# nv-tlabs/DiffusionTexturePainting

Measured on AMD Instinct MI355X. Metric: 512x512 inpaint stamps/sec @20 DDIM steps, higher is better.
Workload: dtype f16

## Files before the change

### diffusiontexturepainting_amd/_lib.py

```python
import ctypes as C
import os

import torch

_HERE = os.path.dirname(os.path.abspath(__file__))
LIB_PATH = os.environ.get("DTP_LIB") or os.path.join(_HERE, "libdtp.so")
_lib = None
MAX_SLOTS = 16
SCHEDULERS = {"DDIM": 0, "DPM": 1, "LMSD": 2}
SCHED_ROW = 8


def scheduler_id(name):
    if name not in SCHEDULERS:
        raise ValueError(f"scheduler {name!r} is not supported: choose one of {', '.join(SCHEDULERS)}")
    return SCHEDULERS[name]


class DtpError(RuntimeError):
    pass


class Settings(C.Structure):
    _fields_ = [("steps", C.c_int), ("context_pad", C.c_int), ("tg_steps", C.c_int), ("cfg_weight", C.c_float),
# ... 115 lines not shown
                ("st_out", C.c_void_p), ("st_in", C.c_void_p), ("st_parts", C.c_int), ("st_parts_out", C.c_int),
                ("W8", C.c_void_p), ("ldw8", C.c_int), ("a_scale", C.c_float), ("w_scale", C.c_float), ("gn_cpg", C.c_int), ("Wfr", C.c_void_p),
                ("A8", C.c_void_p), ("lda8", C.c_int), ("A2_8", C.c_void_p), ("lda2_8", C.c_int), ("C8", C.c_void_p), ("ldc8", C.c_int),
                ("c_scale", C.c_float), ("a2_scale", C.c_float)]


GF_BIAS, GF_BIAS_M, GF_RESID, GF_GEGLU, GF_GELU, GF_QUICKGELU, GF_OUT_F32, GF_SILU, GF_LNFOLD = 1, 2, 4, 8, 64, 128, 256, 512, 1024
GF_SOFTMAX16 = 4096
GF_ROWSTATS = 2048
GF_GNSTATS = 1 << 24
GF_RAGGED = 1 << 25

_vp, _i, _f, _i64 = C.c_void_p, C.c_int, C.c_float, C.c_int64
SYMBOLS = {
    "dtp_abi_version": (_i, []),
    "dtp_last_error": (C.c_char_p, []),
    "dtp_create": (_i, [_i, _i, _i, C.POINTER(_vp)]),
    "dtp_destroy": (None, [_vp]),
    "dtp_load_tensor": (_i, [_vp, C.c_char_p, _vp, _i, C.POINTER(_i64), _i]),
    "dtp_finalize_weights": (_i, [_vp]),
    "dtp_vae_encode": (_i, [_vp, _vp, _vp, _vp, _i, _vp]),
    "dtp_unet": (_i, [_vp, _vp, _f, _vp, _vp, _i, _vp]),
    "dtp_vae_decode": (_i, [_vp, _vp, _vp, _i, _vp]),
    "dtp_set_brush": (_i, [_vp, _vp, _i, _i, _vp, _vp]),
    "dtp_set_conditioning": (_i, [_vp, _vp, _vp, _vp, _vp]),
    "dtp_get_conditioning": (_i, [_vp, _vp, _vp, _vp]),
    "dtp_stamp": (_i, [_vp, _vp, C.POINTER(Settings), _vp, _vp, _vp, _i, _vp]),
    "dtp_stamp_slots": (_i, [_vp, _vp, C.POINTER(Settings), _vp, _vp, _vp, _i, C.POINTER(_i), _vp]),
    "dtp_stamp_mixed": (_i, [_vp, _vp, C.POINTER(Settings), _vp, _vp, _vp, _i, C.POINTER(_i), _vp]),
    "dtp_set_brush_slot": (_i, [_vp, _i, _vp, _i, _i, _vp, _vp]),
    "dtp_set_conditioning_slot": (_i, [_vp, _i, _vp, _vp, _vp, _vp]),
    "dtp_get_conditioning_slot": (_i, [_vp, _i, _vp, _vp, _vp]),
    "dtp_ddim_tables": (_i, [_i, C.POINTER(_i64), C.POINTER(_f), C.POINTER(_f)]),
    "dtp_last_stamp_times": (_i, [_vp, C.POINTER(_f * 3)]),
    "dtp_last_stamp_info": (_i, [_vp, C.POINTER(_i), C.POINTER(_i)]),
    "dtp_last_stamp_unet_rows": (_i, [_vp, C.POINTER(_i)]),
    "dtp_profile": (_i, [_vp, _i]),
    "dtp_profile_rows": (_i, [_vp, C.POINTER(ProfRow), _i, C.POINTER(_i)]),
    "dtp_profile_dump": (_i, [_vp, C.c_char_p]),
    "dtp_set_option": (_i, [_vp, C.c_char_p, _i]),
    "dtp_last_stamp_finite": (_i, [_vp, C.POINTER(_i)]),
    "dtp_op_gemm": (_i, [C.POINTER(GemmDesc), _vp]),
    "dtp_op_gemm_f8f8": (_i, [C.POINTER(GemmDesc), _vp]),
    "dtp_op_quant_e4m3": (_i, [_vp, _i, _vp, _i, _i, _f, _i, _vp, _i, _vp, _i, _i, _f, _i, _i, _vp, _i, _f, _vp]),
    "dtp_op_pack_linear": (_i, [_vp, _vp, _i, _i, _i, _i, _vp]),
    "dtp_op_pack_conv": (_i, [_vp, _vp, _i, _i, _i, _i, _i, _vp]),
    "dtp_op_rowsum": (_i, [_vp, _i, _i, _vp, _i, _vp]),
    "dtp_op_quantize_w8": (_i, [_vp, _i, _i, _i, _vp, _i, C.POINTER(_f), _vp]),
    "dtp_op_pack_conv_cb": (_i, [_vp, _vp, _i, _i, _i, _vp]),
    "dtp_op_groupnorm_apply": (_i, [_vp, _i, _vp, _i, _vp, _vp, _vp, _i, _i, _i, _i, _i, _f, _i, _vp]),
    "dtp_op_groupnorm_stats_apply": (_i, [_vp, _i, _vp, _vp, _vp, _vp, _vp, _vp, _i, _i, _i, _i, _f, _i, _vp]),
    "dtp_op_pack_conv_ws": (_i, [_vp, _vp, _vp, _i, _i, _i, _vp]),
    "dtp_op_pack_conv_ws_elems": (C.c_longlong, [_i, _i, _i]),
    "dtp_op_pack_linear_ws": (_i, [_vp, _i, _vp, _i, _i, _vp]),
    "dtp_op_pack_linear_ws_elems": (C.c_longlong, [_i, _i]),
    "dtp_op_groupnorm": (_i, [_vp, _i, _vp, _i, _vp, _vp, _i, _i, _i, _i, _f, _i, _vp]),
    "dtp_op_measure_peaks": (_i, [C.POINTER(C.c_double), C.POINTER(C.c_double)]),
    "dtp_op_reduce_groupnorm": (_i, [_vp, _i, _vp, _vp, _vp, _vp, _vp, _vp, _i, _i, _i, _i, _f, _i, _vp]),
    "dtp_op_xattn": (_i, [_vp, _vp, _vp, _vp, _vp, _i, _vp, _vp, _vp, _vp, _vp, _i, _i, _i, _i, _f, _vp]),
    "dtp_op_reduce_groupnorm_cx": (_i, [_vp, _i, _vp, _vp, _vp, _vp, _vp, _vp, _i, _i, _i, _i, _f, _i, _i, _vp]),
    "dtp_op_xattn_ct": (_i, [_vp, _vp, _vp, _vp, _vp, _i, _vp, _vp, _vp, _vp, _vp, _i, _i, _i, _i, _f, _i, _vp]),
    "dtp_op_gn_fold_weights": (_i, [_vp, _vp, _i, _vp, _vp, _vp, _i, _i, _i, _i, _i, _f, _vp, _vp, _vp]),
    "dtp_op_ffchain": (_i, [_vp, _vp, _i, _vp, _vp, _vp, _i, _vp, _vp, _vp, _i, _i, _f, _vp]),
    "dtp_op_xchain": (_i, [_vp, _vp, _i, _vp, _vp, _vp, _vp, _vp, _vp, _vp, _vp, _vp, _i, _i, _i, _i, _f, _vp]),
    "dtp_op_gn_linear": (_i, [_vp, _vp, _i, _vp, _vp, _vp, _i, _i, _i, _i, _i, _f, _vp, _vp, _i, _vp]),
    "dtp_op_layernorm": (_i, [_vp, _i, _vp, _i, _vp, _vp, _i, _i, _f, _vp]),
    "dtp_op_attention": (_i, [_vp, _vp, _vp, _vp, _i, _i, _i, _i, _i, _i, _i, _i, _i, _i64, _i64, _i64, _i64, _f, _vp]),
    "dtp_op_attention_dma": (_i, [_vp, _vp, _vp, _vp, _i, _i, _i, _i, _i, _i, _i, _i, _i, _i64, _i64, _i64, _i64, _f, _i, _vp]),
    "dtp_op_softmax_rows": (_i, [_vp, _i, _vp, _i, _i, _i, _f, _vp]),
    "dtp_op_attention_fp8": (_i, [_vp, _vp, _vp, _vp, _i, _i, _i, _i, _i, _i, _i, _i, _i, _i64, _i64, _i64, _i64, _f, _f, _f, _vp]),
    "dtp_op_dilate": (_i, [_vp, _vp, _vp, _i, _i, _i, _vp]),
    "dtp_op_dilate_pads": (_i, [_vp, _vp, _vp, _i, _i, C.POINTER(_i), _vp]),
    "dtp_scheduler_tables": (_i, [_i, _i, C.POINTER(_i), C.POINTER(_f), C.POINTER(_f), C.POINTER(_f), C.POINTER(_f)]),
    "dtp_op_sched_step": (_i, [_i, _vp, _vp, _vp, _vp, _vp, _vp, _vp, _vp, _vp, _i, _i, _i, _i, _vp]),
    "dtp_stamp_strength": (_i, [_vp, _vp, C.POINTER(Settings), _vp, _vp, _vp, C.c_double, _vp, _i, C.POINTER(_i), _vp]),
    "dtp_strength_schedule": (_i, [_i, _i, C.c_double, C.POINTER(_i), C.POINTER(_i), C.POINTER(_f)]),
    "dtp_op_strength_init": (_i, [_vp, _vp, _f, _f, _vp, C.c_longlong, _vp]),
    "dtp_stamp_seeded": (_i, [_vp, _vp, C.POINTER(Settings), C.POINTER(C.c_uint64), _i, C.c_double, _vp, _i, C.POINTER(_i), _vp]),
    "dtp_op_stamp_noise": (_i, [C.c_uint64, _i, _vp, C.c_longlong, _vp]),
    "dtp_philox4x32": (_i, [C.POINTER(C.c_uint32), C.POINTER(C.c_uint32), C.POINTER(C.c_uint32)]),
    "dtp_refit_stage": (_i, [_vp, C.c_char_p, _vp, _i, C.POINTER(_i64), _i]),
    "dtp_refit_lora": (_i, [_vp, _f]),
    "dtp_last_refit_info": (_i, [_vp, C.POINTER(_i), C.POINTER(_i), C.POINTER(_f)]),
    "dtp_op_lora_refit": (_i, [_vp, _vp, _vp, _i, _f, _vp, _vp, _i, _i, _i, _i, _vp]),
    "dtp_stroke": (_i, [_vp, _vp, _i, _i, C.POINTER(StrokeStamp), _i, C.POINTER(Settings), C.POINTER(StrokeOpts), _vp, _vp]),
    "dtp_stroke_plan": (_i, [_i, _i, _i, _i, C.POINTER(StrokeStamp), _i, _i, C.POINTER(_i), C.POINTER(_i)]),
    "dtp_last_stroke_info": (_i, [_vp, C.POINTER(_i), C.POINTER(_i), C.POINTER(_i)]),
    "dtp_op_stroke_gather": (_i, [_vp, _i, _i, _vp, _i, _i, C.POINTER(_i), C.POINTER(_i), C.POINTER(_i), _i, _i, _i, _vp]),
    "dtp_op_stroke_paste": (_i, [_vp, _vp, _vp, _i, _i, _i, _i, C.POINTER(_i), C.POINTER(_i), C.POINTER(_i), _i, _vp]),
    "dtp_mesh_create": (_i, [_vp, _vp, _i, _vp, _i, _vp, C.POINTER(_vp)]),
    "dtp_mesh_destroy": (_i, [_vp]),
    "dtp_mesh_camera": (_i, [C.POINTER(_f * 3), C.POINTER(_f * 3), C.POINTER(_f * 3), _f, C.POINTER(_f * 12)]),
    "dtp_mesh_stroke": (_i, [_vp, _vp, _vp, _i, _i, C.POINTER(MeshStamp), _i, C.POINTER(Settings), C.POINTER(MeshStrokeOpts), _vp, _vp]),
    "dtp_op_mesh_render": (_i, [_vp, C.POINTER(_f * 12), _f, _i, _vp, _i, _i, _i, _i, _i, _i, _vp, _vp, _vp]),
    "dtp_op_mesh_backproject": (_i, [_vp, _vp, _i, _vp, _vp, _i, _vp, _i, _i, _vp]),
    "dtp_mesh_stroke_bleed": (_i, [_vp, _vp, _vp, _i, _i, C.POINTER(MeshStamp), _i, C.POINTER(Settings), C.POINTER(MeshStrokeOpts), _vp, _i, _vp]),
    "dtp_mesh_bleed": (_i, [_vp, _vp, _i, _i, _i, C.POINTER(_i * 4), _vp]),
    "dtp_op_mesh_coverage": (_i, [_vp, _i, _i, _vp, _vp]),
    "dtp_mesh_bleed_offsets": (_i, [_i, C.POINTER(_i), C.POINTER(C.c_byte)]),
    "dtp_mesh_pick": (_i, [_vp, C.POINTER(Ray), _i, _vp, _vp]),
    "dtp_mesh_ray_frame": (_i, [C.POINTER(_f * 3), C.POINTER(_f * 3), C.POINTER(_f * 12)]),
    "dtp_mesh_path_plan": (_i, [_vp, _i, _f, C.POINTER(PathState), _vp, _vp, _vp, _i, C.POINTER(_i)]),
    "dtp_op_mesh_pick": (_i, [_vp, C.POINTER(Ray), _i, _vp, _vp]),
    "dtp_view_camera": (_i, [C.POINTER(_f * 3), C.POINTER(_f * 3), C.POINTER(_f * 3), _f, _i, _i, _f, C.POINTER(ViewCam)]),
    "dtp_view_rays": (_i, [C.POINTER(ViewCam), _i, _i, _vp, _i, _vp]),
    "dtp_mesh_view": (_i, [_vp, _vp, _i, _i, C.POINTER(ViewCam), _i, _i, C.POINTER(ViewOpts), _vp, _vp, _vp, _vp]),
# ... 68 lines not shown
```

### diffusiontexturepainting_amd/csrc/api_ops.hip

```cpp
#include <stdarg.h>
#include <stdio.h>
#include <stdlib.h>
#include <mutex>
#include <vector>

#include "../../include/dtp.h"
#include "common.h"

static thread_local char g_err[1024] = "";

void dtp_set_error(const char* fmt, ...) {
  va_list ap;
  va_start(ap, fmt);
  vsnprintf(g_err, sizeof(g_err), fmt, ap);
  va_end(ap);
}

namespace {
struct OpsScratch {
  f16* zero = nullptr;
  float* ws = nullptr;
  size_t ws_bytes = 0;
  int* geglu_map = nullptr;
  int geglu_map_n = 0;
  int num_cu = 256;
  bool init = false;
};
OpsScratch g_ops;
std::mutex g_ops_mu;

int ops_init() {
  if (g_ops.init) return DTP_OK;
  HIP_CHECK(hipMalloc(&g_ops.zero, 256));
  HIP_CHECK(hipMemset(g_ops.zero, 0, 256));
  hipDeviceProp_t prop;
  int dev = 0;
  HIP_CHECK(hipGetDevice(&dev));
  HIP_CHECK(hipGetDeviceProperties(&prop, dev));
  g_ops.num_cu = prop.multiProcessorCount;
  g_ops.init = true;
  return DTP_OK;
}

int ops_ws(size_t bytes) {
  if (bytes <= g_ops.ws_bytes) return DTP_OK;
  HIP_CHECK(hipDeviceSynchronize());
  if (g_ops.ws) HIP_CHECK(hipFree(g_ops.ws));
  g_ops.ws = nullptr;
  g_ops.ws_bytes = 0;
  HIP_CHECK(hipMalloc(&g_ops.ws, bytes));
  g_ops.ws_bytes = bytes;
  return DTP_OK;
}
}

extern "C" {

int dtp_abi_version(void) { return DTP_ABI_VERSION; }
const char* dtp_last_error(void) { return g_err; }

int dtp_op_gemm(dtp_gemm_desc* d, dtp_stream s) {
  std::lock_guard<std::mutex> lk(g_ops_mu);
  int rc = ops_init();
  if (rc) return rc;
  static bool halo_init = false;
  if (!halo_init) { dtp_conv_halo_init(); dtp_gemm_wide_init(); dtp_lnlin_init(); dtp_conv_ws_init(); dtp_gemm_ws_init(); halo_init = true; }
  GemmParams p = {};
  p.A = (const f16*)d->A; p.W = (const f16*)d->W; p.C = d->C; p.bias = d->bias; p.R = (const f16*)d->R;
  p.zero = g_ops.zero;
  p.M = d->M; p.N = d->N; p.K = d->K;
  p.lda = d->lda; p.ldw = d->ldw; p.ldc = d->ldc; p.ldr = d->ldr;
  p.nkb = (d->K + 63) / 64;
  p.Hi = d->Hi; p.Wi = d->Wi; p.Ho = d->Ho; p.Wo = d->Wo; p.Cin = d->Cin; p.stride = d->stride; p.pad = d->pad;
  p.flags = d->flags | (d->conv ? GF_CONV3 : 0) | (d->upsample2x ? GF_UPS2 : 0);
  p.lns = d->lns; p.ln_eps = d->ln_eps;
  p.A2 = (const f16*)d->A2; p.lda2 = d->lda2; p.Cin2 = d->Cin2;
  p.batch = d->batch; p.a_bs = d->a_bs; p.w_bs = d->w_bs; p.c_bs = d->c_bs; p.r_bs = d->r_bs;
  p.bias_bs = d->bias_bs; p.lns_bs = d->lns_bs; p.sm_valid = d->sm_valid;
  p.st_out = d->st_out; p.st_in = d->st_in; p.st_parts = d->st_parts;
  if (p.batch > 1) p.st_rows = p.batch * p.M;
  p.W8 = (const unsigned char*)d->W8; p.ldw8 = d->ldw8; p.a_scale = d->a_scale; p.w_scale = d->w_scale;
  p.Wfr = (const f16*)d->Wfr;
  p.gn_cpg = d->gn_cpg;
  static bool fp8_init = false;
  if (!fp8_init) { dtp_gemm_fp8_init(); fp8_init = true; }
  if (p.ldw < p.nkb * 64) { dtp_set_error("gemm: ldw=%d smaller than padded K=%d", p.ldw, p.nkb * 64); return DTP_ERR_ARG; }
  int tile = 0;
  dtp_gemm_pick(p, &tile, g_ops.num_cu);
  if (d->tile >= 0) tile = d->tile;
  const DtpTile t = dtp_tile(tile);
  int sp = t.split == SPLIT_COLS ? 4 : t.split == SPLIT_K ? p.splits : 1;
  if (d->splits >= 1 && (d->batch <= 1 || t.split != SPLIT_K)) sp = d->splits;
  if ((t.fam == TF_FP8) != (p.W8 != nullptr)) { dtp_set_error("gemm: tiles 24..28 and W8 go together"); return DTP_ERR_ARG; }
  if (t.fam == TF_HALO && !d->Wcb) { dtp_set_error("conv_halo: Wcb missing"); return DTP_ERR_ARG; }
  p.Wcb = (const f16*)d->Wcb;
  (void)dtp_tile_apply(p, tile, sp);
  rc = ops_ws(dtp_gemm_workspace_bytes(p));
  if (rc) return rc;
  p.part = g_ops.ws;
  if (p.flags & GF_ROWSTATS) d->st_parts_out = dtp_tile_row_parts(p, tile);
  return dtp_launch_tile(p, tile, (hipStream_t)s);
}

int dtp_op_gemm_f8f8(dtp_gemm_desc* d, dtp_stream s) {
  std::lock_guard<std::mutex> lk(g_ops_mu);
  int rc = ops_init();
  if (rc) return rc;
  static bool f8f8_init = false;
  if (!f8f8_init) { dtp_gemm_f8f8_init(); f8f8_init = true; }
  GemmParams p = {};
  p.A8 = (const unsigned char*)d->A8; p.lda8 = d->lda8;
  p.A2_8 = (const unsigned char*)d->A2_8; p.lda2_8 = d->lda2_8; p.Cin2 = d->A2_8 ? d->Cin2 : 0;
  p.W8 = (const unsigned char*)d->W8; p.ldw8 = d->ldw8;
  p.C = d->C; p.ldc = d->ldc; p.C8 = (unsigned char*)d->C8; p.ldc8 = d->ldc8;
  p.bias = d->bias; p.R = (const f16*)d->R; p.ldr = d->ldr;
  p.zero = g_ops.zero;
  p.M = d->M; p.N = d->N; p.K = d->K;
  p.flags = d->flags;
  p.st_out = d->st_out;
  p.a_scale = d->a_scale; p.w_scale = d->w_scale; p.c_scale = d->c_scale; p.a2_scale = d->a2_scale;
  p.splits = 1;
  const int tile = d->tile >= 0 ? d->tile : dtp_gemm_f8f8_pick(p, g_ops.num_cu);
  if (p.flags & GF_ROWSTATS) d->st_parts_out = (p.N + 127) / 128;
  return dtp_launch_gemm_f8f8(p, tile, (hipStream_t)s);
}

int dtp_op_quant_e4m3(const void* x, int ldx, void* y, int ldy, int K, float scale, int ln, const void* x2, int ldx2, void* y2, int ldy2,
                      int K2, float scale2, int ln2, int M, const float* st_in, int st_parts, float eps, dtp_stream s) {
  Quant8Params q = {};
  q.M = M; q.njobs = x2 ? 2 : 1;
  q.job[0] = Quant8Job{(const f16*)x, ldx, K, (unsigned char*)y, ldy, scale, ln};
  if (x2) q.job[1] = Quant8Job{(const f16*)x2, ldx2, K2, (unsigned char*)y2, ldy2, scale2, ln2};
  q.st_in = st_in; q.st_parts = st_parts; q.st_rows = M; q.eps = eps;
  return dtp_launch_quant8(q, (hipStream_t)s);
}

int dtp_op_pack_linear(const float* w, void* out, int N, int K, int ldw, int geglu, dtp_stream s) {
  std::lock_guard<std::mutex> lk(g_ops_mu);
  int rc = ops_init();
  if (rc) return rc;
  const int* map = nullptr;
  if (geglu) {
    if (N % 256) { dtp_set_error("pack_linear: GEGLU needs N %% 256 == 0"); return DTP_ERR_ARG; }
    std::vector<int> h(N);
    for (int f = 0; f < N / 2; ++f) {
      h[f] = (f / 64) * 128 + (f % 64);
      h[N / 2 + f] = (f / 64) * 128 + 64 + (f % 64);
    }
    if (g_ops.geglu_map_n < N) {
      if (g_ops.geglu_map) HIP_CHECK(hipFree(g_ops.geglu_map));
      HIP_CHECK(hipMalloc(&g_ops.geglu_map, sizeof(int) * N));
      g_ops.geglu_map_n = N;
    }
    HIP_CHECK(hipMemcpyAsync(g_ops.geglu_map, h.data(), sizeof(int) * N, hipMemcpyHostToDevice, (hipStream_t)s));
    HIP_CHECK(hipStreamSynchronize((hipStream_t)s));
    map = g_ops.geglu_map;
  }
  return dtp_launch_pack_linear_weight(w, (f16*)out, N, K, ldw, map, (hipStream_t)s);
}

int dtp_op_quantize_w8(const void* w, int ldw, int K, int rows, void* out, int ldw8, float* w_scale, dtp_stream s) {
  if (!w || !out || !w_scale || (ldw8 & 127) || ldw8 < K) { dtp_set_error("quantize_w8: bad argument"); return DTP_ERR_ARG; }
  return dtp_quantize_weights_fp8((const f16*)w, ldw, K, rows, (unsigned char*)out, ldw8, w_scale, (hipStream_t)s);
}

int dtp_op_rowsum(const void* w, int ld, int K, float* out, int rows, dtp_stream s) {
  return dtp_launch_rowsum_f16((const f16*)w, ld, K, out, rows, (hipStream_t)s);
}

int dtp_op_pack_conv(const float* w, void* out, int Cout, int Cin, int Cin_pad, int taps, int ldw, dtp_stream s) {
  return dtp_launch_pack_conv_weight(w, (f16*)out, Cout, Cin, Cin_pad, taps, ldw, (hipStream_t)s);
}

int dtp_op_pack_conv_cb(const float* w, void* out, int Cout, int Cin, int ldw, dtp_stream s) {
  return dtp_launch_pack_conv_weight_cb(w, (f16*)out, Cout, Cin, ldw, (hipStream_t)s);
}

int dtp_op_pack_conv_ws(const float* w, const float* w1, void* out, int Cout, int Cin, int Cin2, dtp_stream s) {
  return dtp_launch_pack_conv_ws(w, w1, (f16*)out, Cout, Cin, Cin2, (hipStream_t)s);
}
int dtp_op_pack_linear_ws(const void* w, int ldw, void* out, int N, int K, dtp_stream s) {
  return dtp_launch_pack_linear_ws((const f16*)w, ldw, (f16*)out, N, K, (hipStream_t)s);
}
long long dtp_op_pack_linear_ws_elems(int N, int K) { return (long long)dtp_gemm_ws_packed_elems(N, K); }
long long dtp_op_pack_conv_ws_elems(int Cout, int Cin, int Cin2) { return (long long)dtp_conv_ws_packed_elems(Cout, Cin, Cin2); }

int dtp_op_groupnorm(const void* x, int ldx, void* y, int ldy, const float* gamma, const float* beta, int B, int HW, int C,
                     int groups, float eps, int silu, dtp_stream s) {
  std::lock_guard<std::mutex> lk(g_ops_mu);
  int rc = ops_init();
  if (rc) return rc;
  rc = ops_ws(dtp_groupnorm_ws_bytes(B, HW, C, groups));
  if (rc) return rc;
  return dtp_launch_groupnorm(GnParams{(const f16*)x, ldx, (f16*)y, ldy, gamma, beta, B, HW, C, groups, eps, silu}, g_ops.ws, (hipStream_t)s);
}

int dtp_op_groupnorm_apply(const void* x, int ldx, void* y, int ldy, const float* gamma, const float* beta, const float* partial, int nchunk,
                           int B, int HW, int C, int groups, float eps, int silu, dtp_stream s) {
  return dtp_launch_groupnorm_apply(GnParams{(const f16*)x, ldx, (f16*)y, ldy, gamma, beta, B, HW, C, groups, eps, silu}, partial, nchunk, (hipStream_t)s);
}

int dtp_op_reduce_groupnorm_cx(const float* part, int splits, const float* bias, const void* resid, void* conv_out, void* y, const float* gamma,
                               const float* beta, int B, int HW, int C, int groups, float eps, int silu, int cx, dtp_stream s) {
  std::lock_guard<std::mutex> lk(g_ops_mu);
  int rc = ops_init();
  if (rc) return rc;
  rc = ops_ws(dtp_groupnorm_ws_bytes(B, HW, C, groups));
  if (rc) return rc;
  if (cx <= 0 || cx > C) { dtp_set_error("reduce_groupnorm: cx %d outside (0, C = %d]", cx, C); return DTP_ERR_ARG; }
  const GnReduceSrc rd = {part, splits, (long long)B * HW * cx, cx, bias, (const f16*)resid, cx};
  return dtp_launch_reduce_groupnorm(GnParams{(const f16*)conv_out, C, (f16*)y, C, gamma, beta, B, HW, C, groups, eps, silu}, rd, cx, g_ops.ws, (hipStream_t)s);
}

int dtp_op_reduce_groupnorm(const float* part, int splits, const float* bias, const void* resid, void* conv_out, void* y, const float* gamma,
                            const float* beta, int B, int HW, int C, int groups, float eps, int silu, dtp_stream s) {
  return dtp_op_reduce_groupnorm_cx(part, splits, bias, resid, conv_out, y, gamma, beta, B, HW, C, groups, eps, silu, C, s);
}

int dtp_op_gn_fold_weights(const void* x, const void* W, int ldw, const float* bias, const float* gamma, const float* beta, int B, int HW, int C,
                           int Nout, int groups, float eps, void* Wout, float* bias_out, dtp_stream s) {
  std::lock_guard<std::mutex> lk(g_ops_mu);
  int rc = ops_init();
  if (rc) return rc;
  rc = ops_ws(dtp_groupnorm_ws_bytes(B, HW, C, groups));
  if (rc) return rc;
  const GnParams gp = {(const f16*)x, C, nullptr, 0, gamma, beta, B, HW, C, groups, eps, 0};
  rc = dtp_launch_groupnorm_stats(gp, g_ops.ws, nullptr, (hipStream_t)s);
  if (rc) return rc;
  const int rows = (Nout + 127) / 128 * 128;
  return dtp_launch_gn_fold_weights(gp, g_ops.ws, 0, (const f16*)W, ldw, bias, Nout, (f16*)Wout, (long long)rows * ldw, bias_out, rows, (hipStream_t)s);
}

int dtp_op_groupnorm_stats_apply(const float* part, int splits, const float* bias, const void* resid, void* x, void* y, const float* gamma,
                                 const float* beta, int B, int HW, int C, int groups, float eps, int silu, dtp_stream s) {
  if (part && splits < 1) { dtp_set_error("groupnorm_stats_apply: %d slabs", splits); return DTP_ERR_ARG; }
  std::lock_guard<std::mutex> lk(g_ops_mu);
  int rc = ops_init();
  if (rc) return rc;
// ... 129 lines not shown
```

### diffusiontexturepainting_amd/csrc/builder.hip

```cpp
#include "engine.h"

#include <math.h>
#include <stdio.h>

#include <algorithm>

static Op make_gemm_op(Ctx* c, GemmParams p, int tile, int bias_step_off);

static const float* step_bias(const Ctx* c, int bias_step_off, int step, const float* fallback) {
  return bias_step_off >= 0 ? c->temb_table + (size_t)step * c->unet.temb_total + bias_step_off : fallback;
}
static constexpr int GF_CLAIMABLE = GF_BIAS | GF_RESID | GF_CONV3 | GF_UPS2 | GF_MFAST | GF_RAGGED;

void prog_push(Ctx* c, Prog* prog, int kind, double flops, double bytes, Op fn, const std::string& label) {
  prog->last_gemm.valid = false;
  prog->ops.push_back([=](hipStream_t s, int step) -> int {
    if (!c->profile) return fn(s, step);
    ProfRec r;
    r.kind = kind; r.flops = flops; r.bytes = bytes; r.label = label.c_str();
    HIP_CHECK(hipEventCreate(&r.e0));
    HIP_CHECK(hipEventCreate(&r.e1));
    HIP_CHECK(hipEventRecord(r.e0, s));
    const int rc = fn(s, step);
    HIP_CHECK(hipEventRecord(r.e1, s));
// ... 250 lines not shown
  HIP_CHECK(hipMemsetAsync(c->fp8_amax, 0, DTP_FP8_SLOTS * sizeof(unsigned int), s));
  c->calibrating = true;
  const int rc = up->main.run(s, step);
  c->calibrating = false;
  RC(rc);
  std::vector<float> amax(DTP_FP8_SLOTS);
  HIP_CHECK(hipMemcpyAsync(amax.data(), c->fp8_amax, DTP_FP8_SLOTS * sizeof(float), hipMemcpyDeviceToHost, s));
  HIP_CHECK(hipStreamSynchronize(s));
  auto pow2_for = [](float a) { return a > 0.f ? exp2f(ceilf(log2f(a * DTP_FP8_MARGIN / 448.0f))) : 1.0f; };
  for (size_t i = up->cal_begin; i < up->cal_end; ++i) {
    Fp8Cal& r = c->fp8_cals[i];
    if (r.kind == 0) {
      *r.s0 = pow2_for(amax[r.slot0]);
    } else {
      const float aq = amax[r.slot0] * r.softmax_scale * 1.4426950408889634f, ak = amax[r.slot0 + 1], av = amax[r.slot0 + 2];
      *r.s0 = (aq > 0.f && ak > 0.f) ? exp2f(roundf(0.5f * log2f(ak / aq))) : 1.0f;
      *r.s1 = pow2_for(av);
    }
  }
  up->fp8_calibrated = true;
  return DTP_OK;
}

static Op make_gemm_op(Ctx* c, GemmParams p, int tile, int bias_step_off) {
  return [=](hipStream_t s, int step) -> int {
    GemmParams q = p;
    q.part = c->ws;
    if (p.a_scale_host) {
      if (c->calibrating && p.amax_slot1 > 0) {
        const int ka = p.A2 ? p.K - p.Cin2 : p.K;
        RC(dtp_launch_amax_f16(p.A, p.M, ka, p.lda, c->fp8_amax + p.amax_slot1 - 1, s));
        if (p.A2) RC(dtp_launch_amax_f16(p.A2, p.M, p.Cin2, p.lda2, c->fp8_amax + p.amax_slot1 - 1, s));
      }
      q.a_scale = *p.a_scale_host;
    }
    q.bias = step_bias(c, bias_step_off, step, q.bias);
    return dtp_launch_tile(q, tile, s);
  };
}

int push_gemm(Ctx* c, Prog* prog, GemmParams p, int bias_step_off, double k_alg, RowStats* emit) {
  if (!emit_rowstats(p, emit)) emit = nullptr;
  int tile = 0;
  dtp_gemm_pick(p, &tile, c->num_cu);
  int sp = p.splits;
  if (p.W8) { tile = 24 + ((p.flags & GF_GEGLU) ? (p.M >= 512 ? 0 : 3) : (p.M >= 512 ? 0 : 2)); sp = 1; }
  if ((p.flags & GF_GNAPPLY) && (p.flags & GF_CONV3)) { tile = (p.Hi * p.Wi <= 256) ? 14 : 12; sp = 1; }
  if ((p.flags & GF_GNAPPLY) && !(p.flags & GF_CONV3)) {
    tile = DTP_TILE_LNLIN;
    sp = lnlin_default_ranges(p);
    if (!sp) { dtp_set_error("push_gemm: no lnlin configuration for the GroupNorm-on-load Linear (M %d N %d K %d)", p.M, p.N, p.K); return DTP_ERR_ARG; }
  }
  if (c->autotune) RC(tune_gemm(c, p, &tile, &sp));
  (void)dtp_tile_apply(p, tile, sp);
  const DtpTile t = dtp_tile(tile);
  if (emit) {
    emit->parts = dtp_tile_row_parts(p, tile);
    emit->M = p.M * (p.batch > 1 ? p.batch : 1);
  }
  c->ws_need = std::max(c->ws_need, dtp_gemm_workspace_bytes(p));
  p.zero = c->zero;
  const double n_out = (p.flags & GF_GEGLU) ? p.N / 2.0 : (double)p.N;
  const double a_elems = (p.flags & GF_CONV3) ? (double)p.M * (k_alg / 9.0) * ((p.flags & GF_UPS2) ? 0.25 : (double)(p.stride * p.stride))
                                               : (double)p.M * k_alg;
  const double nb = p.batch > 1 ? (double)p.batch : 1.0;
  const double bytes = 2.0 * nb * (a_elems + (double)p.N * k_alg + (double)p.M * n_out);
  char lab[160];
  const bool f8tile = t.fam == TF_FP8;
  snprintf(lab, sizeof(lab), "%s M=%d N=%d K=%d tile=%d splits=%d%s%s%s%s", (p.flags & GF_CONV3) ? "conv3" : "gemm", p.M, p.N, p.K, tile,
           t.split == SPLIT_COLS ? p.col_ranges : p.splits, (p.flags & GF_UPS2) ? " ups" : "", (p.flags & GF_GEGLU) ? (f8tile ? " geglu fp8" : " geglu") : (f8tile ? " fp8" : ""), p.stride == 2 ? " s2" : "",
           p.batch > 1 ? (" x" + std::to_string(p.batch)).c_str() : "");
  const double flops = 2.0 * nb * p.M * (double)p.N * k_alg;
  prog_push(c, prog, t.pk, flops, bytes, make_gemm_op(c, p, tile, bias_step_off), lab);
  if (p.splits > 1 || (t.fam == TF_CONVWS && t.var >= 2)) {
    LastGemm& lg = prog->last_gemm;
    lg.valid = true; lg.p = p; lg.tile = tile; lg.bias_step_off = bias_step_off; lg.op_index = prog->ops.size() - 1;
    lg.kind = t.pk; lg.flops = flops; lg.bytes = bytes; lg.label = lab;
  }
  return DTP_OK;
}

int Builder::conv3(const T& x, const ConvW& w, int stride, int pad, bool ups, int Ho, int Wo, const T* resid, int bias_step_off, T& y,
                   const Conv3Opts& o) {
  if ((w.cin2 > 0) != (o.tail != nullptr) || (o.tail && o.tail->C != w.cin2)) { dtp_set_error("conv3: shortcut tail mismatch"); return DTP_ERR_ARG; }
  if (x.C != w.cin || w.taps != 9) { dtp_set_error("conv3: channel mismatch %d vs %d", x.C, w.cin); return DTP_ERR_ARG; }
  GemmParams p = {};
  p.A = x.p; p.W = w.w;
  p.M = x.B * Ho * Wo; p.N = w.cout; p.K = w.K;
  p.lda = x.ld; p.ldw = w.ldw;
  p.nkb = w.ldw / 64;
  p.Hi = x.H; p.Wi = x.W; p.Ho = Ho; p.Wo = Wo; p.Cin = w.cin; p.stride = stride; p.pad = pad;
  p.flags = GF_CONV3 | (ups ? GF_UPS2 : 0) | o.extra_flags;
  if (c->R % 64) p.flags |= GF_RAGGED;
  if (o.tail) { p.A2 = o.tail->p; p.lda2 = o.tail->ld; p.Cin2 = w.cin2; }
  p.Wcb = w.wcb;
  p.Wfr = w.wfr;
  if (o.extra_flags & GF_GNAPPLY) {
    if (!o.gn.part) { dtp_set_error("conv3: GF_GNAPPLY without GroupNorm parameters"); return DTP_ERR_ARG; }
    p.gn_part = o.gn.part; p.gn_gamma = o.gn.gamma; p.gn_beta = o.gn.beta; p.gn_eps = o.gn.eps;
    p.gn_nchunk = o.gn.nchunk; p.gn_cpg = o.gn.cpg; p.gn_silu = 1;
  }
  if (o.out_override) {
    y = T();
    y.p = (f16*)o.out_override; y.B = x.B; y.H = Ho; y.W = Wo; y.C = w.cout; y.ld = o.ldc_override;
  } else if (o.dst) {
    if (o.dst->C != w.cout || o.dst->rows() != (long long)x.B * Ho * Wo) { dtp_set_error("conv3: destination view mismatch"); return DTP_ERR_ARG; }
    y = *o.dst;
  } else {
    y = alloc(x.B, Ho, Wo, w.cout);
    if (!y.p) return DTP_ERR_HIP;
  }
  p.C = y.p; p.ldc = y.ld;
  if (w.b || bias_step_off >= 0) { p.flags |= GF_BIAS; p.bias = w.b; }
  if (resid) { p.flags |= GF_RESID; p.R = resid->p; p.ldr = resid->ld; }
  return push_gemm(c, prog, p, bias_step_off, 9.0 * w.cin_true + w.cin2);
}

int Builder::gn_conv3(const T& x, const NormW& n, float eps, const ConvW& w, const T* resid, int bias_step_off, T& y, const T* tail, const T* dst) {
  Ctx* cc = c;
  const int HW = x.H * x.W, C = x.C;
  Conv3Opts opts;
  opts.tail = tail; opts.dst = dst;
  const bool fuse = cc->fuse_gn_conv && HW >= 1024 && x.rows() <= 16384 && w.wcb && w.taps == 9 && (C & 63) == 0 && C <= 1024 && x.C == w.cin && (C % 32) == 0 && C / 32 >= 8 &&
                    (w.cout & 7) == 0 && (x.ld & 7) == 0;
  if (!fuse) {
    T t;
    RC(gn(x, n, eps, true, t));
    RC(conv3(t, w, 1, 1, false, x.H, x.W, resid, bias_step_off, y, opts));
    release(t);
    return DTP_OK;
  }
  const ReduceClaim claim = claim_reduce(x);
  float* partials = (float*)block_clear_of_claim(cc, dtp_groupnorm_ws_bytes(x.B, HW, C, 32), claim, "gn_conv3", "partials");
  if (!partials) return DTP_ERR_HIP;
  cc->ws_need = std::max(cc->ws_need, claim.slab_bytes());
  push_gn_stats(*this, gn_params(x, n, eps, true), partials, claim, " (apply in conv)");
  opts.extra_flags = GF_GNAPPLY; opts.gn = {partials, n.g, n.b, eps, dtp_groupnorm_stat_chunks(HW), C / 32};
  const int rc = conv3(x, w, 1, 1, false, x.H, x.W, resid, bias_step_off, y, opts);
  ctx_pool_put(cc, partials);
  return rc;
}

int Builder::alloc_stats(long long rows, int C, RowStats& st) {
  void* p = nullptr;
  RC(ctx_pool_get(c, (size_t)((C + 63) / 64) * rows * 2 * sizeof(float), &p));
  st.buf = (float*)p;
  st.parts = 0;
  st.M = (int)rows;
  return DTP_OK;
// ... 176 lines not shown
```

### diffusiontexturepainting_amd/csrc/common.h

```cpp
#pragma once
#include <hip/hip_runtime.h>
#include <stdint.h>

#include "../../include/dtp.h"

typedef _Float16 f16;
typedef f16 f16x2 __attribute__((ext_vector_type(2)));
typedef f16 f16x4 __attribute__((ext_vector_type(4)));
typedef f16 f16x8 __attribute__((ext_vector_type(8)));
typedef float f32x4 __attribute__((ext_vector_type(4)));
typedef float f32x16 __attribute__((ext_vector_type(16)));

static __device__ __forceinline__ uint32_t lds_addr(const void* p) {
  return (uint32_t)(uintptr_t)(const __attribute__((address_space(3))) void*)p;
}
static __device__ __forceinline__ f16x8 lds_read16(uint32_t addr) {
  f16x8 v;
  asm volatile("ds_read_b128 %0, %1" : "=v"(v) : "v"(addr));
  return v;
}
template <int N, int NF>
static __device__ __forceinline__ void wait_lds_frags(f16x8 (&f)[NF]) {
  static_assert(NF == 2 || NF == 3 || NF == 4 || NF == 5 || NF == 6 || NF == 7 || NF == 8, "fragment count");
  if constexpr (NF == 2) asm volatile("s_waitcnt lgkmcnt(%2)" : "+v"(f[0]), "+v"(f[1]) : "n"(N));
// ... 140 lines not shown
}
static __device__ __forceinline__ void gn_mean_rstd(double s, double q, float inv_count, float eps, float& mean, float& rstd) {
  const float nf = rintf(1.0f / inv_count);
  const double n = (double)nf;
  double inv = (double)(1.0f / nf);
  inv = inv * (2.0 - n * inv);
  const double m = s * inv;
  const double var = q * inv - m * m;
  mean = (float)m;
  rstd = rsqrtf(fmaxf((float)var, 0.f) + eps);
}

#define DTP_WAVE 64

#define HIP_CHECK(x)                                                                        \
  do {                                                                                      \
    hipError_t e_ = (x);                                                                    \
    if (e_ != hipSuccess) {                                                                 \
      dtp_set_error("%s:%d %s -> %s", __FILE__, __LINE__, #x, hipGetErrorString(e_));       \
      return DTP_ERR_HIP;                                                                   \
    }                                                                                       \
  } while (0)


void dtp_set_error(const char* fmt, ...);

enum {
  GF_BIAS = 1,
  GF_BIAS_M = 2,
  GF_RESID = 4,
  GF_GEGLU = 8,
  GF_CONV3 = 16,
  GF_UPS2 = 32,
  GF_GELU = 64,
  GF_QUICKGELU = 128,
  GF_OUT_F32 = 256,
  GF_SILU = 512,
  GF_LNFOLD = 1024,
  GF_ROWSTATS = 2048,
  GF_SOFTMAX16 = 4096,
  GF_MFAST = 1 << 20,
  GF_NOREDUCE = 1 << 21,
  GF_XCDSPLIT = 1 << 23,
  GF_GNSTATS = 1 << 24,
  GF_RAGGED = 1 << 25,
  GF_GNAPPLY = 1 << 22,
};

struct GemmParams {
  const f16* A;
  const f16* W;
  const f16* Wcb;
  const f16* Wfr;
  void* C;
  float* part;
  const float* bias;
  const f16* R;
  const f16* zero;
  const float* lns;
  float ln_eps;
  const float* st_in;
  int st_parts;
  float* st_out;
  int M, N, K;
  int lda, ldw, ldc, ldr;
  int nkb;
  int splits;
  int kb_per_split;
  int col_ranges;
  int Hi, Wi, Ho, Wo, Cin, stride, pad;
  const f16* A2;
  int lda2, Cin2;
  int flags;
  int batch;
  long long a_bs, w_bs, c_bs, r_bs;
  int bias_bs, lns_bs, st_rows;
  int sm_valid;
  const float *gn_part, *gn_gamma, *gn_beta;
  int gn_nchunk, gn_cpg, gn_silu;
  float gn_eps;
  const unsigned char* W8;
  int ldw8;
  float a_scale, w_scale;
  const float* a_scale_host;
  int amax_slot1;
  const unsigned char* A8;
  int lda8;
  const unsigned char* A2_8;
  int lda2_8;
  unsigned char* C8;
  int ldc8;
  float c_scale;
  float a2_scale;
};

struct Quant8Job {
  const f16* x; int ld, K;
  unsigned char* y; int ldy;
  float scale;
  int ln;
};
struct Quant8Params {
  int M, njobs;
  Quant8Job job[2];
  const float* st_in; int st_parts, st_rows;
  float eps;
// ... 93 lines not shown
  int dup;
};
bool dtp_xchain_supported(const XchainParams& p);
int dtp_launch_xchain(const XchainParams& p, hipStream_t s);
void dtp_xchain_init();

struct FfchainParams {
  const f16* X; int ldx;
  const f16* W1; int ldw1;
  const float *lns1, *b1;
  const f16* Wm; int ldwm;
  const float* bm;
  const f16* R; int ldr;
  f16* Out; int ldo;
  int M, C;
  float ln_eps;
};
bool dtp_ffchain_supported(const FfchainParams& p);
int dtp_launch_ffchain(const FfchainParams& p, hipStream_t s);
void dtp_ffchain_init();

int dtp_launch_concat_channels(const f16* a, int lda, int Ca, const f16* b, int ldb, int Cb, f16* y, int ldy, long long rows,
                               hipStream_t s);
#define DTP_COPY_SEGS 8
struct CopySegs {
  int n;
  const char* src[DTP_COPY_SEGS];
  char* dst[DTP_COPY_SEGS];
  long long rows[DTP_COPY_SEGS], row_bytes[DTP_COPY_SEGS], src_stride[DTP_COPY_SEGS], dst_stride[DTP_COPY_SEGS];
  long long chunks[DTP_COPY_SEGS], total;
};
int dtp_launch_copy_rows(CopySegs segs, hipStream_t s);
int dtp_launch_f32_to_f16(const float* x, f16* y, long long n, hipStream_t s);
int dtp_launch_nchw_f32_to_nhwc_f16(const float* x, f16* y, int B, int C, int HW, int Cpad, hipStream_t s);
int dtp_launch_nhwc_f16_to_nchw_f32(const f16* x, int ldx, float* y, int B, int C, int HW, hipStream_t s);
int dtp_launch_pack_conv_weight(const float* w, f16* out, int Cout, int Cin, int Cin_pad, int taps, int ldw, hipStream_t s);
int dtp_launch_pack_linear_weight(const float* w, f16* out, int N, int K, int ldw, const int* row_map, hipStream_t s);
int dtp_launch_rowdot(const float* w, const float* v, float* out, int N, int K, hipStream_t s);
int dtp_launch_scale_cols(float* w, const float* g, int N, int K, hipStream_t s);
int dtp_launch_rowsum_f16(const f16* w, int ld, int K, float* out, int rows, hipStream_t s);
int dtp_launch_matmul_f32(const float* A, const float* B, float* C, int M, int N, int K, hipStream_t s);
int dtp_launch_expand_kv(const f16* kv, f16* kexp, f16* vexp, int N, int T, int C, int H, float scale, hipStream_t s);
int dtp_launch_transpose_f16(const f16* src, int lds_, f16* dst, int ldd, int rows, int cols, hipStream_t s);
int dtp_launch_rowdot_f16(const f16* a, int ld, const float* v, float* out, int rows, int K, hipStream_t s);
bool dtp_gemm_fp8_supported(const GemmParams& p);
int dtp_launch_gemm_fp8(const GemmParams& p, int tile, hipStream_t s);
void dtp_gemm_fp8_init();
int dtp_quantize_weights_fp8(const f16* w, int ldw, int K, int rows, unsigned char* out, int ldw8, float* scale_out, hipStream_t s);
bool dtp_gemm_wide_supported(const GemmParams& p, int variant);
int dtp_launch_gemm_wide(const GemmParams& p, int variant, hipStream_t s);
void dtp_gemm_wide_init();
constexpr int DTP_TILE_LNLIN = 50;
constexpr int DTP_TILE_WS0 = 51;
constexpr int DTP_WS_VARIANTS = 4;
constexpr int DTP_TILE_GEMMWS = 55;
constexpr int DTP_TILE_IDS = 56;

enum { PK_GEMM0 = 0, PK_ATTN = 12, PK_GN = 13, PK_LN = 14, PK_ELEM = 15, PK_SOFTMAX = 16, PK_HALO0 = 17, PK_BIG0 = 21, PK_WIDE0 = 25, PK_FP8 = 27, PK_KH2 = 28, PK_LW = 36, PK_XATTN = 44, PK_HALO3 = 45, PK_LNLIN = 47, PK_WS0 = 48, PK_GEMMWS = 52, PK_F8F8 = 53, PK_QUANT8 = 54, PK_COUNT = 55 };

enum DtpFamily : unsigned char { TF_NONE, TF_GEMM, TF_HALO, TF_WIDE, TF_FP8, TF_LNLIN, TF_CONVWS, TF_GEMMWS };
enum DtpSplit : unsigned char {
  SPLIT_K,
  SPLIT_HALO,
  SPLIT_BLOCKS,
  SPLIT_COLS,
  SPLIT_NONE,
};
struct DtpTile {
  DtpFamily fam;
  int var;
  int bm, bn, ns;
  int kh, lw;
  DtpSplit split;
  int pk;
};
inline DtpTile dtp_tile(int id) {
  static constexpr int sm[4] = {128, 128, 64, 64}, sn[4] = {128, 64, 64, 128};
  const int s = id & 3;
  if (id >= 0 && id < 12) return {TF_GEMM, 0, sm[s], sn[s], 2 + id / 4, 1, 0, SPLIT_K, PK_GEMM0 + id};
  if (id >= 12 && id < 16) return {TF_HALO, id - 12, 0, 0, 0, 0, 0, SPLIT_HALO, PK_HALO0 + id - 12};
  if (id >= 16 && id < 20) return {TF_GEMM, 0, id < 18 ? 256 : 128, id < 18 ? 128 : 256, 2 + (id & 1), 1, 0, SPLIT_K, PK_BIG0 + id - 16};
  if (id == 20 || id == 21) return {TF_WIDE, id - 20, 256, id == 20 ? 256 : 320, 2, 0, 0, SPLIT_NONE, PK_WIDE0 + id - 20};
  if (id >= 24 && id < 28) return {TF_FP8, id - 24, sm[s], sn[s], 2, 0, 0, SPLIT_NONE, PK_FP8};
  if (id == 28) return {TF_FP8, 4, 256, 256, 2, 0, 0, SPLIT_NONE, PK_FP8};
  if (id >= 32 && id < 40) return {TF_GEMM, 0, sm[s], sn[s], 2 + (id - 32) / 4, 2, 0, SPLIT_K, PK_KH2 + id - 32};
  if (id >= 40 && id < 48) return {TF_GEMM, 0, sm[s], sn[s], 3, 1, id < 44 ? 4 : 8, SPLIT_K, PK_LW + id - 40};
  if (id == 48 || id == 49) return {TF_HALO, id - 44, 0, 0, 0, 0, 0, SPLIT_HALO, PK_HALO3 + id - 48};
  if (id == DTP_TILE_LNLIN) return {TF_LNLIN, 0, 0, 0, 0, 0, 0, SPLIT_COLS, PK_LNLIN};
  if (id >= DTP_TILE_WS0 && id < DTP_TILE_WS0 + DTP_WS_VARIANTS) return {TF_CONVWS, id - DTP_TILE_WS0, 0, 0, 0, 0, 0, SPLIT_BLOCKS, PK_WS0 + id - DTP_TILE_WS0};
  if (id == DTP_TILE_GEMMWS) return {TF_GEMMWS, 0, 64, 64, 0, 0, 0, SPLIT_BLOCKS, PK_GEMMWS};
  return {};
}
inline bool dtp_tile_apply(GemmParams& p, int tile, int sp) {
  const DtpTile t = dtp_tile(tile);
  if (sp < 1) sp = 1;
  if (t.fam == TF_HALO) p.W = p.Wcb;
  if (t.split == SPLIT_NONE || t.split == SPLIT_COLS) {
    p.kb_per_split = p.nkb; p.splits = 1;
    if (t.split == SPLIT_COLS) p.col_ranges = sp;
    return t.split == SPLIT_COLS || sp == 1;
  }
  p.kb_per_split = (p.nkb + sp - 1) / sp;
  if (t.split == SPLIT_BLOCKS) { p.splits = sp; return true; }
  if (t.split == SPLIT_HALO && sp > 1) p.kb_per_split = (((p.nkb + 8) / 9 + sp - 1) / sp) * 9;
  p.splits = (p.nkb + p.kb_per_split - 1) / p.kb_per_split;
  return p.splits == sp;
}
inline int dtp_tile_row_parts(const GemmParams& p, int tile) {
  const DtpTile t = dtp_tile(tile);
  if (t.split == SPLIT_COLS) return p.col_ranges;
  if (!t.bn) return 0;
  return p.splits > 1 ? 1 : (p.N + t.bn - 1) / t.bn;
}
bool dtp_lnlin_supported(const GemmParams& p, int nsplit);
int dtp_launch_lnlin(const GemmParams& p, int nsplit, hipStream_t s);
void dtp_lnlin_init();
bool dtp_conv_ws_supported(const GemmParams& p, int variant, int nsplit);
int dtp_launch_conv_ws(const GemmParams& p, int variant, hipStream_t s);
void dtp_conv_ws_init();
size_t dtp_conv_ws_packed_elems(int Cout, int Cin, int Cin2);
int dtp_conv_ws_gn_chunks(int Ho, int Wo);
int dtp_launch_pack_conv_ws(const float* w, const float* w1, f16* out, int Cout, int Cin, int Cin2, hipStream_t s);
bool dtp_gemm_ws_supported(const GemmParams& p, int nsplit);
int dtp_launch_gemm_ws(const GemmParams& p, hipStream_t s);
void dtp_gemm_ws_init();
size_t dtp_gemm_ws_packed_elems(int N, int K);
int dtp_launch_pack_linear_ws(const f16* w, int ldw, f16* out, int N, int K, hipStream_t s);
bool dtp_conv_halo_supported(const GemmParams& p);
bool dtp_conv_halo3_supported(const GemmParams& p);
int dtp_launch_conv_halo(const GemmParams& p, int variant, hipStream_t s);
void dtp_conv_halo_init();
int dtp_launch_pack_conv_weight_cb(const float* w, f16* out, int Cout, int Cin, int ldw, hipStream_t s);
int dtp_launch_touch(const void* p, size_t bytes, float* sink, hipStream_t s);
int dtp_launch_amax_f16(const f16* x, long long rows, int cols, int ld, unsigned int* slot, hipStream_t s);
int dtp_launch_lora_merge(float* w, const float* up, const float* down, int N, int K, int rank, float scale, hipStream_t s);
```

### diffusiontexturepainting_amd/csrc/context.hip

```cpp
#include <stdio.h>
#include <stdlib.h>
#include <string.h>
#include <algorithm>

#include "engine.h"

int stamp_init(Ctx* c) {
  void* p;
  const size_t hw = (size_t)c->h * c->h, RR = (size_t)c->R * c->R;
  RC(ctx_persistent(c, c->maxB * hw * 4 * 4, &p, true)); c->x32 = (float*)p;
  RC(ctx_persistent(c, 3 * c->maxB * hw * 4 * 4, &p, true)); c->hist32 = (float*)p;
  RC(ctx_persistent(c, c->maxB * 4 * RR * 4, &p, true)); c->canvas32 = (float*)p;
  RC(ctx_persistent(c, 2 * c->maxB * RR * 4, &p, true)); c->alpha_tmp = (float*)p;
  RC(ctx_persistent(c, sizeof(StampParams), &p, true)); c->stamp_params = (StampParams*)p;
  RC(ctx_persistent(c, (size_t)DTP_MAX_SLOTS * 2 * 14 * 768 * 4, &p, true)); c->cond32 = (float*)p;
  RC(ctx_persistent(c, (size_t)DTP_MAX_SLOTS * 3 * RR * 4, &p, true)); c->brush32 = (float*)p;
  RC(ctx_persistent(c, 64 * sizeof(int), &p, true)); c->slot_map = (int*)p;
  RC(ctx_persistent(c, 256, &p, true)); c->finite_flag = (int*)p;
  RC(ctx_persistent(c, RR * 4, &p, true)); c->mesh_face_idx = (int*)p;
  return DTP_OK;
}

extern "C" {

int dtp_create(int device, int resolution, int max_batch, dtp_ctx** out) {
  if (!out || resolution < 64 || resolution % 8 || max_batch < 1 || max_batch > 64) {
    dtp_set_error("dtp_create: resolution must be a multiple of 8 and at least 64, 1 <= max_batch <= 64 (got resolution %d, max_batch %d)", resolution, max_batch);
    return DTP_ERR_ARG;
  }
  HIP_CHECK(hipSetDevice(device));
  Ctx* c = new Ctx();
  c->device = device; c->R = resolution; c->h = resolution / 8; c->maxB = max_batch;
  hipDeviceProp_t prop;
  HIP_CHECK(hipGetDeviceProperties(&prop, device));
  c->num_cu = prop.multiProcessorCount;
  void* z;
  HIP_CHECK(hipMalloc(&z, 4096));
  HIP_CHECK(hipMemset(z, 0, 4096));
  c->zero = (f16*)z;
  for (int i = 0; i < 4; ++i) HIP_CHECK(hipEventCreate(&c->ev[i]));
  tune_cache_load(c);
  auto on = [](const char* name) { const char* e = getenv(name); return e && e[0] && e[0] != '0'; };
  c->fuse_reduce_gn = !on("DTP_NO_FUSE_REDUCE_GN"); c->dedupe_prefix = !on("DTP_NO_DEDUPE");
#ifdef DTP_EXPERIMENTAL
  c->fuse_gn_conv = on("DTP_GN_CONV");
#endif
  c->fuse_xattn = !on("DTP_NO_XATTN"); c->fold_gn_linear = !on("DTP_NO_FOLD_GN");
  c->conv_ws = !on("DTP_NO_WS"); c->conv_ws_vae = !on("DTP_NO_WS_VAE"); c->gemm_ws = on("DTP_GEMMWS");
  c->gn_epilogue = !on("DTP_NO_GN_EPILOGUE"); c->reduce_in_concat_gn = !on("DTP_NO_REDUCE_IN_CONCAT_GN"); c->gna_lnlin = !on("DTP_NO_GNA_LNLIN");
  c->tune_lnlin = !on("DTP_NO_LNLIN"); c->tune_halo3 = !on("DTP_NO_HALO3");
  c->xchain = !on("DTP_NO_XCHAIN"); c->xattn_tiles = !on("DTP_XATTN_CT1");
  if (const char* e = getenv("DTP_FFCHAIN")) c->ffchain = atoi(e);
  *out = (dtp_ctx*)c;
  return DTP_OK;
}

void dtp_destroy(dtp_ctx* ctx) {
  Ctx* c = (Ctx*)ctx;
  if (!c) return;
  (void)hipSetDevice(c->device);
  (void)hipDeviceSynchronize();
  graphs_drop_all(c);
  journal_drop_ctx(c);
  delta_drop_ctx(c);
  mesh_drop_ctx(c);
  for (auto& s : c->staged) (void)hipFree(s.second.d);
  for (auto& s : c->refit_staged) (void)hipFree(s.second.d);
  for (int i = 0; i < 2; ++i) if (c->refit_ev[i]) (void)hipEventDestroy(c->refit_ev[i]);
  for (void* p : c->chunks) (void)hipFree(p);
  for (auto& b : c->pool.blocks) (void)hipFree(b.p);
  for (void* p : c->persistent) (void)hipFree(p);
  if (c->ws) (void)hipFree(c->ws);
  if (c->zero) (void)hipFree(c->zero);
  if (c->tune_thrash) (void)hipFree(c->tune_thrash);
  for (int i = 0; i < 4; ++i) if (c->ev[i]) (void)hipEventDestroy(c->ev[i]);
  delete c;
}

int dtp_load_tensor(dtp_ctx* ctx, const char* name, const float* data, int is_device, const int64_t* shape, int ndim) {
  Ctx* c = (Ctx*)ctx;
  if (!c || !name || !data || ndim < 1 || ndim > 4) { dtp_set_error("dtp_load_tensor: bad argument"); return DTP_ERR_ARG; }
  if (c->finalized) { dtp_set_error("dtp_load_tensor: weights already finalized"); return DTP_ERR_STATE; }
  HIP_CHECK(hipSetDevice(c->device));
  Staged s;
  s.n = 1;
  for (int i = 0; i < ndim; ++i) { s.shape.push_back(shape[i]); s.n *= (size_t)shape[i]; }
  HIP_CHECK(hipMalloc(&s.d, std::max<size_t>(s.n * 4, 16)));
  HIP_CHECK(hipMemcpy(s.d, data, s.n * 4, is_device ? hipMemcpyDeviceToDevice : hipMemcpyHostToDevice));
  auto it = c->staged.find(name);
  if (it != c->staged.end()) { (void)hipFree(it->second.d); c->staged.erase(it); }
  c->staged.emplace(name, std::move(s));
  return DTP_OK;
}

int dtp_finalize_weights(dtp_ctx* ctx) {
  Ctx* c = (Ctx*)ctx;
  if (!c) { dtp_set_error("dtp_finalize_weights: null handle"); return DTP_ERR_ARG; }
  if (c->finalized) { dtp_set_error("dtp_finalize_weights: already finalized"); return DTP_ERR_STATE; }
  HIP_CHECK(hipSetDevice(c->device));
  dtp_gemm_init();
  dtp_conv_halo_init();
  dtp_gemm_wide_init();
  dtp_gemm_fp8_init();
  dtp_gemm_f8f8_init();
  dtp_xattn_init();
// ... 75 lines not shown
  c->profile = enable != 0;
  return DTP_OK;
}

int dtp_profile_rows(dtp_ctx* ctx, dtp_prof_row* rows, int max_rows, int* n_rows) {
  Ctx* c = (Ctx*)ctx;
  if (!c || !rows || !n_rows) return DTP_ERR_ARG;
  HIP_CHECK(hipDeviceSynchronize());
  dtp_prof_row acc[PK_COUNT] = {};
  for (int k = 0; k < PK_COUNT; ++k) acc[k].kind = k;
  for (const ProfRec& r : c->prof) {
    float ms = 0.f;
    HIP_CHECK(hipEventElapsedTime(&ms, r.e0, r.e1));
    dtp_prof_row& a = acc[r.kind];
    a.launches += 1; a.ms += ms; a.flops += r.flops; a.bytes += r.bytes;
  }
  int n = 0;
  for (int k = 0; k < PK_COUNT && n < max_rows; ++k)
    if (acc[k].launches) rows[n++] = acc[k];
  *n_rows = n;
  return DTP_OK;
}

int dtp_profile_dump(dtp_ctx* ctx, const char* path) {
  Ctx* c = (Ctx*)ctx;
  if (!c || !path) return DTP_ERR_ARG;
  HIP_CHECK(hipDeviceSynchronize());
  FILE* f = fopen(path, "w");
  if (!f) { dtp_set_error("dtp_profile_dump: cannot open %s", path); return DTP_ERR_ARG; }
  fprintf(f, "kind,us,tflops,algo_GBps,label\n");
  for (const ProfRec& r : c->prof) {
    float ms = 0.f;
    (void)hipEventElapsedTime(&ms, r.e0, r.e1);
    fprintf(f, "%d,%.2f,%.1f,%.1f,%s\n", r.kind, ms * 1e3, r.flops / (ms * 1e-3) / 1e12, r.bytes / (ms * 1e-3) / 1e9, r.label ? r.label : "");
  }
  fclose(f);
  return DTP_OK;
}

int dtp_set_option(dtp_ctx* ctx, const char* name, int value) {
  Ctx* c = (Ctx*)ctx;
  if (!c || !name) return DTP_ERR_ARG;
  if (!strcmp(name, "scheduler")) {
    if (value != DTP_SCHED_DDIM && value != DTP_SCHED_DPM && value != DTP_SCHED_LMSD) {
      dtp_set_error("dtp_set_option: scheduler %d is not one of DDIM = 0, DPM = 1, LMSD = 2", value);
      return DTP_ERR_ARG;
    }
    c->scheduler = value;
    return DTP_OK;
  }
  if (!strcmp(name, "use_graph")) { c->use_graph = value != 0; return DTP_OK; }
  if (!strcmp(name, "autotune")) { c->autotune = value != 0; return DTP_OK; }
  if (!strcmp(name, "check_finite")) { c->check_finite = value != 0; return DTP_OK; }
  if (!strcmp(name, "fuse_gn_conv")) {
#ifndef DTP_EXPERIMENTAL
    if (value) { dtp_set_error("dtp_set_option: fuse_gn_conv is an experiment (slower: DESIGN.md 3.6) -- build with DTP_EXPERIMENTAL=1"); return DTP_ERR_ARG; }
#endif
    if (!c->unet_progs.empty() || !c->enc_progs.empty() || !c->dec_progs.empty()) {
      dtp_set_error("dtp_set_option: fuse_gn_conv must be chosen before the first launch program is built");
      return DTP_ERR_STATE;
    }
    c->fuse_gn_conv = value != 0;
    return DTP_OK;
  }
  if (!strcmp(name, "dedupe_prefix")) {
    c->dedupe_prefix = value != 0;
    graphs_drop_all(c);
    return DTP_OK;
  }
  if (value && c->R % 64 && (!strcmp(name, "fp8_linear") || !strcmp(name, "fp8_operands") || !strcmp(name, "fp8_attention"))) {
    dtp_set_error("dtp_set_option: %s is parity-only and not offered at resolution %d (a multiple of 8 that is not a multiple of 64)", name, c->R);
    return DTP_ERR_STATE;
  }
  const struct { const char* name; bool Ctx::*flag; } fp8[] = {
      {"fp8_linear", &Ctx::fp8_linear}, {"fp8_operands", &Ctx::fp8_operands}, {"fp8_attention", &Ctx::fp8_attention}};
  for (const auto& o : fp8) {
    if (strcmp(name, o.name)) continue;
    if (!c->unet_progs.empty() && c->*o.flag != (value != 0)) {
      dtp_set_error("dtp_set_option: %s must be chosen before the first UNet program is built", o.name);
      return DTP_ERR_STATE;
    }
    c->*o.flag = value != 0;
    return DTP_OK;
  }
  dtp_set_error("dtp_set_option: unknown option '%s'", name);
  return DTP_ERR_ARG;
}

int dtp_last_stamp_info(dtp_ctx* ctx, int* unet_evals, int* graph_nodes) {
  Ctx* c = (Ctx*)ctx;
  if (!c) return DTP_ERR_ARG;
  if (unet_evals) *unet_evals = c->last_evals;
  if (graph_nodes) *graph_nodes = c->last_nodes;
  return DTP_OK;
}

int dtp_last_stamp_unet_rows(dtp_ctx* ctx, int* rows) {
  Ctx* c = (Ctx*)ctx;
  if (!c || !rows) return DTP_ERR_ARG;
  *rows = c->last_unet_rows;
  return DTP_OK;
}

}
```

### diffusiontexturepainting_amd/csrc/conv_ws.hip

```cpp
#include <stdlib.h>
#include <type_traits>

#include "common.h"

namespace {

typedef __attribute__((address_space(3))) void* lds_ptr_t;
typedef unsigned int u32x4 __attribute__((ext_vector_type(4)));

template <int OFF>
__device__ __forceinline__ f16x8 lds_read16_off(uint32_t addr) {
  f16x8 v;
  asm volatile("ds_read_b128 %0, %1 offset:%2" : "=v"(v) : "v"(addr), "n"(OFF));
  return v;
}
template <int N>
__device__ __forceinline__ void wait_vmcnt() { asm volatile("s_waitcnt vmcnt(%0)" ::"n"(N) : "memory"); }

template <int TH, int TW, int NI, int NT, bool CO = false>
struct WsGeom {
  static constexpr int PW = TW + 3, PH = TH + 2;
  static constexpr int HP1 = PH * PW, HP = NI * HP1;
  static constexpr int HL = (HP + 31) / 32;
  static constexpr int PBYTES = HL * 32 * 128;
  static constexpr int TM = NI * TH * TW / 32;
  static constexpr int RPT = 32 / TW, TPI = TH / RPT;
  static constexpr int CBLK = 1152;
  static constexpr int CMB = 4 * (CO ? 1 : NT) * TM * 4 * CBLK;
  static constexpr int MAINB = (3 * PBYTES > CMB ? 3 * PBYTES : CMB);
  static constexpr int STATB = (NI == 1 && NT == 2) ? (4 * NT * 32 * 2 + NT * 32 * 2) * 8 : 0;
  static constexpr int LDS = MAINB + STATB;
  static constexpr int LT = (HL - 1) / (NT * TM);
  static constexpr int WAITB = (17 - LT) * NT;
  static_assert(TW == 8 || TW == 16, "pixel tile width");
  static_assert(TH % RPT == 0 && (NI * TH * TW) % 32 == 0, "whole MFMA tiles");
  static_assert(HP * 128 < 65536, "fragment offsets are 16-bit immediates");
  static_assert(LT < 8 && WAITB < 64, "patch pieces fit in the taps before the barrier; vmcnt is a 6-bit counter");
  static_assert(LDS <= (CO ? 80 : 160) * 1024, "LDS");
};

__global__ void pack_conv_ws_kernel(const float* __restrict__ w, f16* __restrict__ out, int Cout, int Cin, long long total) {
  for (long long i = (long long)blockIdx.x * 256 + threadIdx.x; i < total; i += (long long)gridDim.x * 256) {
    const int e = (int)(i & 7), l = (int)((i >> 3) & 63);
    long long f = i >> 9;
    const int tap = (int)(f % 9); f /= 9;
    const int wq = (int)(f & 3); f >>= 2;
    const int ncb = Cin >> 6;
    const int cb = (int)(f % ncb), nt = (int)(f / ncb);
    const int n = nt * 32 + (l & 31), ch = cb * 64 + 16 * wq + 8 * (l >> 5) + e;
    out[i] = n < Cout ? (f16)w[((size_t)n * Cin + ch) * 9 + tap] : (f16)0.f;
  }
}

__global__ void pack_conv_ws_tail_kernel(const float* __restrict__ w, f16* __restrict__ out, int Cout, int Cin2, long long total) {
  for (long long i = (long long)blockIdx.x * 256 + threadIdx.x; i < total; i += (long long)gridDim.x * 256) {
    const int e = (int)(i & 7), l = (int)((i >> 3) & 63);
    long long g = i >> 9;
    const int wq = (int)(g & 3); g >>= 2;
    const int ntb = Cin2 >> 6;
    const int tb = (int)(g % ntb), nt = (int)(g / ntb);
    const int n = nt * 32 + (l & 31), ch = tb * 64 + 16 * wq + 8 * (l >> 5) + e;
    out[i] = n < Cout ? (f16)w[(size_t)n * Cin2 + ch] : (f16)0.f;
  }
}

template <class G, int KY, int J>
__device__ __forceinline__ void rd_frags(f16x8 (&dst)[G::TM], uint32_t ct) {
  if constexpr (J < G::TM) {
    dst[J] = lds_read16_off<((J / G::TPI) * G::HP1 + (G::RPT * (J % G::TPI) + KY) * G::PW) * 128>(ct);
    rd_frags<G, KY, J + 1>(dst, ct);
  }
}

template <int TH, int TW, int NI, int NT, bool NTW, bool CO = false, bool RAG = false>
__global__ __launch_bounds__(256, CO ? 2 : 1) void convws_kernel(const GemmParams p) {
  using G = WsGeom<TH, TW, NI, NT, CO>;
  constexpr int TM = G::TM, HL = G::HL, PW = G::PW, PH = G::PH, HP1 = G::HP1, PB = G::PBYTES, NTM = NT * TM;
  extern __shared__ __attribute__((aligned(16))) char smem[];

  const int tid = threadIdx.x, lane = tid & 63;
  const int wave = __builtin_amdgcn_readfirstlane(tid >> 6);
  const int frow = lane & 31, fhalf = lane >> 5;

  const int H = p.Ho, W = p.Wo;
  const int tiles_x = RAG ? (W + TW - 1) / TW : W / TW, tiles_y = RAG ? (H + TH - 1) / TH : H / TH;
  const int hw = H * W;
  const bool pow2 = ((hw & (hw - 1)) | (tiles_x & (tiles_x - 1)) | (tiles_y & (tiles_y - 1))) == 0;
  const int images = pow2 ? (p.M >> __builtin_ctz(hw)) : p.M / hw;
  const int npg = (images / NI) * tiles_y * tiles_x;
  const int nts = (p.N + 31) >> 5, nrs = (nts + NT - 1) / NT, S = p.splits;
  const int units = nrs * S;
  const int xcd = blockIdx.x & 7, idx = blockIdx.x >> 3;
  int pg, u;
  if ((units & 7) == 0) { const int q = idx / npg; pg = idx - q * npg; u = q * 8 + xcd; }
  else { const int pgq = (npg + 7) >> 3; const int q = idx / pgq; pg = (idx - q * pgq) * 8 + xcd; u = q; }
  if (u >= units || pg >= npg) return;
  const int ncb = p.Cin >> 6;
  int z = 0, nr = u, mb0 = 0, mb1 = ncb;
  if (S > 1) {
    nr = u / S; z = u - nr * S;
    mb0 = z * ncb / S; mb1 = (z + 1) * ncb / S;
  }
  int tx, ty, img0;
  if (pow2) {
    const int sx = __builtin_ctz(tiles_x), sy = __builtin_ctz(tiles_y);
    tx = pg & (tiles_x - 1); ty = (pg >> sx) & (tiles_y - 1); img0 = (pg >> (sx + sy)) * NI;
  } else {
    tx = pg % tiles_x; ty = (pg / tiles_x) % tiles_y; img0 = (pg / (tiles_x * tiles_y)) * NI;
  }
  const int y0 = ty * TH, x0 = tx * TW;

  const auto rsW = __builtin_amdgcn_make_buffer_rsrc((void*)p.Wfr, 0, (int)0x80000000u, 0x00020000);
  constexpr int OOB = (int)0x80000000u;
  int wvoff[NT], wbase[NT];
#pragma unroll
  for (int i = 0; i < NT; ++i) {
    const int nt = nr * NT + i;
    wvoff[i] = nt < nts ? lane * 16 : OOB;
    wbase[i] = (nt < nts ? nt : 0) * ncb * 4 + wave;
  }
  auto wload = [&](int i, int cb, int tap) -> f16x8 {
    const u32x4 v = __builtin_amdgcn_raw_buffer_load_b128(rsW, wvoff[i], ((wbase[i] + cb * 4) * 9 + tap) * 1024, NTW ? 2 : 0);
    return __builtin_bit_cast(f16x8, v);
  };
  f16x8 wf[NT][9];
  if (mb0 < mb1) {
#pragma unroll
    for (int t = 0; t < 9; ++t)
#pragma unroll
      for (int i = 0; i < NT; ++i) wf[i][t] = wload(i, mb0, t);
  }
  __builtin_amdgcn_sched_barrier(0);

  const auto rsA = __builtin_amdgcn_make_buffer_rsrc((void*)p.A, 0, (int)0x80000000u, 0x00020000);
  int voffA[HL];
  {
    const int ups = (p.flags & GF_UPS2) ? 1 : 0;
    const int s0 = wave * 8 + (lane >> 3);
    int il = 0, hy = s0 / PW, hx = s0 - hy * PW;
    constexpr int DY = 32 / PW, DX = 32 - DY * PW;
#pragma unroll
    for (int i = 0; i < HL; ++i) {
      const int iy = y0 + hy - 1, ix = x0 + hx - 1;
      const bool ok = il < NI && hx < TW + 2 && (unsigned)iy < (unsigned)H && (unsigned)ix < (unsigned)W;
      voffA[i] = ok ? ((((img0 + il) * p.Hi + (iy >> ups)) * p.Wi + (ix >> ups)) * p.lda + (((lane & 7) ^ (hx & 7)) << 3)) * 2 : -1;
      hx += DX; hy += DY;
      if (hx >= PW) { hx -= PW; ++hy; }
      if (hy >= PH) { hy -= PH; ++il; }
    }
  }
  auto a_piece_at = [&](uint32_t bo, int cb, int i) {
    const int vo = voffA[i];
    __builtin_amdgcn_raw_ptr_buffer_load_lds(rsA, (lds_ptr_t)(smem + bo + (i * 4 + wave) * 1024), 16, vo, cb * 128, 0, 0);
  };
  if (mb0 < mb1) {
#pragma unroll
    for (int i = 0; i < HL; ++i) a_piece_at(0u, mb0, i);
    if (mb0 + 1 < mb1) {
#pragma unroll
      for (int i = 0; i < HL; ++i) a_piece_at((uint32_t)PB, mb0 + 1, i);
    }
  }

  const int pxl = frow % TW, pyl = frow / TW;
  uint32_t colterm[3];
#pragma unroll
  for (int kx = 0; kx < 3; ++kx)
    colterm[kx] = lds_addr(smem) + (pyl * PW + pxl + kx) * 128 + ((((2 * wave + fhalf) ^ ((pxl + kx) & 7))) << 4);

  f32x16 acc[NT][TM];
#pragma unroll
  for (int i = 0; i < NT; ++i)
#pragma unroll
    for (int j = 0; j < TM; ++j)
#pragma unroll
      for (int r = 0; r < 16; ++r) acc[i][j][r] = 0.f;

  constexpr int NBF = CO ? 2 : 3;
  f16x8 bf[NBF][TM];
  auto rd = [&](auto tapc, uint32_t bo, f16x8 (&dst)[TM]) {
    constexpr int TAP = decltype(tapc)::value, KY = TAP / 3, KX = TAP % 3;
#ifndef DTP_WS_NO_LDSREAD
    rd_frags<G, KY, 0>(dst, colterm[KX] + bo);
#else
#pragma unroll
    for (int j = 0; j < TM; ++j) asm volatile("" : "+v"(dst[j]));
#endif
  };
  if (mb0 < mb1 && !(p.sm_valid & 1)) {
    wait_vmcnt<0>();
    __builtin_amdgcn_s_barrier();
    rd(std::integral_constant<int, 0>{}, 0u, bf[0]);
    auto do_cb = [&](auto morec, auto more2c, int cb, uint32_t bo, uint32_t bo1, uint32_t bo2) {
      constexpr bool MORE = decltype(morec)::value, MORE2 = decltype(more2c)::value;
      auto tap = [&](auto tapc) {
        constexpr int TAP = decltype(tapc)::value, CUR = TAP % NBF, NXT = (TAP + 1) % NBF;
        __builtin_amdgcn_sched_barrier(0);
#ifdef DTP_WS_NO_LDSREAD
#define DTP_WS_WAIT(n, f) asm volatile("" ::: "memory")
#else
#define DTP_WS_WAIT(n, f) wait_lds_frags<n, TM>(f)
#endif
        if constexpr (TAP < 8) {
          rd(std::integral_constant<int, TAP + 1>{}, bo, bf[NXT]);
          __builtin_amdgcn_sched_barrier(0);
          DTP_WS_WAIT(TM, bf[CUR]);
        } else {
          DTP_WS_WAIT(0, bf[CUR]);
          if constexpr (MORE) {
            wait_vmcnt<G::WAITB>();
            __builtin_amdgcn_s_barrier();
            if constexpr (!CO) {
              rd(std::integral_constant<int, 0>{}, bo1, bf[NXT]);
              __builtin_amdgcn_sched_barrier(0);
            }
          }
        }
#pragma unroll
        for (int j = 0; j < TM; ++j)
#pragma unroll
          for (int i = 0; i < NT; ++i) {
#ifndef DTP_WS_NO_MFMA
            acc[i][j] = __builtin_amdgcn_mfma_f32_32x32x16_f16(wf[i][TAP], bf[CUR][j], acc[i][j], 0, 0, 0);
#else
            asm volatile("" : "+v"(acc[i][j]) : "v"(wf[i][TAP]), "v"(bf[CUR][j]));
#endif
            if constexpr (MORE2) {
              if (TAP * NTM + j * NT + i < HL) {
                __builtin_amdgcn_sched_barrier(0);
#ifndef DTP_WS_NO_DMA
                a_piece_at(bo2, cb + 2, TAP * NTM + j * NT + i);
#endif
                __builtin_amdgcn_sched_barrier(0);
              }
            }
          }
        if constexpr (MORE) {
          __builtin_amdgcn_sched_barrier(0);
#ifndef DTP_WS_NO_WLOAD
#pragma unroll
          for (int i = 0; i < NT; ++i) wf[i][TAP] = wload(i, cb + 1, TAP);
#endif
          __builtin_amdgcn_sched_barrier(0);
          if constexpr (CO && TAP == 8) rd(std::integral_constant<int, 0>{}, bo1, bf[0]);
        }
      };
#undef DTP_WS_WAIT
      tap(std::integral_constant<int, 0>{}); tap(std::integral_constant<int, 1>{}); tap(std::integral_constant<int, 2>{});
      tap(std::integral_constant<int, 3>{}); tap(std::integral_constant<int, 4>{}); tap(std::integral_constant<int, 5>{});
      tap(std::integral_constant<int, 6>{}); tap(std::integral_constant<int, 7>{}); tap(std::integral_constant<int, 8>{});
    };
    typedef std::true_type Y;
    typedef std::false_type N_;
    uint32_t bo = 0, bo1 = PB, bo2 = 2 * PB;
    int cb = mb0;
    for (; cb + 2 < mb1; ++cb) {
      do_cb(Y{}, Y{}, cb, bo, bo1, bo2);
      const uint32_t t = bo; bo = bo1; bo1 = bo2; bo2 = t;
    }
    if (cb + 1 < mb1) {
      do_cb(Y{}, N_{}, cb, bo, bo1, bo2);
      ++cb;
      bo = bo1;
    }
    do_cb(N_{}, N_{}, cb, bo, bo1, bo2);
  }

  if (p.A2 && !(p.sm_valid & 1)) {
    const int ntb = p.Cin2 >> 6;
    const int tk0 = (int)((long long)z * ntb / S), tk1 = (int)((long long)(z + 1) * ntb / S);
    if (tk0 < tk1) {
      const auto rsT = __builtin_amdgcn_make_buffer_rsrc((void*)p.A2, 0, (int)0x80000000u, 0x00020000);
      int voffT[TM];
#pragma unroll
      for (int j = 0; j < TM; ++j) {
        const int il = j / G::TPI, py = G::RPT * (j % G::TPI) + pyl;
        voffT[j] = ((((img0 + il) * H + y0 + py) * W + x0 + pxl) * p.lda2 + 8 * fhalf) * 2;
        if (RAG && (y0 + py >= H || x0 + pxl >= W)) voffT[j] = OOB;
      }
      int tbase[NT];
#pragma unroll
      for (int i = 0; i < NT; ++i) tbase[i] = nts * ncb * 36 + (nr * NT + i < nts ? nr * NT + i : 0) * ntb * 4;
      constexpr int D = CO ? 2 : (TM % 4 == 0) ? 4 : 3;
      static_assert(TM % D == 0, "tile ring");
      f16x8 ring[4 * D];
      constexpr int WTB = CO ? 1 : 2;
      f16x8 wt[WTB][NT][4];
      auto frag_load = [&](int tb, int j, int slot) {
        const int vo = tb < tk1 ? voffT[j] : OOB;
#pragma unroll
        for (int ks = 0; ks < 4; ++ks) {
          const u32x4 v = __builtin_amdgcn_raw_buffer_load_b128(rsT, vo, tb * 128 + ks * 32, 0);
          ring[slot * 4 + ks] = __builtin_bit_cast(f16x8, v);
        }
      };
      auto wt_load = [&](int tb, int par) {
#pragma unroll
        for (int i = 0; i < NT; ++i) {
          const int vo = tb < tk1 ? wvoff[i] : OOB;
#pragma unroll
          for (int ks = 0; ks < 4; ++ks) {
            const u32x4 v = __builtin_amdgcn_raw_buffer_load_b128(rsW, vo, (tbase[i] + tb * 4 + ks) * 1024, NTW ? 2 : 0);
            wt[par % WTB][i][ks] = __builtin_bit_cast(f16x8, v);
          }
        }
      };
      const int nround = (tk1 - tk0 + 3) >> 2;
      int tb = tk0 + wave;
      wt_load(tb, 0);
#pragma unroll
      for (int j = 0; j < D; ++j) frag_load(tb, j, j);
      auto block = [&](auto parc, int tbc, bool more) {
        constexpr int PAR = decltype(parc)::value % WTB;
        if (WTB == 2 && more) wt_load(tbc + 4, PAR ^ 1);
#pragma unroll
        for (int j = 0; j < TM; ++j) {
#pragma unroll
          for (int ks = 0; ks < 4; ++ks)
#pragma unroll
            for (int i = 0; i < NT; ++i)
              acc[i][j] = __builtin_amdgcn_mfma_f32_32x32x16_f16(wt[PAR][i][ks], ring[(j % D) * 4 + ks], acc[i][j], 0, 0, 0);
// ... 3 lines not shown
        if (WTB == 1 && more) wt_load(tbc + 4, 0);
      };
      for (int r = 0; r < nround; r += 2) {
        block(std::integral_constant<int, 0>{}, tb, r + 1 < nround);
        if (r + 1 < nround) block(std::integral_constant<int, 1>{}, tb + 4, r + 2 < nround);
        tb += 8;
      }
    }
  }

  if (p.sm_valid & 2) return;
  __builtin_amdgcn_s_barrier();
  constexpr int CB = G::CBLK;
  constexpr int RT = CO ? 1 : NT;
  const int epx = tid >> 3, c4 = tid & 7;
  const int epxl = epx % TW, epyl = epx / TW;
  const char* const src0 = smem + (c4 >> 1) * CB + ((epx * 2 + (c4 & 1)) ^ ((epx >> 2) & 1)) * 16;
  constexpr bool CAN_STATS = G::STATB > 0;
  const bool stats = CAN_STATS && (p.flags & GF_GNSTATS) && p.splits == 1;
  double* const sred = (double*)(smem + G::MAINB);
#pragma unroll
  for (int i0 = 0; i0 < NT; i0 += RT) {
    if (i0 > 0) __syncthreads();
    {
      char* const mine = smem + wave * RT * TM * 4 * CB + ((frow * 2 + fhalf) ^ ((frow >> 2) & 1)) * 16;
#pragma unroll
      for (int i = 0; i < RT; ++i)
#pragma unroll
        for (int j = 0; j < TM; ++j)
#pragma unroll
          for (int q = 0; q < 4; ++q) {
            const f32x4 v = {acc[i0 + i][j][4 * q], acc[i0 + i][j][4 * q + 1], acc[i0 + i][j][4 * q + 2], acc[i0 + i][j][4 * q + 3]};
            *(f32x4*)(mine + ((i * TM + j) * 4 + q) * CB) = v;
          }
    }
    __syncthreads();
#pragma unroll
    for (int i = 0; i < RT; ++i) {
      const int n = (nr * NT + i0 + i) * 32 + 4 * c4;
      const bool ncol = n + 4 <= p.N;
      f32x4 bv = {0.f, 0.f, 0.f, 0.f};
      if (p.splits == 1 && (p.flags & GF_BIAS) && ncol) bv = *(const f32x4*)(p.bias + n);
      float ssum[4] = {0.f, 0.f, 0.f, 0.f}, qsum[4] = {0.f, 0.f, 0.f, 0.f};
#pragma unroll
      for (int j = 0; j < TM; ++j) {
        const char* src = src0 + (i * TM + j) * 4 * CB;
        const f32x4 v0 = *(const f32x4*)src, v1 = *(const f32x4*)(src + RT * TM * 4 * CB), v2 = *(const f32x4*)(src + 2 * RT * TM * 4 * CB),
                    v3 = *(const f32x4*)(src + 3 * RT * TM * 4 * CB);
        f32x4 v;
#pragma unroll
        for (int e = 0; e < 4; ++e) v[e] = ((v0[e] + v1[e]) + v2[e]) + v3[e];
        const int il = j / G::TPI, py = G::RPT * (j % G::TPI) + epyl;
        if (RAG && (y0 + py >= H || x0 + epxl >= W)) continue;
        const size_t m = ((size_t)(img0 + il) * H + y0 + py) * W + x0 + epxl;
        if (!ncol) continue;
        if (p.splits > 1) {
          *(f32x4*)(p.part + ((size_t)z * p.M + m) * p.N + n) = v;
        } else {
#pragma unroll
          for (int e = 0; e < 4; ++e) v[e] += bv[e];
          if (p.flags & GF_RESID) {
            const f16x4 r = *(const f16x4*)(p.R + m * p.ldr + n);
#pragma unroll
            for (int e = 0; e < 4; ++e) v[e] += (float)r[e];
          }
          const f16x4 o = {(f16)v[0], (f16)v[1], (f16)v[2], (f16)v[3]};
          *(f16x4*)((f16*)p.C + m * p.ldc + n) = o;
          if constexpr (CAN_STATS) {
#pragma unroll
            for (int e = 0; e < 4; ++e) { const float f = (float)o[e]; ssum[e] += f; qsum[e] += f * f; }
          }
        }
      }
      if constexpr (CAN_STATS) {
        if (stats) {
          double sd[4], qd[4];
#pragma unroll
          for (int e = 0; e < 4; ++e) {
            sd[e] = (double)ssum[e]; qd[e] = (double)qsum[e];
#pragma unroll
            for (int o = 8; o < 64; o <<= 1) { sd[e] += shfl_xor_d(sd[e], o); qd[e] += shfl_xor_d(qd[e], o); }
          }
          if (lane < 8) {
            double* d = sred + ((wave * NT + i0 + i) * 32 + 4 * c4) * 2;
#pragma unroll
            for (int e = 0; e < 4; ++e) { d[2 * e] = sd[e]; d[2 * e + 1] = qd[e]; }
          }
        }
      }
    }
  }
  if constexpr (CAN_STATS) {
    if (stats) {
      __syncthreads();
      double* const tot = sred + 4 * NT * 32 * 2;
      if (tid < NT * 32 * 2) tot[tid] = ((sred[tid] + sred[NT * 64 + tid]) + sred[2 * NT * 64 + tid]) + sred[3 * NT * 64 + tid];
      __syncthreads();
      const int cpg = p.gn_cpg, groups = p.N / cpg;
      const int c_lo = nr * NT * 32, c_hi = min(p.N, c_lo + NT * 32);
      const int g_lo = c_lo / cpg, g_hi = (c_hi - 1) / cpg;
      const int g = g_lo + tid;
      if (g <= g_hi) {
        const int a = max(g * cpg, c_lo), b = min((g + 1) * cpg, c_hi);
        double sg = 0.0, qg = 0.0;
        for (int c = a; c < b; ++c) { sg += tot[(c - c_lo) * 2]; qg += tot[(c - c_lo) * 2 + 1]; }
        const int ntile = tiles_x * tiles_y, pt = ty * tiles_x + tx;
        float* const base = p.st_out + ((size_t)img0 * 2 * ntile + 2 * pt) * groups * 2;
        float* const mine = base + (size_t)(nr & 1) * groups * 2 + g * 2;
        mine[0] = (float)sg; mine[1] = (float)qg;
        if (g * cpg >= c_lo && (g + 1) * cpg <= c_hi) {
          float* const other = base + (size_t)((nr & 1) ^ 1) * groups * 2 + g * 2;
          other[0] = 0.f; other[1] = 0.f;
        }
      }
    }
  }
}

template <int TH, int TW, int NI, int NT, bool CO = false>
int launch_ws(const GemmParams& p, hipStream_t s) {
  using G = WsGeom<TH, TW, NI, NT, CO>;
  const bool rag = (p.Ho % TH) || (p.Wo % TW);
  const int npg = (p.M / (p.Ho * p.Wo) / NI) * ((p.Ho + TH - 1) / TH) * ((p.Wo + TW - 1) / TW);
  const int nrs = (((p.N + 31) >> 5) + NT - 1) / NT;
  const int units = nrs * p.splits;
  const int blocks = (units & 7) == 0 ? units * npg : ((npg + 7) >> 3) * 8 * units;
  static const int dbg = [] { const char* e = getenv("DTP_WS_DEBUG"); return e ? atoi(e) : 0; }();
  GemmParams q = p;
  q.sm_valid = dbg & 3;
  const bool nt = (dbg & 4) ? false : (dbg & 8) ? true : npg == 1;
  if constexpr (NI == 1 && NT == 2) {
    if (rag) {
      if (nt) hipLaunchKernelGGL((convws_kernel<TH, TW, NI, NT, true, CO, true>), dim3(blocks), dim3(256), G::LDS, s, q);
      else hipLaunchKernelGGL((convws_kernel<TH, TW, NI, NT, false, CO, true>), dim3(blocks), dim3(256), G::LDS, s, q);
      return hipGetLastError() == hipSuccess ? DTP_OK : DTP_ERR_HIP;
    }
  }
  if (nt) hipLaunchKernelGGL((convws_kernel<TH, TW, NI, NT, true, CO>), dim3(blocks), dim3(256), G::LDS, s, q);
  else hipLaunchKernelGGL((convws_kernel<TH, TW, NI, NT, false, CO>), dim3(blocks), dim3(256), G::LDS, s, q);
  return hipGetLastError() == hipSuccess ? DTP_OK : DTP_ERR_HIP;
}

template <int TH, int TW, int NI, int NT, bool CO = false>
void set_ws_attr() {
  (void)hipFuncSetAttribute((const void*)convws_kernel<TH, TW, NI, NT, true, CO>, hipFuncAttributeMaxDynamicSharedMemorySize, WsGeom<TH, TW, NI, NT, CO>::LDS);
  (void)hipFuncSetAttribute((const void*)convws_kernel<TH, TW, NI, NT, false, CO>, hipFuncAttributeMaxDynamicSharedMemorySize, WsGeom<TH, TW, NI, NT, CO>::LDS);
  if constexpr (NI == 1 && NT == 2) {
    (void)hipFuncSetAttribute((const void*)convws_kernel<TH, TW, NI, NT, true, CO, true>, hipFuncAttributeMaxDynamicSharedMemorySize, WsGeom<TH, TW, NI, NT, CO>::LDS);
    (void)hipFuncSetAttribute((const void*)convws_kernel<TH, TW, NI, NT, false, CO, true>, hipFuncAttributeMaxDynamicSharedMemorySize, WsGeom<TH, TW, NI, NT, CO>::LDS);
  }
}

}

void dtp_conv_ws_init() {
  set_ws_attr<8, 8, 3, 1>();
  set_ws_attr<16, 16, 1, 1>();
  set_ws_attr<8, 16, 1, 2>();
  set_ws_attr<8, 16, 1, 2, true>();
}

int dtp_conv_ws_gn_chunks(int Ho, int Wo) { return 2 * ((Ho + 7) / 8) * ((Wo + 15) / 16); }

size_t dtp_conv_ws_packed_elems(int Cout, int Cin, int Cin2) { return (size_t)((Cout + 31) / 32) * ((size_t)(Cin / 64) * 36 + (size_t)(Cin2 / 64) * 4) * 512; }

int dtp_launch_pack_conv_ws(const float* w, const float* w1, f16* out, int Cout, int Cin, int Cin2, hipStream_t s) {
  if ((Cin & 63) || (Cin2 & 63) || (Cin2 > 0) != (w1 != nullptr)) { dtp_set_error("pack_conv_ws: Cin %d / Cin2 %d must be multiples of 64", Cin, Cin2); return DTP_ERR_ARG; }
  const long long total = (long long)dtp_conv_ws_packed_elems(Cout, Cin, 0);
  const int blocks = (int)((total + 255) / 256 > 65535 ? 65535 : (total + 255) / 256);
  hipLaunchKernelGGL(pack_conv_ws_kernel, dim3(blocks), dim3(256), 0, s, w, out, Cout, Cin, total);
  if (Cin2 > 0) {
    const long long t2 = (long long)dtp_conv_ws_packed_elems(Cout, 0, Cin2);
    const int b2 = (int)((t2 + 255) / 256 > 65535 ? 65535 : (t2 + 255) / 256);
    hipLaunchKernelGGL(pack_conv_ws_tail_kernel, dim3(b2), dim3(256), 0, s, w1, out + total, Cout, Cin2, t2);
  }
  return hipGetLastError() == hipSuccess ? DTP_OK : DTP_ERR_HIP;
}

bool dtp_conv_ws_supported(const GemmParams& p, int variant, int nsplit) {
  if (!p.Wfr || !(p.flags & GF_CONV3) || p.batch > 1) return false;
  if (p.A2 && ((p.Cin2 & 63) || (p.lda2 & 7) || (size_t)p.M * p.lda2 * 2 >= ((size_t)1 << 31))) return false;
  if (p.flags & (GF_GEGLU | GF_OUT_F32 | GF_LNFOLD | GF_ROWSTATS | GF_BIAS_M | GF_GELU | GF_QUICKGELU | GF_SILU | GF_GNAPPLY | GF_SOFTMAX16)) return false;
  if (p.stride != 1 || p.pad != 1 || (p.Cin & 63) || (p.N & 3) || (p.lda & 7) || (p.ldc & 3)) return false;
  const bool rag = (p.flags & GF_RAGGED) != 0;
  if (p.flags & GF_UPS2) {
    if ((p.Ho != 2 * p.Hi && !(rag && p.Ho == 2 * p.Hi - 1)) || (p.Wo != 2 * p.Wi && !(rag && p.Wo == 2 * p.Wi - 1))) return false;
  }
  else if (p.Ho != p.Hi || p.Wo != p.Wi) return false;
  if ((p.flags & GF_RESID) && (p.ldr & 3)) return false;
  if (p.Ho < 1 || p.Wo < 1 || p.M % (p.Ho * p.Wo)) return false;
  const int images = p.M / (p.Ho * p.Wo);
  if (variant == 0) { if (p.Ho != 8 || p.Wo != 8 || images % 3) return false; }
  else if (variant == 1) { if (p.Ho != 16 || p.Wo != 16) return false; }
  else if (variant == 2 || variant == 3) { if (((p.Ho & 7) || (p.Wo & 15)) && !rag) return false; }
  else return false;
  if (p.flags & GF_GNSTATS) {
    if (variant < 2 || nsplit != 1 || !p.st_out || p.gn_cpg < 4 || p.gn_cpg > 64 || (p.N % p.gn_cpg) || p.N / p.gn_cpg > 32) return false;
  }
  if (nsplit < 1 || nsplit > p.Cin / 64) return false;
  if ((size_t)images * p.Hi * p.Wi * p.lda * 2 >= ((size_t)1 << 31) || dtp_conv_ws_packed_elems(p.N, p.Cin, p.A2 ? p.Cin2 : 0) * 2 >= ((size_t)1 << 31)) return false;
  return true;
}

int dtp_launch_conv_ws(const GemmParams& pin, int variant, hipStream_t s) {
  if (!dtp_conv_ws_supported(pin, variant, pin.splits)) {
    dtp_set_error("conv_ws: unsupported problem (M %d N %d Cin %d %dx%d flags %#x, variant %d, %d slices)", pin.M, pin.N, pin.Cin, pin.Hi, pin.Wi, pin.flags, variant, pin.splits);
    return DTP_ERR_ARG;
  }
  const int rc = variant == 0 ? launch_ws<8, 8, 3, 1>(pin, s) : variant == 1 ? launch_ws<16, 16, 1, 1>(pin, s) : variant == 2 ? launch_ws<8, 16, 1, 2>(pin, s) : launch_ws<8, 16, 1, 2, true>(pin, s);
  if (rc != DTP_OK) { dtp_set_error("conv_ws launch failed: %s", hipGetErrorString(hipGetLastError())); return rc; }
  if (pin.splits > 1 && !(pin.flags & GF_NOREDUCE)) return dtp_launch_splitk_reduce(pin, s);
  return DTP_OK;
}
```

### diffusiontexturepainting_amd/csrc/engine.h

```cpp
#pragma once
#include <deque>
#include <functional>
#include <map>
#include <string>
#include <tuple>
#include <unordered_map>
#include <vector>

#include "../../include/dtp.h"
#include "common.h"

#define RC(x)            \
  do {                   \
    int rc_ = (x);       \
    if (rc_) return rc_; \
  } while (0)

struct Staged {
  float* d = nullptr;
  std::vector<int64_t> shape;
  size_t n = 0;
};

struct ConvW {
  f16* w = nullptr;
  f16* wcb = nullptr;
  f16* wfr = nullptr;
  float* b = nullptr;
  float* lns = nullptr;
  int cout = 0, cin = 0 , cin_true = 0, taps = 1, K = 0, ldw = 0;
  int cin2 = 0;
  unsigned char* w8 = nullptr;
  int ldw8 = 0;
  float w8_scale = 1.f;
};
struct NormW {
  float *g = nullptr, *b = nullptr;
  int c = 0;
};

struct T {
  f16* p = nullptr;
  int B = 0, H = 0, W = 0, C = 0, ld = 0;
  long long rows() const { return (long long)B * H * W; }
};

struct T8 {
  unsigned char* p = nullptr;
  int B = 0, H = 0, W = 0, C = 0, ld = 0;
  const float* scale_host = nullptr;
  float scale = 1.f;
  int amax_slot1 = 0;
  long long rows() const { return (long long)B * H * W; }
  float now() const { return scale_host ? *scale_host : scale; }
};

struct Ctx;

using Op = std::function<int(hipStream_t, int )>;
struct ProfRec {
  int kind;
  double flops, bytes;
  hipEvent_t e0, e1;
  const char* label;
};
struct LastGemm {
  bool valid = false;
  GemmParams p;
  int tile = 0, bias_step_off = -1;
  size_t op_index = 0;
  int kind = 0;
  double flops = 0, bytes = 0;
  std::string label;
};
struct Prog {
  std::vector<Op> ops;
  LastGemm last_gemm;
  int run(hipStream_t s, int step) const {
    for (const Op& o : ops) RC(o(s, step));
    return DTP_OK;
// ... 174 lines not shown
struct Ctx {
  int device = 0, R = 0, h = 0, maxB = 1, num_cu = 256;
  bool finalized = false;
  std::unordered_map<std::string, Staged> staged;

  std::vector<void*> chunks;
  char* cur = nullptr;
  size_t cur_left = 0, arena_total = 0;
  Pool pool;
  std::vector<void*> persistent;
  f16* zero = nullptr;
  float* ws = nullptr;
  size_t ws_bytes = 0, ws_need = 0;

  UNetW unet;
  VaeW vae;
  ImgEncW ienc;

  std::map<int, UNetProg> unet_progs;
  std::map<int, VaeEncProg> enc_progs;
  std::map<int, VaeDecProg> dec_progs;

  float* temb_table = nullptr;
  int temb_rows = 0;
  f16* temb_sin = nullptr;
  f16 *temb_h1 = nullptr, *temb_h2 = nullptr;
  int sched_steps = -1;
  int sched_kind = -1;
  int scheduler = DTP_SCHED_DDIM;

  float* cond32 = nullptr;
  float* brush32 = nullptr;
  bool slot_set[DTP_MAX_SLOTS] = {};
  unsigned long long slot_version[DTP_MAX_SLOTS] = {};
  unsigned long long cond_version = 0;
  int* slot_map = nullptr;

  float* x32 = nullptr;
  float* hist32 = nullptr;
  float* canvas32 = nullptr;
  float* alpha_tmp = nullptr;
  StampParams* stamp_params = nullptr;
  std::map<int, StampBufs> stamp_bufs;
  IencBufs ienc_bufs;
  int* finite_flag = nullptr;
  bool check_finite = false;
  bool dedupe_prefix = true;
  bool fuse_gn_conv = false;
  bool fuse_xattn = true;
  bool fold_gn_linear = true;
  bool fuse_reduce_gn = true;
  bool pack_ws = false;
  bool conv_ws = true, conv_ws_vae = true;
  bool gemm_ws = false;
  bool gn_epilogue = true;
  bool reduce_in_concat_gn = true;
  bool gna_lnlin = true;
  bool tune_lnlin = true, tune_halo3 = true;
  bool xchain = true;
  bool xattn_tiles = true;
  int ffchain = -1;
  bool fp8_linear = false;
  bool fp8_attention = false;
  bool fp8_operands = false;
  std::deque<float> fp8_scales;
  std::deque<Fp8Cal> fp8_cals;
  unsigned int* fp8_amax = nullptr;
  int fp8_nslots = 0;
  bool calibrating = false;
  bool finite_pending = false;
  std::map<StageKey, StampGraph> graphs;
  unsigned long long graph_clock = 0;
  hipEvent_t ev[4] = {nullptr, nullptr, nullptr, nullptr};
  int last_evals = 0, last_nodes = 0, last_unet_rows = 0;
  std::map<int, unsigned char*> stroke_masks;
  int last_stroke_stamps = -1, last_stroke_groups = 0, last_stroke_evals = 0;
  int* mesh_face_idx = nullptr;
  unsigned char* mesh_disc = nullptr;
  struct Journal* journal_open = nullptr;
  bool use_graph = true;
  bool exec_imgenc_ready = false;
  bool profile = false;
  std::vector<ProfRec> prof;
  bool autotune = true;
  std::map<std::string, std::pair<int, int>> tuned;
  std::map<std::string, std::pair<float, float>> tune_ms;
  double rep_cold_ms = 0, rep_hot_ms = 0;
  hipEvent_t tune_ev[2] = {nullptr, nullptr};
  void* tune_thrash = nullptr;
  std::string tune_cache_path;
  size_t tune_saved = 0;

  std::unordered_map<std::string, float*> refit_base;
  std::vector<RefitTarget> refit_targets;
  std::vector<RowsumJob> refit_rowsums;
  std::vector<TransposeJob> refit_transposes;
  std::unordered_map<std::string, Staged> refit_staged;
  void* refit_tables = nullptr;
  hipEvent_t refit_ev[2] = {nullptr, nullptr};
  int refit_matrices = -1, refit_launches = 0;
  float refit_ms = 0.f;
};

int ctx_arena_alloc(Ctx* c, size_t bytes, void** out);
int ctx_pool_get(Ctx* c, size_t bytes, void** out);
void ctx_pool_put(Ctx* c, void* p);
int ctx_persistent(Ctx* c, size_t bytes, void** out, bool zero);
void mesh_drop_ctx(Ctx* c);
void journal_drop_ctx(Ctx* c);
struct Journal* journal_armed(Ctx* c, const void* texture, int H, int W);
int journal_save_windows(struct Journal* j, int R, const int* xs, const int* ys, int k, int wrap, hipStream_t s);
int journal_save_box(struct Journal* j, const int* bb, int grow, hipStream_t s);
void delta_drop_ctx(Ctx* c);
const Staged* ctx_find(Ctx* c, const std::string& name);
int ctx_fetch_host(Ctx* c, const std::string& name, std::vector<float>& out);
int ctx_upload_f32(Ctx* c, const std::vector<float>& v, float** out);
int load_norm(Ctx* c, const std::string& name, NormW& n);
int load_conv(Ctx* c, const std::string& name, ConvW& w, int cin_pad = 0, bool bias = true);
int load_conv_with_shortcut(Ctx* c, const std::string& conv, const std::string& shortcut, ConvW& w);
int load_linear_pair(Ctx* c, const std::string& first, const std::string& second, ConvW& w);
int load_linear(Ctx* c, const std::vector<std::string>& names, ConvW& w, bool bias, bool geglu = false,
                const std::string& fold_ln = std::string());
int load_plain_f16(Ctx* c, const std::string& name, f16** out);

int dtp_launch_lora_refit(const LoraRefitJob* jobs, int njobs, int max_n, int max_k, float scale, hipStream_t s);
int dtp_launch_lora_wbeta(const LoraRefitJob* jobs, int njobs, int max_n, float scale, hipStream_t s);
int dtp_launch_rowsum_f16_grouped(const RowsumJob* jobs, int njobs, int max_rows, hipStream_t s);
int dtp_launch_transpose_f16_grouped(const TransposeJob* jobs, int njobs, int max_rows, int max_cols, hipStream_t s);

struct RowStats {
  float* buf = nullptr;
  int parts = 0, M = 0;
  int rows_total = 0, row_off = 0;
};

void prog_push(Ctx* c, Prog* prog, int kind, double flops, double bytes, Op fn, const std::string& label);
int push_gemm(Ctx* c, Prog* prog, GemmParams p, int bias_step_off, double k_alg, RowStats* emit = nullptr);
bool dtp_conv_output_can_carry_gn_stats(const GemmParams& p);

struct MemRange { const void* p; size_t bytes; };

struct ReduceClaim {
  bool claimed = false;
  GemmParams p = {};
  int bias_step_off = -1;
  explicit operator bool() const { return claimed; }
  size_t slab_bytes() const;
  std::vector<MemRange> busy() const;
  GnReduceSrc src(const Ctx* c, int step) const;
};

struct GnOnLoad { const float *part = nullptr, *gamma = nullptr, *beta = nullptr; float eps = 0.f; int nchunk = 0, cpg = 0; };
struct Conv3Opts {
  int extra_flags = 0;
  void* out_override = nullptr; int ldc_override = 0;
  const T* tail = nullptr;
  const T* dst = nullptr;
  GnOnLoad gn;
  static Conv3Opts into(const T& view) { Conv3Opts o; o.dst = &view; return o; }
  static Conv3Opts f32_out(float* out, int ldc) { Conv3Opts o; o.extra_flags = GF_OUT_F32; o.out_override = out; o.ldc_override = ldc; return o; }
};

struct Builder {
  Ctx* c;
  Prog* prog;
  bool fp8 = false;
  bool f8ops = false;
  void push(int kind, double flops, double bytes, Op fn, const std::string& label = std::string());
  T alloc(int B, int H, int W, int C);
  void release(const T& t);
  int gn(const T& x, const NormW& n, float eps, bool silu, T& y);
// ... 101 lines not shown
```

### diffusiontexturepainting_amd/csrc/engine.hip

```cpp
#include "engine.h"

#include <algorithm>

static size_t up_to(size_t x, size_t m) { return (x + m - 1) / m * m; }

int ctx_arena_alloc(Ctx* c, size_t bytes, void** out) {
  bytes = up_to(bytes, 256);
  if (bytes > c->cur_left) {
    const size_t chunk = std::max(bytes, (size_t)512 << 20);
    void* p = nullptr;
    HIP_CHECK(hipMalloc(&p, chunk));
    HIP_CHECK(hipMemset(p, 0, chunk));
    c->chunks.push_back(p);
    c->cur = (char*)p;
    c->cur_left = chunk;
    c->arena_total += chunk;
  }
  *out = c->cur;
  c->cur += bytes;
  c->cur_left -= bytes;
  return DTP_OK;
}

int ctx_pool_get(Ctx* c, size_t bytes, void** out) {
// ... 49 lines not shown
int ctx_upload_f32(Ctx* c, const std::vector<float>& v, float** out) {
  void* p;
  RC(ctx_arena_alloc(c, v.size() * sizeof(float), &p));
  HIP_CHECK(hipMemcpy(p, v.data(), v.size() * sizeof(float), hipMemcpyHostToDevice));
  *out = (float*)p;
  return DTP_OK;
}

int load_norm(Ctx* c, const std::string& name, NormW& n) {
  const Staged *g = ctx_find(c, name + ".weight"), *b = ctx_find(c, name + ".bias");
  if (!g || !b) { dtp_set_error("missing norm '%s'", name.c_str()); return DTP_ERR_MISSING; }
  void *pg, *pb;
  RC(ctx_arena_alloc(c, g->n * 4, &pg));
  RC(ctx_arena_alloc(c, b->n * 4, &pb));
  HIP_CHECK(hipMemcpy(pg, g->d, g->n * 4, hipMemcpyDeviceToDevice));
  HIP_CHECK(hipMemcpy(pb, b->d, b->n * 4, hipMemcpyDeviceToDevice));
  n.g = (float*)pg; n.b = (float*)pb; n.c = (int)g->n;
  return DTP_OK;
}

int load_conv(Ctx* c, const std::string& name, ConvW& w, int cin_pad, bool bias) {
  const Staged* s = ctx_find(c, name + ".weight");
  if (!s) { dtp_set_error("missing weight '%s.weight'", name.c_str()); return DTP_ERR_MISSING; }
  const int cout = (int)s->shape[0], cin = (int)s->shape[1];
  const int taps = s->shape.size() == 4 ? (int)(s->shape[2] * s->shape[3]) : 1;
  if (cin_pad <= 0) cin_pad = (int)up_to(cin, 8);
  w.cout = cout; w.cin = cin_pad; w.cin_true = cin; w.taps = taps; w.K = taps * cin_pad; w.ldw = (int)up_to(w.K, 64);
  void* p;
  RC(ctx_arena_alloc(c, up_to(cout, 128) * (size_t)w.ldw * 2, &p));
  w.w = (f16*)p;
  RC(dtp_launch_pack_conv_weight(s->d, w.w, cout, cin, cin_pad, taps, w.ldw, 0));
  if (taps == 9 && (cin & 63) == 0) {
    void* p2;
    RC(ctx_arena_alloc(c, up_to(cout, 128) * (size_t)w.ldw * 2, &p2));
    w.wcb = (f16*)p2;
    RC(dtp_launch_pack_conv_weight_cb(s->d, w.wcb, cout, cin, w.ldw, 0));
  }
  if (c->pack_ws && taps == 9 && (cin & 63) == 0 && cout >= 32) {
    void* p3;
    RC(ctx_arena_alloc(c, dtp_conv_ws_packed_elems(cout, cin, 0) * 2, &p3));
    w.wfr = (f16*)p3;
    RC(dtp_launch_pack_conv_ws(s->d, nullptr, w.wfr, cout, cin, 0, 0));
  }
  w.b = nullptr;
  if (bias) {
    const Staged* b = ctx_find(c, name + ".bias");
    if (!b) { dtp_set_error("missing bias '%s.bias'", name.c_str()); return DTP_ERR_MISSING; }
    void* pb;
    RC(ctx_arena_alloc(c, b->n * 4, &pb));
    HIP_CHECK(hipMemcpy(pb, b->d, b->n * 4, hipMemcpyDeviceToDevice));
    w.b = (float*)pb;
  }
  return DTP_OK;
}

int load_conv_with_shortcut(Ctx* c, const std::string& conv, const std::string& shortcut, ConvW& w) {
  const Staged *s = ctx_find(c, conv + ".weight"), *t = ctx_find(c, shortcut + ".weight");
  const Staged *sb = ctx_find(c, conv + ".bias"), *tb = ctx_find(c, shortcut + ".bias");
  if (!s || !t || !sb || !tb) { dtp_set_error("missing tensors for '%s' + '%s'", conv.c_str(), shortcut.c_str()); return DTP_ERR_MISSING; }
  const int cout = (int)s->shape[0], cin = (int)s->shape[1], cin2 = (int)t->shape[1];
  if ((int)t->shape[0] != cout || ((9 * cin) & 63) || (cin2 & 63)) { dtp_set_error("shortcut fusion: unsupported shape at '%s'", conv.c_str()); return DTP_ERR_ARG; }
  w.cout = cout; w.cin = cin; w.cin_true = cin; w.taps = 9; w.cin2 = cin2;
  w.K = 9 * cin + cin2; w.ldw = (int)up_to(w.K, 64);
  void* p;
  RC(ctx_arena_alloc(c, up_to(cout, 128) * (size_t)w.ldw * 2, &p));
  w.w = (f16*)p;
  RC(dtp_launch_pack_conv_weight(s->d, w.w, cout, cin, cin, 9, w.ldw, 0));
  RC(dtp_launch_pack_conv_weight(t->d, w.w + 9 * cin, cout, cin2, cin2, 1, w.ldw, 0));
  void* p2;
  RC(ctx_arena_alloc(c, up_to(cout, 128) * (size_t)w.ldw * 2, &p2));
  w.wcb = (f16*)p2;
  RC(dtp_launch_pack_conv_weight_cb(s->d, w.wcb, cout, cin, w.ldw, 0));
  RC(dtp_launch_pack_conv_weight(t->d, w.wcb + 9 * cin, cout, cin2, cin2, 1, w.ldw, 0));
  if (c->pack_ws && (cin & 63) == 0 && cout >= 32) {
    void* p3;
    RC(ctx_arena_alloc(c, dtp_conv_ws_packed_elems(cout, cin, cin2) * 2, &p3));
    w.wfr = (f16*)p3;
    RC(dtp_launch_pack_conv_ws(s->d, t->d, w.wfr, cout, cin, cin2, 0));
  }
  std::vector<float> b1, b2;
  RC(ctx_fetch_host(c, conv + ".bias", b1));
  RC(ctx_fetch_host(c, shortcut + ".bias", b2));
  for (size_t i = 0; i < b1.size(); ++i) b1[i] += b2[i];
  b1.resize(up_to(b1.size(), 128), 0.f);
  return ctx_upload_f32(c, b1, &w.b);
}

static int pack_linear_ws(Ctx* c, ConvW& w) {
  if (!c->pack_ws || !c->gemm_ws || w.taps != 1 || (w.K & 63) || w.K < 128 || w.cout < 32 || (w.cout & 3)) return DTP_OK;
  void* p;
  RC(ctx_arena_alloc(c, dtp_gemm_ws_packed_elems(w.cout, w.K) * 2, &p));
  w.wfr = (f16*)p;
  return dtp_launch_pack_linear_ws(w.w, w.ldw, w.wfr, w.cout, w.K, 0);
}

int load_linear_pair(Ctx* c, const std::string& first, const std::string& second, ConvW& w) {
  const Staged *wa = ctx_find(c, first + ".weight"), *wb = ctx_find(c, second + ".weight");
  const Staged *ba = ctx_find(c, first + ".bias"), *bb = ctx_find(c, second + ".bias");
  if (!wa || !wb || !ba || !bb) { dtp_set_error("linear pair: missing '%s' / '%s'", first.c_str(), second.c_str()); return DTP_ERR_MISSING; }
  const int Na = (int)wa->shape[0], Ka = (int)(wa->n / Na), Nb = (int)wb->shape[0], Kb = (int)(wb->n / Nb);
  if (Kb != Na || (Ka & 63) || (Kb & 63)) { dtp_set_error("linear pair: shapes [%d,%d] then [%d,%d] do not chain", Na, Ka, Nb, Kb); return DTP_ERR_ARG; }
  const int K = Ka + Kb;
  float *prod = nullptr, *cat = nullptr, *bias = nullptr;
  HIP_CHECK(hipMalloc(&prod, (size_t)Nb * Ka * 4));
  HIP_CHECK(hipMalloc(&cat, (size_t)Nb * K * 4));
  HIP_CHECK(hipMalloc(&bias, (size_t)Nb * 4));
// ... 134 lines not shown
```

### diffusiontexturepainting_amd/csrc/tune.hip

```cpp
#include "engine.h"

#include <stdio.h>
#include <stdlib.h>
#include <string.h>
#include <unistd.h>

#include <algorithm>

static void tune_read_file(Ctx* c, const char* path) {
  FILE* f = fopen(path, "r");
  if (!f) return;
  char key[256];
  int tile, splits;
  while (fscanf(f, "%255s %d %d", key, &tile, &splits) == 3)
    if (tile >= 0 && tile < DTP_TILE_IDS && splits >= 1 && splits <= 64) c->tuned[key] = std::make_pair(tile, splits);
  fclose(f);
}

void tune_cache_load(Ctx* c) {
  const char* seed = getenv("DTP_TUNE_SEED");
  if (seed && *seed) tune_read_file(c, seed);
  const char* e = getenv("DTP_TUNE_CACHE");
  if (!e || !*e) return;
  c->tune_cache_path = e;
// ... 62 lines not shown
      continue;
    }
    if (geglu && t.bn != 128) continue;
    if (p.nkb < 3 && t.ns > 2) continue;
    if ((t.bm == 256 && p.M < 192) || (t.bn == 256 && p.N < 192)) continue;
    for (int sp : cand_splits) {
      if (sp > 1 && (geglu || (p.flags & GF_LNFOLD) || p.batch > 1 || p.nkb / sp < 2)) break;
      add(tile, sp);
    }
  }
  {
    static const int ranges[] = {1, 2, 3, 4, 5, 6, 8, 10, 12, 16, 20, 24, 32, 40};
    for (int sp : ranges)
      if (c->tune_lnlin && dtp_lnlin_supported(p, sp)) add(DTP_TILE_LNLIN, sp);
  }
  for (int tile = 0; tile < DTP_TILE_IDS && p.Wcb && dtp_conv_halo_supported(p); ++tile) {
    const DtpTile t = dtp_tile(tile);
    if (t.fam != TF_HALO) continue;
    const bool small = p.Hi * p.Wi <= 256;
    if (t.var < 4 ? (t.var >= 2) != small : (!c->tune_halo3 || !small || !dtp_conv_halo3_supported(p))) continue;
    for (int sp : cand_splits) {
      if (sp > 1 && p.nkb / sp < 9) break;
      add(tile, sp);
    }
  }
  for (int tile = 0; tile < DTP_TILE_IDS; ++tile) {
    const DtpTile t = dtp_tile(tile);
    static const int slices[] = {1, 2, 3, 4, 5, 6, 8, 10};
    if (t.fam != TF_CONVWS) continue;
    for (int sp : slices) {
      if (!c->conv_ws || !ws_ok[t.var] || !dtp_conv_ws_supported(p, t.var, sp)) continue;
      if (t.var >= 2 && sp > 4) continue;
      add(tile, sp);
    }
  }
  if (gw_ok) {
    static const int slices[] = {1, 2, 3, 4, 5, 6, 8};
    for (int sp : slices)
      if (dtp_gemm_ws_supported(p, sp) && !(sp > 1 && p.nkb / sp < 4)) add(DTP_TILE_GEMMWS, sp);
  }
  return out;
}

int tune_gemm(Ctx* c, const GemmParams& p, int* tile, int* sp) {
  char key[200];
  int kl = snprintf(key, sizeof(key), "k8|%d,%d,%d,%d,%d,%d,%d,%d,%d,%d,%d,%d,%d,%d", p.M, p.N, p.K, p.flags & ~GF_MFAST, p.Hi, p.Wi, p.Cin,
                    p.stride, p.lda, p.ldc, p.ldw, p.st_parts, p.Cin2, p.lda2);
  if (p.batch > 1) kl += snprintf(key + kl, sizeof(key) - kl, ",b%d", p.batch);
  if (p.W8) kl += snprintf(key + kl, sizeof(key) - kl, ",f8");
  bool ws_ok[DTP_WS_VARIANTS];
  bool ws_any = false;
  for (int v = 0; v < DTP_WS_VARIANTS; ++v) { ws_ok[v] = p.Wfr && (p.flags & GF_CONV3) && dtp_conv_ws_supported(p, v, 1); ws_any = ws_any || ws_ok[v]; }
  if (ws_any) kl += snprintf(key + kl, sizeof(key) - kl, ",ws2");
  if (!(p.flags & GF_LNFOLD)) {
    bool ll = false;
    for (int r = 1; r <= 40 && !ll; ++r) ll = dtp_lnlin_supported(p, r);
    if (ll) snprintf(key + kl, sizeof(key) - kl, ",ll");
  }
  const bool gw_ok = dtp_gemm_ws_supported(p, 1);
  if (gw_ok) { kl = (int)strlen(key); snprintf(key + kl, sizeof(key) - kl, ",gw"); }
  auto it = c->tuned.find(key);
  if (it != c->tuned.end() && !tune_entry_valid(p, it->second.first, it->second.second)) {
    fprintf(stderr, "[dtp] tune table entry '%s' -> (%d, %d) does not fit the problem; re-tuning\n", key, it->second.first, it->second.second);
    c->tuned.erase(it);
    it = c->tuned.end();
  }
  if (it == c->tuned.end()) {
    if (!c->tune_ev[0]) { HIP_CHECK(hipEventCreate(&c->tune_ev[0])); HIP_CHECK(hipEventCreate(&c->tune_ev[1])); }
    constexpr size_t THRASH_BYTES = (size_t)512 << 20;
    if (!c->tune_thrash) HIP_CHECK(hipMalloc(&c->tune_thrash, THRASH_BYTES));
    const size_t a_bytes = (p.flags & GF_CONV3) ? (size_t)(p.M / (p.Ho * p.Wo)) * p.Hi * p.Wi * p.lda * 2 : (size_t)p.M * p.lda * 2;
    auto time_cfg = [&](int cfg_tile, int cfg_sp, int reps, bool cold, float* out_ms) -> int {
      GemmParams q = p;
      (void)dtp_tile_apply(q, cfg_tile, cfg_sp);
      const size_t need = dtp_gemm_workspace_bytes(q);
      if (need > c->ws_bytes) { c->ws_need = std::max(c->ws_need, need); RC(ensure_ws(c)); }
      q.part = c->ws;
      q.zero = c->zero;
      float ms = 1e30f;
      for (int rep = 0; rep < reps; ++rep) {
        if (cold) {
          HIP_CHECK(hipMemsetAsync(c->tune_thrash, rep, THRASH_BYTES, 0));
          RC(dtp_launch_touch(q.A, a_bytes, (float*)c->tune_thrash, 0));
          if (q.R) RC(dtp_launch_touch(q.R, (size_t)q.M * q.ldr * 2, (float*)c->tune_thrash, 0));
        }
        HIP_CHECK(hipEventRecord(c->tune_ev[0], 0));
        RC(dtp_launch_tile(q, cfg_tile, 0));
        HIP_CHECK(hipEventRecord(c->tune_ev[1], 0));
        HIP_CHECK(hipEventSynchronize(c->tune_ev[1]));
        float ev = 0.f;
        HIP_CHECK(hipEventElapsedTime(&ev, c->tune_ev[0], c->tune_ev[1]));
        if (cold || rep) ms = std::min(ms, ev);
      }
      *out_ms = ms;
      return DTP_OK;
    };
    struct Cand { float ms; int tile, sp; };
    std::vector<Cand> cands;
    for (const TuneCfg& cfg : tune_candidates(c, p, ws_ok, gw_ok)) {
      float ms;
      RC(time_cfg(cfg.tile, cfg.sp, 5, true, &ms));
      cands.push_back({ms, cfg.tile, cfg.sp});
    }
    std::sort(cands.begin(), cands.end(), [](const Cand& x, const Cand& y) { return x.ms < y.ms; });
    for (size_t i = 0; i < cands.size() && i < 3; ++i) {
      float ms;
// ... 35 lines not shown
```

### diffusiontexturepainting_amd/csrc/unet.hip

```cpp
#include <math.h>

#include "engine.h"

static const int CH[4] = {320, 640, 1280, 1280};

static int load_res(Ctx* c, const std::string& p, ResW& w, bool temb, int& temb_off_acc, std::vector<std::string>* tnames) {
  RC(load_norm(c, p + ".norm1", w.n1));
  RC(load_conv(c, p + ".conv1", w.c1));
  RC(load_norm(c, p + ".norm2", w.n2));
  w.has_sc = ctx_find(c, p + ".conv_shortcut.weight") != nullptr;
  if (w.has_sc) RC(load_conv_with_shortcut(c, p + ".conv2", p + ".conv_shortcut", w.c2));
  else RC(load_conv(c, p + ".conv2", w.c2));
  if (temb) {
    w.temb_off = temb_off_acc;
    temb_off_acc += w.c1.cout;
    tnames->push_back(p);
  }
  return DTP_OK;
}

static int load_xf(Ctx* c, const std::string& p, XfW& w, int& kv_counter) {
  const std::string t = p + ".transformer_blocks.0";
  RC(load_norm(c, p + ".norm", w.gn));
  RC(load_conv(c, p + ".proj_in", w.proj_in));
// ... 67 lines not shown
  for (auto& kv : c->staged)
    if (kv.first.rfind("lora.", 0) == 0 && kv.first.find("_lora.down.weight") != std::string::npos) keys.push_back(kv.first);
  for (const std::string& k : keys) {
    const size_t pp = k.find(".processor.");
    if (pp == std::string::npos) continue;
    const std::string module = k.substr(5, pp - 5);
    const size_t ps = pp + 11, pe = k.find("_lora.down.weight");
    const std::string proj = k.substr(ps, pe - ps);
    const std::string upk = "lora." + module + ".processor." + proj + "_lora.up.weight";
    const std::string tgt = "unet." + module + (proj == "to_out" ? ".to_out.0.weight" : "." + proj + ".weight");
    const Staged *dn = ctx_find(c, k), *up = ctx_find(c, upk), *w = ctx_find(c, tgt);
    if (!up || !w) { dtp_set_error("LoRA: missing '%s' or target '%s'", upk.c_str(), tgt.c_str()); return DTP_ERR_MISSING; }
    const int rank = (int)dn->shape[0], K = (int)dn->shape[1], N = (int)up->shape[0];
    if ((int)w->shape[0] != N || (int)w->shape[1] != K || (int)up->shape[1] != rank) {
      dtp_set_error("LoRA: shape mismatch for '%s'", tgt.c_str());
      return DTP_ERR_ARG;
    }
    RC(dtp_launch_lora_merge(w->d, up->d, dn->d, N, K, rank, 1.0f, 0));
  }
  HIP_CHECK(hipDeviceSynchronize());
  return DTP_OK;
}

int load_unet_weights(Ctx* c) {
  RC(keep_refit_bases(c));
  RC(merge_lora(c));
  struct WsScope {
    Ctx* c;
    explicit WsScope(Ctx* cc) : c(cc) { c->pack_ws = c->conv_ws; }
    ~WsScope() { c->pack_ws = false; }
  } ws_scope(c);
  UNetW& u = c->unet;
  const std::string P = "unet.";
  int toff = 0, kvn = 0;
  std::vector<std::string> tn;
  RC(load_conv(c, P + "conv_in", u.conv_in, 16));
  RC(load_linear(c, {P + "time_embedding.linear_1"}, u.t1, true));
  RC(load_linear(c, {P + "time_embedding.linear_2"}, u.t2, true));
  for (int i = 0; i < 4; ++i) {
    for (int j = 0; j < 2; ++j) {
      RC(load_res(c, P + "down_blocks." + std::to_string(i) + ".resnets." + std::to_string(j), u.down_res[i][j], true, toff, &tn));
      if (i < 3) RC(load_xf(c, P + "down_blocks." + std::to_string(i) + ".attentions." + std::to_string(j), u.down_xf[i][j], kvn));
    }
    if (i < 3) RC(load_conv(c, P + "down_blocks." + std::to_string(i) + ".downsamplers.0.conv", u.down_conv[i]));
  }
  RC(load_res(c, P + "mid_block.resnets.0", u.mid_res[0], true, toff, &tn));
  RC(load_xf(c, P + "mid_block.attentions.0", u.mid_xf, kvn));
  RC(load_res(c, P + "mid_block.resnets.1", u.mid_res[1], true, toff, &tn));
  for (int i = 0; i < 4; ++i) {
    for (int j = 0; j < 3; ++j) {
      RC(load_res(c, P + "up_blocks." + std::to_string(i) + ".resnets." + std::to_string(j), u.up_res[i][j], true, toff, &tn));
      if (i > 0) RC(load_xf(c, P + "up_blocks." + std::to_string(i) + ".attentions." + std::to_string(j), u.up_xf[i][j], kvn));
    }
    if (i < 3) RC(load_conv(c, P + "up_blocks." + std::to_string(i) + ".upsamplers.0.conv", u.up_conv[i]));
  }
  RC(load_norm(c, P + "conv_norm_out", u.norm_out));
  RC(load_conv(c, P + "conv_out", u.conv_out));
  u.temb_total = toff;
  std::vector<std::string> names;
  for (auto& p : tn) names.push_back(p + ".time_emb_proj");
  RC(load_linear(c, names, u.tproj, false));
  std::vector<float> bias;
  for (auto& p : tn) {
    std::vector<float> a, b;
    RC(ctx_fetch_host(c, p + ".time_emb_proj.bias", a));
    RC(ctx_fetch_host(c, p + ".conv1.bias", b));
    for (size_t i = 0; i < a.size(); ++i) bias.push_back(a[i] + b[i]);
  }
  bias.resize((bias.size() + 127) / 128 * 128, 0.f);
  RC(ctx_upload_f32(c, bias, &u.tproj.b));
  return DTP_OK;
}

int ensure_temb(Ctx* c, const std::vector<float>& timesteps) {
  const int n = (int)timesteps.size();
  if (n > 1000) { dtp_set_error("temb: too many timesteps"); return DTP_ERR_ARG; }
  if (n > c->temb_rows) {
    const int rows = 1000;
    void* p;
    RC(ctx_persistent(c, (size_t)rows * c->unet.temb_total * 4, &p, true)); c->temb_table = (float*)p;
    RC(ctx_persistent(c, (size_t)rows * 320 * 2, &p, true)); c->temb_sin = (f16*)p;
    RC(ctx_persistent(c, (size_t)rows * 1280 * 2, &p, true)); c->temb_h1 = (f16*)p;
    RC(ctx_persistent(c, (size_t)rows * 1280 * 2, &p, true)); c->temb_h2 = (f16*)p;
    c->temb_rows = rows;
  }
  std::vector<f16> sin_tab((size_t)n * 320);
  for (int i = 0; i < n; ++i)
    for (int j = 0; j < 160; ++j) {
      const float f = expf(-logf(10000.0f) * (float)j / 160.0f);
      const float a = timesteps[i] * f;
      sin_tab[(size_t)i * 320 + j] = (f16)cosf(a);
      sin_tab[(size_t)i * 320 + 160 + j] = (f16)sinf(a);
    }
  HIP_CHECK(hipMemcpy(c->temb_sin, sin_tab.data(), sin_tab.size() * 2, hipMemcpyHostToDevice));
  auto gemm = [&](const f16* A, const ConvW& w, void* C, int flags) -> int {
    GemmParams p = {};
    p.A = A; p.W = w.w; p.C = C; p.bias = w.b; p.zero = c->zero;
    p.M = n; p.N = w.cout; p.K = w.K; p.lda = w.K; p.ldw = w.ldw; p.ldc = w.cout; p.nkb = w.ldw / 64;
    p.flags = flags | GF_BIAS;
    p.splits = 1; p.kb_per_split = p.nkb;
    return dtp_launch_gemm(p, p.M > 64 ? 0 : 3, 0);
  };
  RC(gemm(c->temb_sin, c->unet.t1, c->temb_h1, GF_SILU));
  RC(gemm(c->temb_h1, c->unet.t2, c->temb_h2, GF_SILU));
  RC(gemm(c->temb_h2, c->unet.tproj, c->temb_table, GF_OUT_F32));
  HIP_CHECK(hipDeviceSynchronize());
  return DTP_OK;
// ... 441 lines not shown
```

### diffusiontexturepainting_amd/csrc/vae.hip

```cpp
#include <math.h>


#include "engine.h"

int launch_nhwc_f32_to_nchw(const float* x, float* y, int B, int C, int HW, int ldx, hipStream_t s);

static int load_res_v(Ctx* c, const std::string& p, ResW& w) {
  RC(load_norm(c, p + ".norm1", w.n1));
  RC(load_conv(c, p + ".conv1", w.c1));
  RC(load_norm(c, p + ".norm2", w.n2));
  w.has_sc = ctx_find(c, p + ".conv_shortcut.weight") != nullptr;
  if (w.has_sc) RC(load_conv_with_shortcut(c, p + ".conv2", p + ".conv_shortcut", w.c2));
  else RC(load_conv(c, p + ".conv2", w.c2));
  return DTP_OK;
}

static int load_attn_v(Ctx* c, const std::string& p, VaeAttnW& w) {
  RC(load_norm(c, p + ".group_norm", w.gn));
  RC(load_linear(c, {p + ".query", p + ".key"}, w.qk, true));
  RC(load_linear(c, {p + ".proj_attn"}, w.out, true));
  RC(load_plain_f16(c, p + ".value.weight", &w.wv));
  std::vector<float> bv;
  RC(ctx_fetch_host(c, p + ".value.bias", bv));
  return ctx_upload_f32(c, bv, &w.bv);
}

int load_vae_weights(Ctx* c) {
  struct WsScope {
    Ctx* c;
    explicit WsScope(Ctx* cc) : c(cc) { c->pack_ws = c->conv_ws && c->conv_ws_vae; }
    ~WsScope() { c->pack_ws = false; }
  } ws_scope(c);
  VaeW& v = c->vae;
  const std::string P = "vae.";
  RC(load_conv(c, P + "encoder.conv_in", v.enc_in, 8));
  for (int i = 0; i < 4; ++i) {
    for (int j = 0; j < 2; ++j)
      RC(load_res_v(c, P + "encoder.down_blocks." + std::to_string(i) + ".resnets." + std::to_string(j), v.enc_res[i][j]));
    if (i < 3) RC(load_conv(c, P + "encoder.down_blocks." + std::to_string(i) + ".downsamplers.0.conv", v.enc_down[i]));
  }
  RC(load_res_v(c, P + "encoder.mid_block.resnets.0", v.enc_mid[0]));
  RC(load_attn_v(c, P + "encoder.mid_block.attentions.0", v.enc_attn));
  RC(load_res_v(c, P + "encoder.mid_block.resnets.1", v.enc_mid[1]));
  RC(load_norm(c, P + "encoder.conv_norm_out", v.enc_norm_out));
  RC(load_conv(c, P + "encoder.conv_out", v.enc_out));
  RC(load_conv(c, P + "decoder.conv_in", v.dec_in, 8));
  RC(load_res_v(c, P + "decoder.mid_block.resnets.0", v.dec_mid[0]));
  RC(load_attn_v(c, P + "decoder.mid_block.attentions.0", v.dec_attn));
  RC(load_res_v(c, P + "decoder.mid_block.resnets.1", v.dec_mid[1]));
  for (int i = 0; i < 4; ++i) {
    for (int j = 0; j < 3; ++j)
      RC(load_res_v(c, P + "decoder.up_blocks." + std::to_string(i) + ".resnets." + std::to_string(j), v.dec_res[i][j]));
    if (i < 3) RC(load_conv(c, P + "decoder.up_blocks." + std::to_string(i) + ".upsamplers.0.conv", v.dec_up[i]));
  }
  RC(load_norm(c, P + "decoder.conv_norm_out", v.dec_norm_out));
  RC(load_conv(c, P + "decoder.conv_out", v.dec_out));
  std::vector<float> t;
  RC(ctx_fetch_host(c, P + "quant_conv.weight", t)); RC(ctx_upload_f32(c, t, &v.quant_w));
  RC(ctx_fetch_host(c, P + "quant_conv.bias", t)); RC(ctx_upload_f32(c, t, &v.quant_b));
  RC(ctx_fetch_host(c, P + "post_quant_conv.weight", t)); RC(ctx_upload_f32(c, t, &v.pquant_w));
  RC(ctx_fetch_host(c, P + "post_quant_conv.bias", t)); RC(ctx_upload_f32(c, t, &v.pquant_b));
  return DTP_OK;
}

static int vae_attention(Builder& b, const T& x, const VaeAttnW& w, T& out) {
  Ctx* c = b.c;
  const int C = x.C, S = x.H * x.W, B = x.B;
  T t, qk, o;
  RC(b.gn(x, w.gn, 1e-6f, false, t));
  RC(b.linear(t, w.qk, nullptr, 0, qk));
  o = b.alloc(x.B, x.H, x.W, C);
  const int Sp = (S % 64) ? (S + 63) / 64 * 64 : S;
  T sc = b.alloc(1, 1, S, Sp), vt = b.alloc(1, 1, C, Sp);
  if (!o.p || !sc.p || !vt.p) return DTP_ERR_HIP;
  if (Sp != S) {
    const T scz = sc, vtz = vt;
    b.push(PK_ELEM, 0.0, 2.0 * ((double)S + C) * Sp, [=](hipStream_t s, int) {
      HIP_CHECK(hipMemsetAsync(scz.p, 0, (size_t)S * Sp * sizeof(f16), s));
      HIP_CHECK(hipMemsetAsync(vtz.p, 0, (size_t)C * Sp * sizeof(f16), s));
      return DTP_OK;
    }, "vae attention: zero the k-block tails S=" + std::to_string(S));
  }
  const float scale = 1.0f / sqrtf((float)C);
  for (int bi = 0; bi < B; ++bi) {
    auto push = [&](GemmParams g) {
      int tile = 0;
      g.zero = c->zero;
      g.nkb = (g.K + 63) / 64;
      dtp_gemm_pick(g, &tile, c->num_cu);
      g.splits = 1; g.kb_per_split = g.nkb;
      b.push(dtp_tile(tile).pk, 2.0 * g.M * (double)g.N * g.K, 2.0 * ((double)g.M * g.K + (double)g.N * g.K + (double)g.M * g.N),
             [=](hipStream_t s, int) { return dtp_launch_gemm(g, tile, s); });
    };
    GemmParams g = {};
    g.A = w.wv; g.W = t.p + (size_t)bi * S * t.ld; g.C = vt.p; g.bias = w.bv;
    g.M = C; g.N = S; g.K = C; g.lda = C; g.ldw = t.ld; g.ldc = Sp; g.flags = GF_BIAS_M;
    push(g);
    g = GemmParams();
    g.A = qk.p + (size_t)bi * S * qk.ld; g.W = qk.p + (size_t)bi * S * qk.ld + C; g.C = sc.p;
    g.M = S; g.N = S; g.K = C; g.lda = qk.ld; g.ldw = qk.ld; g.ldc = Sp;
    push(g);
    const T scc = sc;
    b.push(PK_SOFTMAX, 0.0, 4.0 * (double)S * S, [=](hipStream_t s, int) { return dtp_launch_softmax_rows(scc.p, Sp, scc.p, Sp, S, S, scale, s); });
    g = GemmParams();
    g.A = sc.p; g.W = vt.p; g.C = o.p + (size_t)bi * S * o.ld;
    g.M = S; g.N = C; g.K = S; g.lda = Sp; g.ldw = Sp; g.ldc = o.ld;
// ... 214 lines not shown
```

### diffusiontexturepainting_amd/ops.py

```python
import ctypes as C

import torch

from . import _lib
from ._lib import (GF_BIAS, GF_BIAS_M, GF_GEGLU, GF_GELU, GF_LNFOLD, GF_OUT_F32, GF_QUICKGELU, GF_RESID, GemmDesc, check,
                   ptr)


def _stream():
    return C.c_void_p(torch.cuda.current_stream().cuda_stream)


def _up(x, m):
    return (x + m - 1) // m * m


def pack_linear(w, geglu=False):
    lib = _lib.load()
    n, k = w.shape
    out = torch.zeros(_up(n, 128), _up(k, 64), dtype=torch.float16, device=w.device)
    w = w.contiguous().float()
    check(lib.dtp_op_pack_linear(ptr(w), ptr(out), n, k, out.shape[1], int(geglu), _stream()), "pack_linear")
    return out


def pack_conv(w, cin_pad=None):
    lib = _lib.load()
    cout, cin, kh, kw = w.shape
    cin_pad = cin_pad or _up(cin, 8)
    out = torch.zeros(_up(cout, 128), _up(kh * kw * cin_pad, 64), dtype=torch.float16, device=w.device)
    w = w.contiguous().float()
    check(lib.dtp_op_pack_conv(ptr(w), ptr(out), cout, cin, cin_pad, kh * kw, out.shape[1], _stream()), "pack_conv")
    return out


def pack_conv_cb(w):
    lib = _lib.load()
    cout, cin = w.shape[:2]
    out = torch.zeros(_up(cout, 128), 9 * cin, dtype=torch.float16, device=w.device)
    w = w.contiguous().float()
    check(lib.dtp_op_pack_conv_cb(ptr(w), ptr(out), cout, cin, out.shape[1], _stream()), "pack_conv_cb")
    return out


def pack_conv_ws(w, w1=None):
    lib = _lib.load()
    cout, cin = w.shape[:2]
    cin2 = w1.shape[1] if w1 is not None else 0
    out = torch.zeros(lib.dtp_op_pack_conv_ws_elems(cout, cin, cin2), dtype=torch.float16, device=w.device)
    w = w.contiguous().float()
    w1 = w1.reshape(cout, cin2).contiguous().float() if w1 is not None else None
    check(lib.dtp_op_pack_conv_ws(ptr(w), ptr(w1), ptr(out), cout, cin, cin2, _stream()), "pack_conv_ws")
    return out


def pack_linear_ws(wp, n, k):
    lib = _lib.load()
    out = torch.zeros(lib.dtp_op_pack_linear_ws_elems(n, k), dtype=torch.float16, device=wp.device)
    check(lib.dtp_op_pack_linear_ws(ptr(wp), wp.stride(0), ptr(out), n, k, _stream()), "pack_linear_ws")
    return out


def lora_refit(w0, up, down, scale=1.0, gamma=None, out=None, row0=0):
    lib = _lib.load()
    n, k = w0.shape
    if out is None:
        out = torch.zeros(_up(row0 + n, 128), _up(k, 64), dtype=torch.float16, device=w0.device)
    if out.dim() != 2 or out.dtype != torch.float16 or out.stride(1) != 1 or out.shape[0] < row0 + n:
        raise ValueError(f"lora_refit: out must be f16 [>= {row0 + n}, ldw] with unit column stride, got {tuple(out.shape)}")
    w0 = w0.contiguous().float()
    rank = 0 if up is None else up.shape[1]
    up = up.contiguous().float() if up is not None else None
    down = down.contiguous().float() if down is not None else None
    gamma = gamma.contiguous().float() if gamma is not None else None
    check(lib.dtp_op_lora_refit(ptr(w0), ptr(up), ptr(down), rank, float(scale), ptr(gamma), ptr(out), int(row0), n, k, out.stride(0),
                                _stream()), "lora_refit")
    return out


def rowsum(wp, k):
    lib = _lib.load()
    out = torch.empty(wp.shape[0], dtype=torch.float32, device=wp.device)
    check(lib.dtp_op_rowsum(ptr(wp), wp.stride(0), k, ptr(out), wp.shape[0], _stream()), "rowsum")
    return out


def quantize_w8(wp, k):
    lib = _lib.load()
    out = torch.zeros(wp.shape[0], _up(k, 128), dtype=torch.uint8, device=wp.device)
    sc = C.c_float()
    check(lib.dtp_op_quantize_w8(ptr(wp), wp.stride(0), k, wp.shape[0], ptr(out), out.shape[1], C.byref(sc), _stream()), "quantize_w8")
    return out, sc.value


def quant_e4m3(x, scale, ln=False, stats_in=None, eps=1e-5, k=None, x2=None, scale2=1.0, ln2=False, k2=None):
    lib = _lib.load()
    m = x.shape[0]
    k = k or x.shape[1]
    y = torch.empty(m, k, dtype=torch.uint8, device=x.device)
    y2 = None
    if x2 is not None:
        k2 = k2 or x2.shape[1]
        y2 = torch.empty(m, k2, dtype=torch.uint8, device=x.device)
    st = stats_in.contiguous() if stats_in is not None else None
    check(lib.dtp_op_quant_e4m3(ptr(x), x.stride(0), ptr(y), y.stride(0), k, float(scale), int(ln),
# ... 37 lines not shown
        st = st[:d.st_parts_out]
    return out, out8, st


def gemm(a, wp, n, k=None, bias=None, resid=None, flags=0, tile=-1, splits=0, out=None, lda=None, lns=None, ln_eps=1e-5, batch=0,
         sm_valid=0, bias_shared=False, tail=None, row_stats=False, stats_in=None, w8=None, w_scale=1.0, a_scale=1.0, layernorm=False,
         wfr=None):
    lib = _lib.load()
    m = a.shape[0] // batch if batch > 1 else a.shape[0]
    k = k or a.shape[1]
    n_out = n // 2 if flags & GF_GEGLU else n
    if out is None:
        out = torch.empty(a.shape[0], n_out, dtype=torch.float32 if flags & GF_OUT_F32 else torch.float16, device=a.device)
    d = GemmDesc()
    d.A, d.W, d.C = a.data_ptr(), wp.data_ptr(), out.data_ptr()
    d.bias = bias.data_ptr() if bias is not None else None
    d.R = resid.data_ptr() if resid is not None else None
    d.M, d.N, d.K = m, n, k
    d.lda, d.ldw, d.ldc = lda or a.stride(0), wp.stride(0), out.stride(0)
    d.ldr = resid.stride(0) if resid is not None else 0
    d.flags = flags | (GF_BIAS if bias is not None and not flags & GF_BIAS_M else 0) | (GF_RESID if resid is not None else 0)
    d.tile, d.splits = tile, splits
    if lns is not None:
        d.lns, d.ln_eps = lns.data_ptr(), ln_eps
        d.flags |= GF_LNFOLD
    if batch > 1:
        npad = wp.shape[0] // batch
        d.batch, d.a_bs, d.w_bs, d.c_bs = batch, m * d.lda, npad * d.ldw, m * d.ldc
        d.r_bs, d.bias_bs, d.lns_bs = m * d.ldr, 0 if bias_shared else npad, npad
    d.sm_valid = sm_valid
    if tail is not None:
        d.A2, d.lda2, d.Cin2 = tail.data_ptr(), tail.stride(0), tail.shape[1]
        d.K = k + tail.shape[1]
    if w8 is not None:
        d.W8, d.ldw8, d.w_scale, d.a_scale = w8.data_ptr(), w8.stride(0), w_scale, a_scale
        if layernorm:
            d.flags |= GF_LNFOLD
            d.ln_eps = ln_eps
    if wfr is not None:
        d.Wfr = wfr.data_ptr()
    st = None
    if row_stats:
        st = torch.zeros((n + 63) // 64, a.shape[0], 2, dtype=torch.float32, device=a.device)
        d.st_out = st.data_ptr()
        d.flags |= _lib.GF_ROWSTATS
    if stats_in is not None:
        d.st_in, d.st_parts = stats_in.data_ptr(), stats_in.shape[0]
    check(lib.dtp_op_gemm(C.byref(d), _stream()), "gemm")
    if row_stats:
        return out, st[: d.st_parts_out]
    return out


def conv3x3(x, wp, cout, stride=1, pad=1, upsample=False, bias=None, resid=None, tile=-1, splits=0, out_hw=None, flags=0,
            tail=None, wcb=None, wfr=None, gn_groups=0):
    lib = _lib.load()
    b, h, w, cin = x.shape
    hv, wv = (2 * h, 2 * w) if upsample else (h, w)
    ho, wo = out_hw or ((hv + 2 * pad - 3) // stride + 1, (wv + 2 * pad - 3) // stride + 1)
    out = torch.empty(b, ho, wo, cout, dtype=torch.float32 if flags & GF_OUT_F32 else torch.float16, device=x.device)
    d = GemmDesc()
    d.A, d.W, d.C = x.data_ptr(), wp.data_ptr(), out.data_ptr()
    d.bias = bias.data_ptr() if bias is not None else None
    d.R = resid.data_ptr() if resid is not None else None
    d.M, d.N, d.K = b * ho * wo, cout, 9 * cin + (tail.shape[-1] if tail is not None else 0)
    if tail is not None:
        d.A2, d.lda2, d.Cin2 = tail.data_ptr(), tail.stride(2), tail.shape[-1]
    d.lda, d.ldw, d.ldc = x.stride(2), wp.stride(0), cout
    d.ldr = resid.stride(2) if resid is not None else 0
    d.conv, d.Hi, d.Wi, d.Ho, d.Wo, d.Cin, d.stride, d.pad, d.upsample2x = 1, h, w, ho, wo, cin, stride, pad, int(upsample)
    d.flags = flags | (GF_BIAS if bias is not None else 0) | (GF_RESID if resid is not None else 0)
    d.tile, d.splits = tile, splits
    if wcb is not None:
        d.Wcb = wcb.data_ptr()
    if wfr is not None:
        d.Wfr = wfr.data_ptr()
    st = None
    if gn_groups:
        st = torch.full((b, 2 * ((ho + 7) // 8) * ((wo + 15) // 16), gn_groups, 2), float("nan"), dtype=torch.float32, device=x.device)
        d.st_out, d.gn_cpg = st.data_ptr(), cout // gn_groups
        d.flags |= _lib.GF_GNSTATS
    check(lib.dtp_op_gemm(C.byref(d), _stream()), "conv3x3")
    return (out, st) if gn_groups else out


def groupnorm(x, gamma, beta, groups=32, eps=1e-5, silu=False):
    lib = _lib.load()
    b, c = x.shape[0], x.shape[-1]
    hw = x.numel() // (b * c)
    y = torch.empty_like(x)
    check(lib.dtp_op_groupnorm(ptr(x), c, ptr(y), c, ptr(gamma), ptr(beta), b, hw, c, groups, eps, int(silu), _stream()),
          "groupnorm")
    return y


def groupnorm_apply(x, gamma, beta, partial, groups=32, eps=1e-5, silu=False):
    lib = _lib.load()
    b, c = x.shape[0], x.shape[-1]
    hw = x.numel() // (b * c)
    y = torch.empty_like(x)
    check(lib.dtp_op_groupnorm_apply(ptr(x), c, ptr(y), c, ptr(gamma), ptr(beta), ptr(partial), partial.shape[1], b, hw, c, groups, eps, int(silu),
                                     _stream()), "groupnorm_apply")
    return y


def reduce_groupnorm(part, gamma, beta, bias=None, resid=None, groups=32, eps=1e-5, silu=False, skip=None):
    lib = _lib.load()
    sp, b, hw, cx = part.shape
    c = cx + (skip.shape[-1] if skip is not None else 0)
    out, y = torch.empty(b, hw, c, dtype=torch.float16, device=part.device), torch.empty(b, hw, c, dtype=torch.float16, device=part.device)
    if skip is not None:
        out[..., cx:] = skip
    check(lib.dtp_op_reduce_groupnorm_cx(ptr(part), sp, ptr(bias), ptr(resid), ptr(out), ptr(y), ptr(gamma), ptr(beta), b, hw, c, groups, eps, int(silu), cx,
                                         _stream()), "reduce_groupnorm")
    return out, y


def groupnorm_stats_apply(gamma, beta, x=None, part=None, bias=None, resid=None, groups=32, eps=1e-5, silu=False):
    lib = _lib.load()
    sp, (b, hw, c) = (part.shape[0], part.shape[1:]) if part is not None else (0, x.shape)
    out = x if part is None else torch.empty(b, hw, c, dtype=torch.float16, device=part.device)
    y = torch.empty_like(out)
    check(lib.dtp_op_groupnorm_stats_apply(ptr(part), sp, ptr(bias), ptr(resid), ptr(out), ptr(y), ptr(gamma), ptr(beta), b, hw, c, groups, eps, int(silu),
                                           _stream()), "groupnorm_stats_apply")
    return out, y


def xattn(x, w1, b1, lns1, st_in, w2, b2, n_samples, sm_valid=14, ln_eps=1e-5, row_stats=False, ct=0):
    lib = _lib.load()
    rows, c = x.shape
    s = rows // n_samples
    y = torch.empty_like(x)
    st = torch.zeros((c + 127) // 128, rows, 2, dtype=torch.float32, device=x.device) if row_stats else None
    check(lib.dtp_op_xattn_ct(ptr(x), ptr(w1), ptr(b1), ptr(lns1), ptr(st_in), st_in.shape[0], ptr(w2), ptr(b2), ptr(x), ptr(y), ptr(st), s, c, n_samples,
                              sm_valid, ln_eps, int(ct), _stream()), "xattn")
    return (y, st) if row_stats else y
# ... 366 lines not shown
```

### include/dtp.h

```cpp
#ifndef DTP_H
#define DTP_H
#include <stddef.h>
#include <stdint.h>

#ifdef __cplusplus
extern "C" {
#endif

#define DTP_ABI_VERSION 3

enum { DTP_OK = 0, DTP_ERR_ARG = 1, DTP_ERR_HIP = 2, DTP_ERR_STATE = 3, DTP_ERR_MISSING = 4 };

typedef struct dtp_ctx dtp_ctx;
typedef void* dtp_stream;

int dtp_abi_version(void);
const char* dtp_last_error(void);

int dtp_create(int device, int resolution, int max_batch, dtp_ctx** out);
void dtp_destroy(dtp_ctx* ctx);

int dtp_load_tensor(dtp_ctx* ctx, const char* name, const float* data, int is_device, const int64_t* shape, int ndim);
int dtp_finalize_weights(dtp_ctx* ctx);

// ... 162 lines not shown
  void* C;
  const float* bias;
  const void* R;
  int M, N, K;
  int lda, ldw, ldc, ldr;
  int conv, Hi, Wi, Ho, Wo, Cin, stride, pad, upsample2x;
  int flags;
  int tile;
  int splits;
  const float* lns;
  float ln_eps;
  const void* A2;
  int lda2, Cin2;
  const void* Wcb;
  int batch;
  int64_t a_bs, w_bs, c_bs, r_bs;
  int bias_bs, lns_bs;
  int sm_valid;
  float* st_out;
  const float* st_in;
  int st_parts;
  int st_parts_out;
  const void* W8;
  int ldw8;
  float a_scale, w_scale;
  int gn_cpg;
  const void* Wfr;
  const void* A8;
  int lda8;
  const void* A2_8;
  int lda2_8;
  void* C8;
  int ldc8;
  float c_scale;
  float a2_scale;
} dtp_gemm_desc;
enum { DTP_GF_BIAS = 1, DTP_GF_BIAS_M = 2, DTP_GF_RESID = 4, DTP_GF_GEGLU = 8, DTP_GF_GELU = 64, DTP_GF_QUICKGELU = 128,
       DTP_GF_OUT_F32 = 256, DTP_GF_SILU = 512, DTP_GF_LNFOLD = 1024, DTP_GF_ROWSTATS = 2048, DTP_GF_SOFTMAX16 = 4096,
       DTP_GF_GNSTATS = 1 << 24, DTP_GF_RAGGED = 1 << 25 };

int dtp_op_gemm(dtp_gemm_desc* d, dtp_stream s);
int dtp_op_gemm_f8f8(dtp_gemm_desc* d, dtp_stream s);
int dtp_op_quant_e4m3(const void* x, int ldx, void* y, int ldy, int K, float scale, int ln, const void* x2, int ldx2, void* y2, int ldy2,
                      int K2, float scale2, int ln2, int M, const float* st_in, int st_parts, float eps, dtp_stream s);
int dtp_op_pack_linear(const float* w, void* out, int N, int K, int ldw, int geglu, dtp_stream s);
int dtp_op_lora_refit(const float* w0, const float* up, const float* down, int rank, float scale, const float* gamma, void* out, int row0,
                      int N, int K, int ldw, dtp_stream s);
int dtp_op_rowsum(const void* w, int ld, int K, float* out, int rows, dtp_stream s);
int dtp_op_quantize_w8(const void* w, int ldw, int K, int rows, void* out, int ldw8, float* w_scale, dtp_stream s);
int dtp_op_pack_conv(const float* w, void* out, int Cout, int Cin, int Cin_pad, int taps, int ldw, dtp_stream s);
int dtp_op_pack_conv_cb(const float* w, void* out, int Cout, int Cin, int ldw, dtp_stream s);
int dtp_op_pack_conv_ws(const float* w, const float* w1, void* out, int Cout, int Cin, int Cin2, dtp_stream s);
long long dtp_op_pack_conv_ws_elems(int Cout, int Cin, int Cin2);
int dtp_op_pack_linear_ws(const void* w, int ldw, void* out, int N, int K, dtp_stream s);
long long dtp_op_pack_linear_ws_elems(int N, int K);
int dtp_op_groupnorm(const void* x, int ldx, void* y, int ldy, const float* gamma, const float* beta, int B, int HW, int C,
                     int groups, float eps, int silu, dtp_stream s);
int dtp_op_groupnorm_apply(const void* x, int ldx, void* y, int ldy, const float* gamma, const float* beta, const float* partial, int nchunk,
                           int B, int HW, int C, int groups, float eps, int silu, dtp_stream s);
int dtp_op_groupnorm_stats_apply(const float* part, int splits, const float* bias, const void* resid, void* x, void* y, const float* gamma,
                                 const float* beta, int B, int HW, int C, int groups, float eps, int silu, dtp_stream s);
int dtp_op_measure_peaks(double* mfma_f16_tflops, double* hbm_copy_gbs);
int dtp_op_reduce_groupnorm(const float* part, int splits, const float* bias, const void* resid, void* conv_out, void* y, const float* gamma,
                            const float* beta, int B, int HW, int C, int groups, float eps, int silu, dtp_stream s);
int dtp_op_reduce_groupnorm_cx(const float* part, int splits, const float* bias, const void* resid, void* conv_out, void* y, const float* gamma,
                               const float* beta, int B, int HW, int C, int groups, float eps, int silu, int cx, dtp_stream s);
int dtp_op_xattn(const void* X, const void* W1, const float* b1, const float* lns1, const float* st_in, int st_parts, const void* W2, const float* b2,
                 const void* R, void* Y, float* st_out, int S, int C, int N, int sm_valid, float ln_eps, dtp_stream s);
int dtp_op_xattn_ct(const void* X, const void* W1, const float* b1, const float* lns1, const float* st_in, int st_parts, const void* W2, const float* b2,
                    const void* R, void* Y, float* st_out, int S, int C, int N, int sm_valid, float ln_eps, int ct, dtp_stream s);
int dtp_op_xchain(const void* A, const void* Wo, int ldwo, const float* bo, const void* Y, const void* W1, const float* b1, const float* lns1,
                  const void* W2, const float* b2, void* Y3, float* st_out, int S, int C, int N, int sm_valid, float ln_eps, dtp_stream s);
int dtp_op_ffchain(const void* X, const void* W1, int ldw1, const float* lns1, const float* b1, const void* Wm, int ldwm, const float* bm,
                   const void* R, void* Out, int M, int C, float ln_eps, dtp_stream s);
int dtp_op_gn_fold_weights(const void* x, const void* W, int ldw, const float* bias, const float* gamma, const float* beta, int B, int HW, int C,
                           int Nout, int groups, float eps, void* Wout, float* bias_out, dtp_stream s);
int dtp_op_gn_linear(const void* x, const void* W, int ldw, const float* bias, const float* gamma, const float* beta, int B, int HW, int C,
                     int Nout, int groups, float eps, void* y, float* st_out, int col_ranges, dtp_stream s);
int dtp_op_layernorm(const void* x, int ldx, void* y, int ldy, const float* gamma, const float* beta, int rows, int C,
                     float eps, dtp_stream s);
int dtp_op_attention(const void* Q, const void* K, const void* V, void* O, int ldq, int ldk, int ldv, int ldo, int B, int H,
                     int Sq, int Skv, int D, int64_t qbs, int64_t kbs, int64_t vbs, int64_t obs, float scale, dtp_stream s);
int dtp_op_attention_dma(const void* Q, const void* K, const void* V, void* O, int ldq, int ldk, int ldv, int ldo, int B, int H,
                         int Sq, int Skv, int D, int64_t qbs, int64_t kbs, int64_t vbs, int64_t obs, float scale, int nw, dtp_stream s);
int dtp_op_attention_fp8(const void* Q, const void* K, const void* V, void* O, int ldq, int ldk, int ldv, int ldo, int B, int H,
                         int Sq, int Skv, int D, int64_t qbs, int64_t kbs, int64_t vbs, int64_t obs, float scale, float q_scale,
                         float v_scale, dtp_stream s);
int dtp_op_softmax_rows(const void* x, int ldx, void* y, int ldy, int rows, int cols, float scale, dtp_stream s);
int dtp_op_strength_init(const float* z0, const float* eps, float a, float b, float* x, long long n, dtp_stream s);
int dtp_op_dilate(const float* canvas, float* tmp, float* out, int B, int R, int pad, dtp_stream s);
int dtp_op_dilate_pads(const float* canvas, float* tmp, float* out, int B, int R, const int* pads, dtp_stream s);
int dtp_op_sched_step(int scheduler, const float* eps_out, float* x, float* hist, void* in16, const float* row, const float* next_scale,
                      const float* cfg, const float* tg, const int* rank, int step_index, int B, int hw, int k, dtp_stream s);

int dtp_op_stroke_gather(const uint8_t* texture, int H, int W, float* canvas, int R, int B, const int* xs, const int* ys, const int* modes,
                         int wrap, int over_y, int over_x, dtp_stream s);
int dtp_op_stroke_paste(const float* dec, const uint8_t* mask, uint8_t* texture, int H, int W, int R, int B, const int* xs, const int* ys,
                        const int* modes, int wrap, dtp_stream s);

int dtp_op_mesh_render(dtp_mesh* mesh, const float cam[12], float fov, int flip_normals, const uint8_t* texture, int H, int W, int R, int mode,
                       int over_y, int over_x, float* canvas, int* face_idx, dtp_stream s);
int dtp_op_mesh_backproject(dtp_mesh* mesh, const float* dec, int dec_finished, const uint8_t* mask, const int* face_idx, int R, uint8_t* texture, int H, int W,
                            dtp_stream s);
int dtp_op_mesh_backproject_masked(dtp_mesh* mesh, const float* dec, int dec_finished, const uint8_t* mask, const int* face_idx, int R,
                                   uint8_t* texture, int H, int W, const uint32_t* face_mask, int mask_words, dtp_stream s);
int dtp_op_mesh_pick(dtp_mesh* mesh, const dtp_ray* rays, int n, dtp_mesh_hit* out, dtp_stream s);
// ... 15 lines not shown
```

Measured before the change: 10.19.

## Add sub-pixel phase decomposition for nearest-upsample 3x3 convs (4 taps per phase)

```diff
diff --git a/diffusiontexturepainting_amd/_lib.py b/diffusiontexturepainting_amd/_lib.py
--- a/diffusiontexturepainting_amd/_lib.py
+++ b/diffusiontexturepainting_amd/_lib.py
@@ -191,6 +191,10 @@
     "dtp_op_groupnorm_stats_apply": (_i, [_vp, _i, _vp, _vp, _vp, _vp, _vp, _vp, _i, _i, _i, _i, _f, _i, _vp]),
     "dtp_op_pack_conv_ws": (_i, [_vp, _vp, _vp, _i, _i, _i, _vp]),
     "dtp_op_pack_conv_ws_elems": (C.c_longlong, [_i, _i, _i]),
+    "dtp_op_pack_conv_ws_ups4": (_i, [_vp, _vp, _i, _i, _vp]),
+    "dtp_op_pack_conv_ws_ups4_elems": (C.c_longlong, [_i, _i]),
+    "dtp_op_conv_ups4": (_i, [C.POINTER(GemmDesc), _vp, _vp]),
+    "dtp_op_conv_ws_supported": (_i, [C.POINTER(GemmDesc), _vp, _i, _i]),
     "dtp_op_pack_linear_ws": (_i, [_vp, _i, _vp, _i, _i, _vp]),
     "dtp_op_pack_linear_ws_elems": (C.c_longlong, [_i, _i]),
     "dtp_op_groupnorm": (_i, [_vp, _i, _vp, _i, _vp, _vp, _i, _i, _i, _i, _f, _i, _vp]),
diff --git a/diffusiontexturepainting_amd/csrc/api_ops.hip b/diffusiontexturepainting_amd/csrc/api_ops.hip
--- a/diffusiontexturepainting_amd/csrc/api_ops.hip
+++ b/diffusiontexturepainting_amd/csrc/api_ops.hip
@@ -59,12 +59,7 @@
 int dtp_abi_version(void) { return DTP_ABI_VERSION; }
 const char* dtp_last_error(void) { return g_err; }
 
-int dtp_op_gemm(dtp_gemm_desc* d, dtp_stream s) {
-  std::lock_guard<std::mutex> lk(g_ops_mu);
-  int rc = ops_init();
-  if (rc) return rc;
-  static bool halo_init = false;
-  if (!halo_init) { dtp_conv_halo_init(); dtp_gemm_wide_init(); dtp_lnlin_init(); dtp_conv_ws_init(); dtp_gemm_ws_init(); halo_init = true; }
+static GemmParams desc_params(const dtp_gemm_desc* d, const void* wfr4) {
   GemmParams p = {};
   p.A = (const f16*)d->A; p.W = (const f16*)d->W; p.C = d->C; p.bias = d->bias; p.R = (const f16*)d->R;
   p.zero = g_ops.zero;
@@ -80,8 +75,18 @@
   p.st_out = d->st_out; p.st_in = d->st_in; p.st_parts = d->st_parts;
   if (p.batch > 1) p.st_rows = p.batch * p.M;
   p.W8 = (const unsigned char*)d->W8; p.ldw8 = d->ldw8; p.a_scale = d->a_scale; p.w_scale = d->w_scale;
-  p.Wfr = (const f16*)d->Wfr;
+  p.Wfr = (const f16*)d->Wfr; p.Wfr4 = (const f16*)wfr4;
   p.gn_cpg = d->gn_cpg;
+  return p;
+}
+
+static int op_gemm(dtp_gemm_desc* d, const void* wfr4, dtp_stream s) {
+  std::lock_guard<std::mutex> lk(g_ops_mu);
+  int rc = ops_init();
+  if (rc) return rc;
+  static bool halo_init = false;
+  if (!halo_init) { dtp_conv_halo_init(); dtp_gemm_wide_init(); dtp_lnlin_init(); dtp_conv_ws_init(); dtp_gemm_ws_init(); halo_init = true; }
+  GemmParams p = desc_params(d, wfr4);
   static bool fp8_init = false;
   if (!fp8_init) { dtp_gemm_fp8_init(); fp8_init = true; }
   if (p.ldw < p.nkb * 64) { dtp_set_error("gemm: ldw=%d smaller than padded K=%d", p.ldw, p.nkb * 64); return DTP_ERR_ARG; }
@@ -100,6 +105,12 @@
   p.part = g_ops.ws;
   if (p.flags & GF_ROWSTATS) d->st_parts_out = dtp_tile_row_parts(p, tile);
   return dtp_launch_tile(p, tile, (hipStream_t)s);
+}
+
+int dtp_op_gemm(dtp_gemm_desc* d, dtp_stream s) { return op_gemm(d, nullptr, s); }
+int dtp_op_conv_ups4(dtp_gemm_desc* d, const void* wfr4, dtp_stream s) {
+  if (!d || !d->conv || !d->upsample2x || !wfr4) { dtp_set_error("conv_ups4: a 3x3 conv over the 2x upsample and its phase weights"); return DTP_ERR_ARG; }
+  return op_gemm(d, wfr4, s);
 }
 
 int dtp_op_gemm_f8f8(dtp_gemm_desc* d, dtp_stream s) {
@@ -184,6 +195,15 @@
 }
 long long dtp_op_pack_linear_ws_elems(int N, int K) { return (long long)dtp_gemm_ws_packed_elems(N, K); }
 long long dtp_op_pack_conv_ws_elems(int Cout, int Cin, int Cin2) { return (long long)dtp_conv_ws_packed_elems(Cout, Cin, Cin2); }
+int dtp_op_pack_conv_ws_ups4(const float* w, void* out, int Cout, int Cin, dtp_stream s) {
+  return dtp_launch_pack_conv_ws_ups4(w, (f16*)out, Cout, Cin, (hipStream_t)s);
+}
+long long dtp_op_pack_conv_ws_ups4_elems(int Cout, int Cin) { return (long long)dtp_conv_ws_ups4_packed_elems(Cout, Cin); }
+int dtp_op_conv_ws_supported(const dtp_gemm_desc* d, const void* wfr4, int tile, int splits) {
+  const DtpTile t = dtp_tile(tile);
+  if (!d || t.fam != TF_CONVWS) return 0;
+  return dtp_conv_ws_supported(desc_params(d, wfr4), t.var, splits < 1 ? 1 : splits) ? 1 : 0;
+}
 
 int dtp_op_groupnorm(const void* x, int ldx, void* y, int ldy, const float* gamma, const float* beta, int B, int HW, int C,
                      int groups, float eps, int silu, dtp_stream s) {
diff --git a/diffusiontexturepainting_amd/csrc/builder.hip b/diffusiontexturepainting_amd/csrc/builder.hip
--- a/diffusiontexturepainting_amd/csrc/builder.hip
+++ b/diffusiontexturepainting_amd/csrc/builder.hip
@@ -326,6 +326,7 @@
     if (!sp) { dtp_set_error("push_gemm: no lnlin configuration for the GroupNorm-on-load Linear (M %d N %d K %d)", p.M, p.N, p.K); return DTP_ERR_ARG; }
   }
   if (c->autotune) RC(tune_gemm(c, p, &tile, &sp));
+  if (c->ups_phase >= 2 && dtp_conv_ws_supported(p, 2 + c->ups_phase, 1)) { tile = DTP_TILE_WSUPS4 + c->ups_phase - 2; sp = 1; }
   (void)dtp_tile_apply(p, tile, sp);
   const DtpTile t = dtp_tile(tile);
   if (emit) {
@@ -342,7 +343,7 @@
   char lab[160];
   const bool f8tile = t.fam == TF_FP8;
   snprintf(lab, sizeof(lab), "%s M=%d N=%d K=%d tile=%d splits=%d%s%s%s%s", (p.flags & GF_CONV3) ? "conv3" : "gemm", p.M, p.N, p.K, tile,
-           t.split == SPLIT_COLS ? p.col_ranges : p.splits, (p.flags & GF_UPS2) ? " ups" : "", (p.flags & GF_GEGLU) ? (f8tile ? " geglu fp8" : " geglu") : (f8tile ? " fp8" : ""), p.stride == 2 ? " s2" : "",
+           t.split == SPLIT_COLS ? p.col_ranges : p.splits, (p.flags & GF_UPS2) ? (t.fam == TF_CONVWS && t.var >= 4 ? " ups4" : " ups") : "", (p.flags & GF_GEGLU) ? (f8tile ? " geglu fp8" : " geglu") : (f8tile ? " fp8" : ""), p.stride == 2 ? " s2" : "",
            p.batch > 1 ? (" x" + std::to_string(p.batch)).c_str() : "");
   const double flops = 2.0 * nb * p.M * (double)p.N * k_alg;
   prog_push(c, prog, t.pk, flops, bytes, make_gemm_op(c, p, tile, bias_step_off), lab);
@@ -369,6 +370,7 @@
   if (o.tail) { p.A2 = o.tail->p; p.lda2 = o.tail->ld; p.Cin2 = w.cin2; }
   p.Wcb = w.wcb;
   p.Wfr = w.wfr;
+  if (ups && c->ups_phase) p.Wfr4 = w.wfr4;
   if (o.extra_flags & GF_GNAPPLY) {
     if (!o.gn.part) { dtp_set_error("conv3: GF_GNAPPLY without GroupNorm parameters"); return DTP_ERR_ARG; }
     p.gn_part = o.gn.part; p.gn_gamma = o.gn.gamma; p.gn_beta = o.gn.beta; p.gn_eps = o.gn.eps;
diff --git a/diffusiontexturepainting_amd/csrc/common.h b/diffusiontexturepainting_amd/csrc/common.h
--- a/diffusiontexturepainting_amd/csrc/common.h
+++ b/diffusiontexturepainting_amd/csrc/common.h
@@ -216,6 +216,7 @@
   const f16* W;
   const f16* Wcb;
   const f16* Wfr;
+  const f16* Wfr4;
   void* C;
   float* part;
   const float* bias;
@@ -415,9 +416,10 @@
 void dtp_gemm_wide_init();
 constexpr int DTP_TILE_LNLIN = 50;
 constexpr int DTP_TILE_WS0 = 51;
-constexpr int DTP_WS_VARIANTS = 4;
+constexpr int DTP_WS_VARIANTS = 6;
 constexpr int DTP_TILE_GEMMWS = 55;
-constexpr int DTP_TILE_IDS = 56;
+constexpr int DTP_TILE_WSUPS4 = 56;
+constexpr int DTP_TILE_IDS = 58;
 
 enum { PK_GEMM0 = 0, PK_ATTN = 12, PK_GN = 13, PK_LN = 14, PK_ELEM = 15, PK_SOFTMAX = 16, PK_HALO0 = 17, PK_BIG0 = 21, PK_WIDE0 = 25, PK_FP8 = 27, PK_KH2 = 28, PK_LW = 36, PK_XATTN = 44, PK_HALO3 = 45, PK_LNLIN = 47, PK_WS0 = 48, PK_GEMMWS = 52, PK_F8F8 = 53, PK_QUANT8 = 54, PK_COUNT = 55 };
 
@@ -450,7 +452,9 @@
   if (id >= 40 && id < 48) return {TF_GEMM, 0, sm[s], sn[s], 3, 1, id < 44 ? 4 : 8, SPLIT_K, PK_LW + id - 40};
   if (id == 48 || id == 49) return {TF_HALO, id - 44, 0, 0, 0, 0, 0, SPLIT_HALO, PK_HALO3 + id - 48};
   if (id == DTP_TILE_LNLIN) return {TF_LNLIN, 0, 0, 0, 0, 0, 0, SPLIT_COLS, PK_LNLIN};
-  if (id >= DTP_TILE_WS0 && id < DTP_TILE_WS0 + DTP_WS_VARIANTS) return {TF_CONVWS, id - DTP_TILE_WS0, 0, 0, 0, 0, 0, SPLIT_BLOCKS, PK_WS0 + id - DTP_TILE_WS0};
+  if (id >= DTP_TILE_WS0 && id < DTP_TILE_WS0 + 4) return {TF_CONVWS, id - DTP_TILE_WS0, 0, 0, 0, 0, 0, SPLIT_BLOCKS, PK_WS0 + id - DTP_TILE_WS0};
+  if (id == DTP_TILE_WSUPS4 || id == DTP_TILE_WSUPS4 + 1)
+    return {TF_CONVWS, 4 + id - DTP_TILE_WSUPS4, 0, 0, 0, 0, 0, SPLIT_BLOCKS, PK_WS0 + 2 + id - DTP_TILE_WSUPS4};
   if (id == DTP_TILE_GEMMWS) return {TF_GEMMWS, 0, 64, 64, 0, 0, 0, SPLIT_BLOCKS, PK_GEMMWS};
   return {};
 }
@@ -484,6 +488,8 @@
 size_t dtp_conv_ws_packed_elems(int Cout, int Cin, int Cin2);
 int dtp_conv_ws_gn_chunks(int Ho, int Wo);
 int dtp_launch_pack_conv_ws(const float* w, const float* w1, f16* out, int Cout, int Cin, int Cin2, hipStream_t s);
+size_t dtp_conv_ws_ups4_packed_elems(int Cout, int Cin);
+int dtp_launch_pack_conv_ws_ups4(const float* w, f16* out, int Cout, int Cin, hipStream_t s);
 bool dtp_gemm_ws_supported(const GemmParams& p, int nsplit);
 int dtp_launch_gemm_ws(const GemmParams& p, hipStream_t s);
 void dtp_gemm_ws_init();
diff --git a/diffusiontexturepainting_amd/csrc/context.hip b/diffusiontexturepainting_amd/csrc/context.hip
--- a/diffusiontexturepainting_amd/csrc/context.hip
+++ b/diffusiontexturepainting_amd/csrc/context.hip
@@ -51,6 +51,7 @@
   c->tune_lnlin = !on("DTP_NO_LNLIN"); c->tune_halo3 = !on("DTP_NO_HALO3");
   c->xchain = !on("DTP_NO_XCHAIN"); c->xattn_tiles = !on("DTP_XATTN_CT1");
   if (const char* e = getenv("DTP_FFCHAIN")) c->ffchain = atoi(e);
+  if (const char* e = getenv("DTP_UPS_PHASE")) c->ups_phase = std::min(std::max(atoi(e), 0), 3);
   *out = (dtp_ctx*)c;
   return DTP_OK;
 }
@@ -232,6 +233,16 @@
   if (!strcmp(name, "use_graph")) { c->use_graph = value != 0; return DTP_OK; }
   if (!strcmp(name, "autotune")) { c->autotune = value != 0; return DTP_OK; }
   if (!strcmp(name, "check_finite")) { c->check_finite = value != 0; return DTP_OK; }
+  if (!strcmp(name, "ups_phase")) {
+    if (value < 0 || value > 3) { dtp_set_error("dtp_set_option: ups_phase %d is not 0 .. 3", value); return DTP_ERR_ARG; }
+    if (!c->unet_progs.empty() || !c->enc_progs.empty() || !c->dec_progs.empty()) {
+      dtp_set_error("dtp_set_option: ups_phase must be chosen before the first launch program is built");
+      return DTP_ERR_STATE;
+    }
+    if (value && !c->ups_phase && c->finalized) { dtp_set_error("dtp_set_option: ups_phase was 0 when the weights were packed"); return DTP_ERR_STATE; }
+    c->ups_phase = value;
+    return DTP_OK;
+  }
   if (!strcmp(name, "fuse_gn_conv")) {
 #ifndef DTP_EXPERIMENTAL
     if (value) { dtp_set_error("dtp_set_option: fuse_gn_conv is an experiment (slower: DESIGN.md 3.6) -- build with DTP_EXPERIMENTAL=1"); return DTP_ERR_ARG; }
diff --git a/diffusiontexturepainting_amd/csrc/conv_ws.hip b/diffusiontexturepainting_amd/csrc/conv_ws.hip
--- a/diffusiontexturepainting_amd/csrc/conv_ws.hip
+++ b/diffusiontexturepainting_amd/csrc/conv_ws.hip
@@ -17,7 +17,7 @@
 template <int N>
 __device__ __forceinline__ void wait_vmcnt() { asm volatile("s_waitcnt vmcnt(%0)" ::"n"(N) : "memory"); }
 
-template <int TH, int TW, int NI, int NT, bool CO = false>
+template <int TH, int TW, int NI, int NT, bool CO = false, int TAPS = 9>
 struct WsGeom {
   static constexpr int PW = TW + 3, PH = TH + 2;
   static constexpr int HP1 = PH * PW, HP = NI * HP1;
@@ -31,11 +31,12 @@
   static constexpr int STATB = (NI == 1 && NT == 2) ? (4 * NT * 32 * 2 + NT * 32 * 2) * 8 : 0;
   static constexpr int LDS = MAINB + STATB;
   static constexpr int LT = (HL - 1) / (NT * TM);
-  static constexpr int WAITB = (17 - LT) * NT;
+  static constexpr int WAITB = (2 * TAPS - 1 - LT) * NT;
   static_assert(TW == 8 || TW == 16, "pixel tile width");
   static_assert(TH % RPT == 0 && (NI * TH * TW) % 32 == 0, "whole MFMA tiles");
   static_assert(HP * 128 < 65536, "fragment offsets are 16-bit immediates");
-  static_assert(LT < 8 && WAITB < 64, "patch pieces fit in the taps before the barrier; vmcnt is a 6-bit counter");
+  static_assert(TAPS == 9 || (TAPS == 4 && TH == 8 && TW == 16 && NI == 1 && NT == 2), "nine taps, or the four of the phase build");
+  static_assert(LT < TAPS - 1 && WAITB < 64, "patch pieces fit in the taps before the barrier; vmcnt is a 6-bit counter");
   static_assert(LDS <= (CO ? 80 : 160) * 1024, "LDS");
 };
 
@@ -64,6 +65,32 @@
   }
 }
 
+__global__ void pack_conv_ws_ups4_kernel(const float* __restrict__ w, f16* __restrict__ out, int Cout, int Cin, long long total) {
+  for (long long i = (long long)blockIdx.x * 256 + threadIdx.x; i < total; i += (long long)gridDim.x * 256) {
+    const int e = (int)(i & 7), l = (int)((i >> 3) & 63);
+    long long f = i >> 9;
+    const int tap = (int)(f & 3); f >>= 2;
+    const int wq = (int)(f & 3); f >>= 2;
+    const int ncb = Cin >> 6, nts = (Cout + 31) >> 5;
+    const int cb = (int)(f % ncb); f /= ncb;
+    const int nt = (int)(f % nts), ph = (int)(f / nts);
+    const int py = ph >> 1, px = ph & 1, ry = tap >> 1, rx = tap & 1;
+    const int ky0 = ry ? 1 + py : 0, ky1 = ry ? 2 : py, kx0 = rx ? 1 + px : 0, kx1 = rx ? 2 : px;
+    const int n = nt * 32 + (l & 31), ch = cb * 64 + 16 * wq + 8 * (l >> 5) + e;
+    float sum = 0.f;
+    if (n < Cout) {
+      const float* src = w + ((size_t)n * Cin + ch) * 9;
+      bool first = true;
+      for (int ky = ky0; ky <= ky1; ++ky)
+        for (int kx = kx0; kx <= kx1; ++kx) {
+          sum = first ? src[ky * 3 + kx] : sum + src[ky * 3 + kx];
+          first = false;
+        }
+    }
+    out[i] = (f16)sum;
+  }
+}
+
 template <class G, int KY, int J>
 __device__ __forceinline__ void rd_frags(f16x8 (&dst)[G::TM], uint32_t ct) {
   if constexpr (J < G::TM) {
@@ -72,29 +99,35 @@
   }
 }
 
-template <int TH, int TW, int NI, int NT, bool NTW, bool CO = false, bool RAG = false>
+template <int TH, int TW, int NI, int NT, bool NTW, bool CO = false, bool RAG = false, int TAPS = 9>
 __global__ __launch_bounds__(256, CO ? 2 : 1) void convws_kernel(const GemmParams p) {
-  using G = WsGeom<TH, TW, NI, NT, CO>;
+  using G = WsGeom<TH, TW, NI, NT, CO, TAPS>;
   constexpr int TM = G::TM, HL = G::HL, PW = G::PW, PH = G::PH, HP1 = G::HP1, PB = G::PBYTES, NTM = NT * TM;
+  constexpr bool PHASE = TAPS == 4;
+  constexpr int LAST = TAPS - 1, KW = PHASE ? 2 : 3;
+  static_assert(!(PHASE && RAG), "the phase build covers aligned maps only");
   extern __shared__ __attribute__((aligned(16))) char smem[];
 
   const int tid = threadIdx.x, lane = tid & 63;
   const int wave = __builtin_amdgcn_readfirstlane(tid >> 6);
   const int frow = lane & 31, fhalf = lane >> 5;
 
-  const int H = p.Ho, W = p.Wo;
+  const int H = PHASE ? p.Hi : p.Ho, W = PHASE ? p.Wi : p.Wo;
   const int tiles_x = RAG ? (W + TW - 1) / TW : W / TW, tiles_y = RAG ? (H + TH - 1) / TH : H / TH;
   const int hw = H * W;
   const bool pow2 = ((hw & (hw - 1)) | (tiles_x & (tiles_x - 1)) | (tiles_y & (tiles_y - 1))) == 0;
-  const int images = pow2 ? (p.M >> __builtin_ctz(hw)) : p.M / hw;
+  const int mrows = PHASE ? p.M >> 2 : p.M;
+  const int images = pow2 ? (mrows >> __builtin_ctz(hw)) : mrows / hw;
   const int npg = (images / NI) * tiles_y * tiles_x;
   const int nts = (p.N + 31) >> 5, nrs = (nts + NT - 1) / NT, S = p.splits;
-  const int units = nrs * S;
+  const int units = nrs * S * (PHASE ? 4 : 1);
   const int xcd = blockIdx.x & 7, idx = blockIdx.x >> 3;
   int pg, u;
   if ((units & 7) == 0) { const int q = idx / npg; pg = idx - q * npg; u = q * 8 + xcd; }
   else { const int pgq = (npg + 7) >> 3; const int q = idx / pgq; pg = (idx - q * pgq) * 8 + xcd; u = q; }
   if (u >= units || pg >= npg) return;
+  const int phase = PHASE ? u & 3 : 0, phy = phase >> 1, phx = phase & 1;
+  if (PHASE) u >>= 2;
   const int ncb = p.Cin >> 6;
   int z = 0, nr = u, mb0 = 0, mb1 = ncb;
   if (S > 1) {
@@ -110,23 +143,23 @@
   }
   const int y0 = ty * TH, x0 = tx * TW;
 
-  const auto rsW = __builtin_amdgcn_make_buffer_rsrc((void*)p.Wfr, 0, (int)0x80000000u, 0x00020000);
+  const auto rsW = __builtin_amdgcn_make_buffer_rsrc((void*)(PHASE ? p.Wfr4 : p.Wfr), 0, (int)0x80000000u, 0x00020000);
   constexpr int OOB = (int)0x80000000u;
   int wvoff[NT], wbase[NT];
 #pragma unroll
   for (int i = 0; i < NT; ++i) {
     const int nt = nr * NT + i;
     wvoff[i] = nt < nts ? lane * 16 : OOB;
-    wbase[i] = (nt < nts ? nt : 0) * ncb * 4 + wave;
+    wbase[i] = (phase * nts + (nt < nts ? nt : 0)) * ncb * 4 + wave;
   }
   auto wload = [&](int i, int cb, int tap) -> f16x8 {
-    const u32x4 v = __builtin_amdgcn_raw_buffer_load_b128(rsW, wvoff[i], ((wbase[i] + cb * 4) * 9 + tap) * 1024, NTW ? 2 : 0);
+    const u32x4 v = __builtin_amdgcn_raw_buffer_load_b128(rsW, wvoff[i], ((wbase[i] + cb * 4) * TAPS + tap) * 1024, NTW ? 2 : 0);
     return __builtin_bit_cast(f16x8, v);
   };
-  f16x8 wf[NT][9];
+  f16x8 wf[NT][TAPS];
   if (mb0 < mb1) {
 #pragma unroll
-    for (int t = 0; t < 9; ++t)
+    for (int t = 0; t < TAPS; ++t)
 #pragma unroll
       for (int i = 0; i < NT; ++i) wf[i][t] = wload(i, mb0, t);
   }
@@ -135,7 +168,7 @@
   const auto rsA = __builtin_amdgcn_make_buffer_rsrc((void*)p.A, 0, (int)0x80000000u, 0x00020000);
   int voffA[HL];
   {
-    const int ups = (p.flags & GF_UPS2) ? 1 : 0;
+    const int ups = (!PHASE && (p.flags & GF_UPS2)) ? 1 : 0;
     const int s0 = wave * 8 + (lane >> 3);
     int il = 0, hy = s0 / PW, hx = s0 - hy * PW;
     constexpr int DY = 32 / PW, DX = 32 - DY * PW;
@@ -165,8 +198,8 @@
   const int pxl = frow % TW, pyl = frow / TW;
   uint32_t colterm[3];
 #pragma unroll
-  for (int kx = 0; kx < 3; ++kx)
-    colterm[kx] = lds_addr(smem) + (pyl * PW + pxl + kx) * 128 + ((((2 * wave + fhalf) ^ ((pxl + kx) & 7))) << 4);
+  for (int kx = 0; kx < KW; ++kx)
+    colterm[kx] = lds_addr(smem) + ((pyl + phy) * PW + pxl + kx + phx) * 128 + ((((2 * wave + fhalf) ^ ((pxl + kx + phx) & 7))) << 4);
 
   f32x16 acc[NT][TM];
 #pragma unroll
@@ -176,10 +209,11 @@
 #pragma unroll
       for (int r = 0; r < 16; ++r) acc[i][j][r] = 0.f;
 
-  constexpr int NBF = CO ? 2 : 3;
+  constexpr bool XB = !CO || PHASE;
+  constexpr int NBF = PHASE ? 2 : CO ? 2 : 3;
   f16x8 bf[NBF][TM];
   auto rd = [&](auto tapc, uint32_t bo, f16x8 (&dst)[TM]) {
-    constexpr int TAP = decltype(tapc)::value, KY = TAP / 3, KX = TAP % 3;
+    constexpr int TAP = decltype(tapc)::value, KY = TAP / KW, KX = TAP % KW;
 #ifndef DTP_WS_NO_LDSREAD
     rd_frags<G, KY, 0>(dst, colterm[KX] + bo);
 #else
@@ -201,7 +235,7 @@
 #else
 #define DTP_WS_WAIT(n, f) wait_lds_frags<n, TM>(f)
 #endif
-        if constexpr (TAP < 8) {
+        if constexpr (TAP < LAST) {
           rd(std::integral_constant<int, TAP + 1>{}, bo, bf[NXT]);
           __builtin_amdgcn_sched_barrier(0);
           DTP_WS_WAIT(TM, bf[CUR]);
@@ -210,7 +244,7 @@
           if constexpr (MORE) {
             wait_vmcnt<G::WAITB>();
             __builtin_amdgcn_s_barrier();
-            if constexpr (!CO) {
+            if constexpr (XB) {
               rd(std::integral_constant<int, 0>{}, bo1, bf[NXT]);
               __builtin_amdgcn_sched_barrier(0);
             }
@@ -242,13 +276,16 @@
           for (int i = 0; i < NT; ++i) wf[i][TAP] = wload(i, cb + 1, TAP);
 #endif
           __builtin_amdgcn_sched_barrier(0);
-          if constexpr (CO && TAP == 8) rd(std::integral_constant<int, 0>{}, bo1, bf[0]);
+          if constexpr (!XB && TAP == LAST) rd(std::integral_constant<int, 0>{}, bo1, bf[0]);
         }
       };
 #undef DTP_WS_WAIT
       tap(std::integral_constant<int, 0>{}); tap(std::integral_constant<int, 1>{}); tap(std::integral_constant<int, 2>{});
-      tap(std::integral_constant<int, 3>{}); tap(std::integral_constant<int, 4>{}); tap(std::integral_constant<int, 5>{});
-      tap(std::integral_constant<int, 6>{}); tap(std::integral_constant<int, 7>{}); tap(std::integral_constant<int, 8>{});
+      tap(std::integral_constant<int, 3>{});
+      if constexpr (TAPS == 9) {
+        tap(std::integral_constant<int, 4>{}); tap(std::integral_constant<int, 5>{});
+        tap(std::integral_constant<int, 6>{}); tap(std::integral_constant<int, 7>{}); tap(std::integral_constant<int, 8>{});
+      }
     };
     typedef std::true_type Y;
     typedef std::false_type N_;
@@ -266,7 +303,7 @@
     do_cb(N_{}, N_{}, cb, bo, bo1, bo2);
   }
 
-  if (p.A2 && !(p.sm_valid & 1)) {
+  if (TAPS == 9 && p.A2 && !(p.sm_valid & 1)) {
     const int ntb = p.Cin2 >> 6;
     const int tk0 = (int)((long long)z * ntb / S), tk1 = (int)((long long)(z + 1) * ntb / S);
     if (tk0 < tk1) {
@@ -376,7 +413,8 @@
         for (int e = 0; e < 4; ++e) v[e] = ((v0[e] + v1[e]) + v2[e]) + v3[e];
         const int il = j / G::TPI, py = G::RPT * (j % G::TPI) + epyl;
         if (RAG && (y0 + py >= H || x0 + epxl >= W)) continue;
-        const size_t m = ((size_t)(img0 + il) * H + y0 + py) * W + x0 + epxl;
+        const size_t m = PHASE ? ((size_t)(img0 + il) * p.Ho + 2 * (y0 + py) + phy) * p.Wo + 2 * (x0 + epxl) + phx
+                               : ((size_t)(img0 + il) * H + y0 + py) * W + x0 + epxl;
         if (!ncol) continue;
         if (p.splits > 1) {
           *(f32x4*)(p.part + ((size_t)z * p.M + m) * p.N + n) = v;
@@ -428,7 +466,7 @@
         const int a = max(g * cpg, c_lo), b = min((g + 1) * cpg, c_hi);
         double sg = 0.0, qg = 0.0;
         for (int c = a; c < b; ++c) { sg += tot[(c - c_lo) * 2]; qg += tot[(c - c_lo) * 2 + 1]; }
-        const int ntile = tiles_x * tiles_y, pt = ty * tiles_x + tx;
+        const int ntile = tiles_x * tiles_y * (PHASE ? 4 : 1), pt = (ty * tiles_x + tx) * (PHASE ? 4 : 1) + phase;
         float* const base = p.st_out + ((size_t)img0 * 2 * ntile + 2 * pt) * groups * 2;
         float* const mine = base + (size_t)(nr & 1) * groups * 2 + g * 2;
         mine[0] = (float)sg; mine[1] = (float)qg;
@@ -465,6 +503,26 @@
   return hipGetLastError() == hipSuccess ? DTP_OK : DTP_ERR_HIP;
 }
 
+template <bool CO>
+int launch_ws_phase(const GemmParams& p, hipStream_t s) {
+  using G = WsGeom<8, 16, 1, 2, CO, 4>;
+  const int npg = (p.M / (p.Ho * p.Wo)) * (p.Hi / 8) * (p.Wi / 16);
+  const int units = (((p.N + 31) >> 5) + 1) / 2 * 4;
+  const int blocks = (units & 7) == 0 ? units * npg : ((npg + 7) >> 3) * 8 * units;
+  static const int dbg = [] { const char* e = getenv("DTP_WS_DEBUG"); return e ? atoi(e) : 0; }();
+  GemmParams q = p;
+  q.sm_valid = dbg & 3;
+  const bool nt = (dbg & 4) ? false : (dbg & 8) ? true : npg == 1;
+  if (nt) hipLaunchKernelGGL((convws_kernel<8, 16, 1, 2, true, CO, false, 4>), dim3(blocks), dim3(256), G::LDS, s, q);
+  else hipLaunchKernelGGL((convws_kernel<8, 16, 1, 2, false, CO, false, 4>), dim3(blocks), dim3(256), G::LDS, s, q);
+  return hipGetLastError() == hipSuccess ? DTP_OK : DTP_ERR_HIP;
+}
+template <bool CO>
+void set_ws_phase_attr() {
+  (void)hipFuncSetAttribute((const void*)convws_kernel<8, 16, 1, 2, true, CO, false, 4>, hipFuncAttributeMaxDynamicSharedMemorySize, WsGeom<8, 16, 1, 2, CO, 4>::LDS);
+  (void)hipFuncSetAttribute((const void*)convws_kernel<8, 16, 1, 2, false, CO, false, 4>, hipFuncAttributeMaxDynamicSharedMemorySize, WsGeom<8, 16, 1, 2, CO, 4>::LDS);
+}
+
 template <int TH, int TW, int NI, int NT, bool CO = false>
 void set_ws_attr() {
   (void)hipFuncSetAttribute((const void*)convws_kernel<TH, TW, NI, NT, true, CO>, hipFuncAttributeMaxDynamicSharedMemorySize, WsGeom<TH, TW, NI, NT, CO>::LDS);
@@ -482,6 +540,8 @@
   set_ws_attr<16, 16, 1, 1>();
   set_ws_attr<8, 16, 1, 2>();
   set_ws_attr<8, 16, 1, 2, true>();
+  set_ws_phase_attr<false>();
+  set_ws_phase_attr<true>();
 }
 
 int dtp_conv_ws_gn_chunks(int Ho, int Wo) { return 2 * ((Ho + 7) / 8) * ((Wo + 15) / 16); }
@@ -501,7 +561,25 @@
   return hipGetLastError() == hipSuccess ? DTP_OK : DTP_ERR_HIP;
 }
 
+size_t dtp_conv_ws_ups4_packed_elems(int Cout, int Cin) { return (size_t)((Cout + 31) / 32) * (size_t)(Cin / 64) * 4 * 16 * 512; }
+
+int dtp_launch_pack_conv_ws_ups4(const float* w, f16* out, int Cout, int Cin, hipStream_t s) {
+  if (Cout < 1 || Cin < 64 || (Cin & 63)) { dtp_set_error("pack_conv_ws_ups4: Cin %d must be a multiple of 64", Cin); return DTP_ERR_ARG; }
+  const long long total = (long long)dtp_conv_ws_ups4_packed_elems(Cout, Cin);
+  const int blocks = (int)((total + 255) / 256 > 65535 ? 65535 : (total + 255) / 256);
+  hipLaunchKernelGGL(pack_conv_ws_ups4_kernel, dim3(blocks), dim3(256), 0, s, w, out, Cout, Cin, total);
+  return hipGetLastError() == hipSuccess ? DTP_OK : DTP_ERR_HIP;
+}
+
 bool dtp_conv_ws_supported(const GemmParams& p, int variant, int nsplit) {
+  if (variant == 4 || variant == 5) {
+    if (!p.Wfr4 || !(p.flags & GF_UPS2) || p.A2 || nsplit != 1) return false;
+    if (p.Ho != 2 * p.Hi || p.Wo != 2 * p.Wi || (p.Hi & 7) || (p.Wi & 15)) return false;
+    if (dtp_conv_ws_ups4_packed_elems(p.N, p.Cin) * 2 >= ((size_t)1 << 31)) return false;
+    GemmParams q = p;
+    if (!q.Wfr) q.Wfr = q.Wfr4;
+    return dtp_conv_ws_supported(q, variant - 2, 1);
+  }
   if (!p.Wfr || !(p.flags & GF_CONV3) || p.batch > 1) return false;
   if (p.A2 && ((p.Cin2 & 63) || (p.lda2 & 7) || (size_t)p.M * p.lda2 * 2 >= ((size_t)1 << 31))) return false;
   if (p.flags & (GF_GEGLU | GF_OUT_F32 | GF_LNFOLD | GF_ROWSTATS | GF_BIAS_M | GF_GELU | GF_QUICKGELU | GF_SILU | GF_GNAPPLY | GF_SOFTMAX16)) return false;
@@ -531,7 +609,8 @@
     dtp_set_error("conv_ws: unsupported problem (M %d N %d Cin %d %dx%d flags %#x, variant %d, %d slices)", pin.M, pin.N, pin.Cin, pin.Hi, pin.Wi, pin.flags, variant, pin.splits);
     return DTP_ERR_ARG;
   }
-  const int rc = variant == 0 ? launch_ws<8, 8, 3, 1>(pin, s) : variant == 1 ? launch_ws<16, 16, 1, 1>(pin, s) : variant == 2 ? launch_ws<8, 16, 1, 2>(pin, s) : launch_ws<8, 16, 1, 2, true>(pin, s);
+  const int rc = variant == 0 ? launch_ws<8, 8, 3, 1>(pin, s) : variant == 1 ? launch_ws<16, 16, 1, 1>(pin, s) : variant == 2 ? launch_ws<8, 16, 1, 2>(pin, s)
+               : variant == 3 ? launch_ws<8, 16, 1, 2, true>(pin, s) : variant == 4 ? launch_ws_phase<false>(pin, s) : launch_ws_phase<true>(pin, s);
   if (rc != DTP_OK) { dtp_set_error("conv_ws launch failed: %s", hipGetErrorString(hipGetLastError())); return rc; }
   if (pin.splits > 1 && !(pin.flags & GF_NOREDUCE)) return dtp_launch_splitk_reduce(pin, s);
   return DTP_OK;
diff --git a/diffusiontexturepainting_amd/csrc/engine.h b/diffusiontexturepainting_amd/csrc/engine.h
--- a/diffusiontexturepainting_amd/csrc/engine.h
+++ b/diffusiontexturepainting_amd/csrc/engine.h
@@ -26,6 +26,7 @@
   f16* w = nullptr;
   f16* wcb = nullptr;
   f16* wfr = nullptr;
+  f16* wfr4 = nullptr;
   float* b = nullptr;
   float* lns = nullptr;
   int cout = 0, cin = 0 , cin_true = 0, taps = 1, K = 0, ldw = 0;
@@ -306,6 +307,7 @@
   bool fuse_reduce_gn = true;
   bool pack_ws = false;
   bool conv_ws = true, conv_ws_vae = true;
+  int ups_phase = 1;
   bool gemm_ws = false;
   bool gn_epilogue = true;
   bool reduce_in_concat_gn = true;
@@ -371,6 +373,7 @@
 int ctx_upload_f32(Ctx* c, const std::vector<float>& v, float** out);
 int load_norm(Ctx* c, const std::string& name, NormW& n);
 int load_conv(Ctx* c, const std::string& name, ConvW& w, int cin_pad = 0, bool bias = true);
+int load_conv_ups4(Ctx* c, const std::string& name, ConvW& w);
 int load_conv_with_shortcut(Ctx* c, const std::string& conv, const std::string& shortcut, ConvW& w);
 int load_linear_pair(Ctx* c, const std::string& first, const std::string& second, ConvW& w);
 int load_linear(Ctx* c, const std::vector<std::string>& names, ConvW& w, bool bias, bool geglu = false,
diff --git a/diffusiontexturepainting_amd/csrc/engine.hip b/diffusiontexturepainting_amd/csrc/engine.hip
--- a/diffusiontexturepainting_amd/csrc/engine.hip
+++ b/diffusiontexturepainting_amd/csrc/engine.hip
@@ -125,6 +125,16 @@
     w.b = (float*)pb;
   }
   return DTP_OK;
+}
+
+int load_conv_ups4(Ctx* c, const std::string& name, ConvW& w) {
+  if (!c->ups_phase || !w.wfr || w.taps != 9 || w.cin2) return DTP_OK;
+  const Staged* s = ctx_find(c, name + ".weight");
+  if (!s) { dtp_set_error("missing weight '%s.weight'", name.c_str()); return DTP_ERR_MISSING; }
+  void* p;
+  RC(ctx_arena_alloc(c, dtp_conv_ws_ups4_packed_elems(w.cout, w.cin_true) * 2, &p));
+  w.wfr4 = (f16*)p;
+  return dtp_launch_pack_conv_ws_ups4(s->d, w.wfr4, w.cout, w.cin_true, 0);
 }
 
 int load_conv_with_shortcut(Ctx* c, const std::string& conv, const std::string& shortcut, ConvW& w) {
diff --git a/diffusiontexturepainting_amd/csrc/tune.hip b/diffusiontexturepainting_amd/csrc/tune.hip
--- a/diffusiontexturepainting_amd/csrc/tune.hip
+++ b/diffusiontexturepainting_amd/csrc/tune.hip
@@ -138,6 +138,7 @@
   bool ws_any = false;
   for (int v = 0; v < DTP_WS_VARIANTS; ++v) { ws_ok[v] = p.Wfr && (p.flags & GF_CONV3) && dtp_conv_ws_supported(p, v, 1); ws_any = ws_any || ws_ok[v]; }
   if (ws_any) kl += snprintf(key + kl, sizeof(key) - kl, ",ws2");
+  if (ws_ok[4] || ws_ok[5]) kl += snprintf(key + kl, sizeof(key) - kl, ",u4");
   if (!(p.flags & GF_LNFOLD)) {
     bool ll = false;
     for (int r = 1; r <= 40 && !ll; ++r) ll = dtp_lnlin_supported(p, r);
diff --git a/diffusiontexturepainting_amd/csrc/unet.hip b/diffusiontexturepainting_amd/csrc/unet.hip
--- a/diffusiontexturepainting_amd/csrc/unet.hip
+++ b/diffusiontexturepainting_amd/csrc/unet.hip
@@ -143,7 +143,10 @@
       RC(load_res(c, P + "up_blocks." + std::to_string(i) + ".resnets." + std::to_string(j), u.up_res[i][j], true, toff, &tn));
       if (i > 0) RC(load_xf(c, P + "up_blocks." + std::to_string(i) + ".attentions." + std::to_string(j), u.up_xf[i][j], kvn));
     }
-    if (i < 3) RC(load_conv(c, P + "up_blocks." + std::to_string(i) + ".upsamplers.0.conv", u.up_conv[i]));
+    if (i < 3) {
+      RC(load_conv(c, P + "up_blocks." + std::to_string(i) + ".upsamplers.0.conv", u.up_conv[i]));
+      RC(load_conv_ups4(c, P + "up_blocks." + std::to_string(i) + ".upsamplers.0.conv", u.up_conv[i]));
+    }
   }
   RC(load_norm(c, P + "conv_norm_out", u.norm_out));
   RC(load_conv(c, P + "conv_out", u.conv_out));
diff --git a/diffusiontexturepainting_amd/csrc/vae.hip b/diffusiontexturepainting_amd/csrc/vae.hip
--- a/diffusiontexturepainting_amd/csrc/vae.hip
+++ b/diffusiontexturepainting_amd/csrc/vae.hip
@@ -51,7 +51,10 @@
   for (int i = 0; i < 4; ++i) {
     for (int j = 0; j < 3; ++j)
       RC(load_res_v(c, P + "decoder.up_blocks." + std::to_string(i) + ".resnets." + std::to_string(j), v.dec_res[i][j]));
-    if (i < 3) RC(load_conv(c, P + "decoder.up_blocks." + std::to_string(i) + ".upsamplers.0.conv", v.dec_up[i]));
+    if (i < 3) {
+      RC(load_conv(c, P + "decoder.up_blocks." + std::to_string(i) + ".upsamplers.0.conv", v.dec_up[i]));
+      RC(load_conv_ups4(c, P + "decoder.up_blocks." + std::to_string(i) + ".upsamplers.0.conv", v.dec_up[i]));
+    }
   }
   RC(load_norm(c, P + "decoder.conv_norm_out", v.dec_norm_out));
   RC(load_conv(c, P + "decoder.conv_out", v.dec_out));
diff --git a/diffusiontexturepainting_amd/ops.py b/diffusiontexturepainting_amd/ops.py
--- a/diffusiontexturepainting_amd/ops.py
+++ b/diffusiontexturepainting_amd/ops.py
@@ -51,6 +51,15 @@
     w = w.contiguous().float()
     w1 = w1.reshape(cout, cin2).contiguous().float() if w1 is not None else None
     check(lib.dtp_op_pack_conv_ws(ptr(w), ptr(w1), ptr(out), cout, cin, cin2, _stream()), "pack_conv_ws")
+    return out
+
+
+def pack_conv_ws_ups4(w):
+    lib = _lib.load()
+    cout, cin = w.shape[:2]
+    out = torch.zeros(lib.dtp_op_pack_conv_ws_ups4_elems(cout, cin), dtype=torch.float16, device=w.device)
+    w = w.contiguous().float()
+    check(lib.dtp_op_pack_conv_ws_ups4(ptr(w), ptr(out), cout, cin, _stream()), "pack_conv_ws_ups4")
     return out
 
 
@@ -194,9 +203,8 @@
     return out
 
 
-def conv3x3(x, wp, cout, stride=1, pad=1, upsample=False, bias=None, resid=None, tile=-1, splits=0, out_hw=None, flags=0,
-            tail=None, wcb=None, wfr=None, gn_groups=0):
-    lib = _lib.load()
+def _conv3x3_desc(x, wp, cout, stride=1, pad=1, upsample=False, bias=None, resid=None, tile=-1, splits=0, out_hw=None, flags=0,
+                  tail=None, wcb=None, wfr=None, gn_groups=0, wfr4=None):
     b, h, w, cin = x.shape
     hv, wv = (2 * h, 2 * w) if upsample else (h, w)
     ho, wo = out_hw or ((hv + 2 * pad - 3) // stride + 1, (wv + 2 * pad - 3) // stride + 1)
@@ -222,8 +230,21 @@
         st = torch.full((b, 2 * ((ho + 7) // 8) * ((wo + 15) // 16), gn_groups, 2), float("nan"), dtype=torch.float32, device=x.device)
         d.st_out, d.gn_cpg = st.data_ptr(), cout // gn_groups
         d.flags |= _lib.GF_GNSTATS
-    check(lib.dtp_op_gemm(C.byref(d), _stream()), "conv3x3")
-    return (out, st) if gn_groups else out
+    return d, out, st
+
+
+def conv3x3(x, wp, cout, *args, **kw):
+    d, out, st = _conv3x3_desc(x, wp, cout, *args, **kw)
+    if kw.get("wfr4") is not None:
+        check(_lib.load().dtp_op_conv_ups4(C.byref(d), ptr(kw["wfr4"]), _stream()), "conv3x3")
+    else:
+        check(_lib.load().dtp_op_gemm(C.byref(d), _stream()), "conv3x3")
+    return (out, st) if st is not None else out
+
+
+def conv_ws_supported(x, wp, cout, tile, splits=1, **kw):
+    d, _, _ = _conv3x3_desc(x, wp, cout, tile=tile, splits=splits, **kw)
+    return bool(_lib.load().dtp_op_conv_ws_supported(C.byref(d), ptr(kw.get("wfr4")), tile, splits))
 
 
 def groupnorm(x, gamma, beta, groups=32, eps=1e-5, silu=False):
diff --git a/include/dtp.h b/include/dtp.h
--- a/include/dtp.h
+++ b/include/dtp.h
@@ -238,6 +238,10 @@
 int dtp_op_pack_conv_cb(const float* w, void* out, int Cout, int Cin, int ldw, dtp_stream s);
 int dtp_op_pack_conv_ws(const float* w, const float* w1, void* out, int Cout, int Cin, int Cin2, dtp_stream s);
 long long dtp_op_pack_conv_ws_elems(int Cout, int Cin, int Cin2);
+int dtp_op_pack_conv_ws_ups4(const float* w, void* out, int Cout, int Cin, dtp_stream s);
+long long dtp_op_pack_conv_ws_ups4_elems(int Cout, int Cin);
+int dtp_op_conv_ups4(dtp_gemm_desc* d, const void* wfr4, dtp_stream s);
+int dtp_op_conv_ws_supported(const dtp_gemm_desc* d, const void* wfr4, int tile, int splits);
 int dtp_op_pack_linear_ws(const void* w, int ldw, void* out, int N, int K, dtp_stream s);
 long long dtp_op_pack_linear_ws_elems(int N, int K);
 int dtp_op_groupnorm(const void* x, int ldx, void* y, int ldy, const float* gamma, const float* beta, int B, int HW, int C,
```

After: 10.33 (median of 6 runs). 1.4% higher.
